# Genesis-Embodied-AI/ThinShellLab

Hardware: AMD Instinct MI355X
Metric: element-steps/s (fwd+adjoint), 100k-tri cloth; 1/2/4/8-GPU scaling (higher is better)
Workload: dtype f64

## Files before the change

### include/tsl_hip.h

```cpp
#ifndef TSL_HIP_H
#define TSL_HIP_H
#include <stdint.h>

#ifdef __cplusplus
extern "C" {
#endif

typedef struct tsl_ctx tsl_ctx;

typedef struct {
  int32_t N, M, NV, NF, v_offset;
  double dx, mass, Kl, Ka, Kb, k_angle;
  const int32_t* f2v_host;
  const int32_t* counter_face_host;
  const int32_t* counter_point_host;
  const double* rest_area_host;
  const double* rest_len_host;
} tsl_cloth_desc;

typedef struct {
  int32_t kind, n_verts, n_cells, v_offset;
  double mu, lam, alpha;
  const int32_t* tets_host;
  const double* B_host;
  const double* W_host;
} tsl_elastic_desc;

typedef struct {
  int32_t b_idx, v_start, v_end;
  int32_t mu_is_param;
  double mu;
} tsl_contact_pair;

typedef struct { int32_t v_start, v_end, f_start, f_end; } tsl_body;

typedef struct {
  int32_t tot_NV, tot_NF;
  double dt, k_contact, eps_contact, eps_v, damping;
  int32_t max_n_constraints;
  int32_t n_cloth;   const tsl_cloth_desc* cloths;
  int32_t n_elastic; const tsl_elastic_desc* elastics;
  int32_t n_body;    const tsl_body* bodies;
  int32_t n_pair;    const tsl_contact_pair* pairs;
  const double* mass_host;
  const double* gravity_host;
  const int32_t* faces_host;
  const int32_t* frozen_host;
  double grid_h;
} tsl_scene_desc;

typedef struct {
  int32_t newton_iters, ls_evals, cg_iters, solves, restarts, fallback, nc;
  double last_delta, last_alpha, energy;
  int32_t unconverged, attained, factorizations, plans;
  double max_rel_residual, max_backward_error;
} tsl_step_stats;

typedef struct {
  int32_t iters, restarts, flag;
  double rel_residual;
  int32_t method;
  int32_t attained;
  double backward_error;
} tsl_solve_stats;

const char* tsl_version(void);
const char* tsl_last_error(void);

int tsl_ctx_create(const tsl_scene_desc* desc, tsl_ctx** out);
void tsl_ctx_destroy(tsl_ctx* ctx);
int tsl_set_stream(tsl_ctx* ctx, void* hip_stream);

int tsl_set_param(tsl_ctx* ctx, const char* key, double value);
int tsl_set_frozen(tsl_ctx* ctx, const int32_t* frozen_host);
int tsl_set_ext_force(tsl_ctx* ctx, const double* ext_force_host);
int tsl_set_gravity(tsl_ctx* ctx, const double* gravity_host);

int tsl_energy(tsl_ctx* ctx, const double* pos_dev, const double* prev_pos_dev, const double* vel_dev,
               const double* ref_angle_dev, double* energy_host);

int tsl_assemble(tsl_ctx* ctx, const double* pos_dev, const double* prev_pos_dev, const double* vel_dev,
                 const double* ref_angle_dev, int spd, double* grad_dev);

int tsl_solve(tsl_ctx* ctx, const double* rhs_dev, double* x_dev, tsl_solve_stats* stats_host);

int tsl_step(tsl_ctx* ctx, double* pos_dev, double* prev_pos_dev, double* vel_dev, double* ref_angle_dev,
             tsl_step_stats* stats_host);

int tsl_contact_detect(tsl_ctx* ctx, const double* pos_dev, const double* prev_pos_dev, int32_t* nc_host);
int tsl_contact_reset(tsl_ctx* ctx);
int tsl_contact_counts(tsl_ctx* ctx, int32_t* out2_host);

int tsl_update_ref_angle(tsl_ctx* ctx, const double* pos_dev, double* ref_angle_dev);

int tsl_adjoint_step(tsl_ctx* ctx, int step, int tot_timestep, const double* pos_buffer_dev, double* pos_grad_dev,
                     const double* ref_angle_buffer_dev, double* angleref_grad_dev, double* tmp_z_frozen_dev,
                     double adjoint_damping, tsl_solve_stats* stats_host);

int tsl_elastic_force(tsl_ctx* ctx, const double* pos_dev, double* force_dev);

int tsl_param_grad(tsl_ctx* ctx, const double* pos_dev, const double* ref_angle_dev, double* out_host);

int tsl_friction_grad(tsl_ctx* ctx, const double* pos_dev, double* out_host);

int tsl_param_grad_keys(tsl_ctx* ctx, const double* pos_dev, const double* ref_angle_dev, const double* p_dev, const char* const* keys,
                        int32_t n_keys, double* out_host);

int tsl_matrix_nnzb(tsl_ctx* ctx, int32_t* nb_host, int32_t* nnzb_host);
int tsl_matrix_export(tsl_ctx* ctx, int32_t* row_ptr_host, int32_t* col_host, double* vals_host);
int tsl_matrix_import(tsl_ctx* ctx, const double* vals_host);
int tsl_constraints_export(tsl_ctx* ctx, int32_t* idx_host, double* w_host, double* k_host, double* dx0_host,
                           double* T_host, double* n_host, double* mu_host, int32_t max_n);
int tsl_contact_blocks_export(tsl_ctx* ctx, double* blocks_host, int32_t max_n, int32_t masked);
int tsl_proj_export(tsl_ctx* ctx, int32_t* proj_flag_host, int32_t* proj_dir_host, int32_t* proj_idx_host, double* proj_w_host);
int tsl_proj_import(tsl_ctx* ctx, const int32_t* proj_flag_host, const int32_t* proj_dir_host);
int tsl_set_border(tsl_ctx* ctx, const int32_t* border_flag_host);

int tsl_spd_project(tsl_ctx* ctx, double* blocks_dev, int32_t n_blocks, int32_t D);

int tsl_profile_reset(tsl_ctx* ctx, int enable);
int tsl_profile_read(tsl_ctx* ctx, double* spmv_ms_host, int64_t* spmv_launches_host, int64_t* spmv_bytes_per_launch_host);
int tsl_profile_read_events(tsl_ctx* ctx, double* spmv_ms_hip_events_host);
int tsl_bench_spmv(tsl_ctx* ctx, int variant, int reps, double* us_per_launch_host);

int tsl_bench_direct(tsl_ctx* ctx, int cls, int reps, double* out4_host);
int tsl_direct_info(tsl_ctx* ctx, double* out10_host);
int tsl_direct_counters(tsl_ctx* ctx, double* out_host, int32_t n);

typedef struct tsl_group tsl_group;
int tsl_group_create(tsl_ctx* const* ctxs, int32_t n, tsl_group** out);
void tsl_group_destroy(tsl_group* g);
int tsl_group_step(tsl_group* g, double* const* pos, double* const* prev_pos, double* const* vel, double* const* ref_angle, tsl_step_stats* stats_host);
int tsl_group_adjoint_step(tsl_group* g, int step, int T, const double* const* pos_buffer, double* const* pos_grad, const double* const* ref_buffer,
                           double* const* angleref_grad, double* const* tmp_z_frozen, const double* adj_damping_host, tsl_solve_stats* stats_host);
int tsl_group_info(tsl_group* g, double* out9_host);

#ifdef __cplusplus
}
#endif
#endif
```

### thinshelllab_amd/_lib.py

```python
import ctypes as C
import os

_HERE = os.path.dirname(os.path.abspath(__file__))
LIB_PATH = os.environ.get("TSL_HIP_LIB") or os.path.join(_HERE, "lib", "libtsl_hip.so")


class TslLibraryError(RuntimeError):
    pass


class TslError(RuntimeError):
    pass


class ClothDesc(C.Structure):
    _fields_ = [("N", C.c_int32), ("M", C.c_int32), ("NV", C.c_int32), ("NF", C.c_int32), ("v_offset", C.c_int32),
                ("dx", C.c_double), ("mass", C.c_double), ("Kl", C.c_double), ("Ka", C.c_double), ("Kb", C.c_double), ("k_angle", C.c_double),
                ("f2v", C.c_void_p), ("counter_face", C.c_void_p), ("counter_point", C.c_void_p), ("rest_area", C.c_void_p), ("rest_len", C.c_void_p)]


class ElasticDesc(C.Structure):
    _fields_ = [("kind", C.c_int32), ("n_verts", C.c_int32), ("n_cells", C.c_int32), ("v_offset", C.c_int32),
                ("mu", C.c_double), ("lam", C.c_double), ("alpha", C.c_double),
                ("tets", C.c_void_p), ("B", C.c_void_p), ("W", C.c_void_p)]


class ContactPair(C.Structure):
    _fields_ = [("b_idx", C.c_int32), ("v_start", C.c_int32), ("v_end", C.c_int32), ("mu_is_param", C.c_int32), ("mu", C.c_double)]


class Body(C.Structure):
    _fields_ = [("v_start", C.c_int32), ("v_end", C.c_int32), ("f_start", C.c_int32), ("f_end", C.c_int32)]


class SceneDesc(C.Structure):
    _fields_ = [("tot_NV", C.c_int32), ("tot_NF", C.c_int32),
                ("dt", C.c_double), ("k_contact", C.c_double), ("eps_contact", C.c_double), ("eps_v", C.c_double), ("damping", C.c_double),
                ("max_n_constraints", C.c_int32),
                ("n_cloth", C.c_int32), ("cloths", C.POINTER(ClothDesc)),
                ("n_elastic", C.c_int32), ("elastics", C.POINTER(ElasticDesc)),
                ("n_body", C.c_int32), ("bodies", C.POINTER(Body)),
                ("n_pair", C.c_int32), ("pairs", C.POINTER(ContactPair)),
                ("mass", C.c_void_p), ("gravity", C.c_void_p), ("faces", C.c_void_p), ("frozen", C.c_void_p),
                ("grid_h", C.c_double)]


class StepStats(C.Structure):
    _fields_ = [("newton_iters", C.c_int32), ("ls_evals", C.c_int32), ("cg_iters", C.c_int32), ("solves", C.c_int32),
                ("restarts", C.c_int32), ("fallback", C.c_int32), ("nc", C.c_int32),
                ("last_delta", C.c_double), ("last_alpha", C.c_double), ("energy", C.c_double),
                ("unconverged", C.c_int32), ("attained", C.c_int32), ("factorizations", C.c_int32), ("plans", C.c_int32),
                ("max_rel_residual", C.c_double), ("max_backward_error", C.c_double)]

    def as_dict(self):
        return {k: getattr(self, k) for k, _ in self._fields_}


class SolveStats(C.Structure):
    _fields_ = [("iters", C.c_int32), ("restarts", C.c_int32), ("flag", C.c_int32), ("rel_residual", C.c_double),
                ("method", C.c_int32), ("attained", C.c_int32), ("backward_error", C.c_double)]

    def as_dict(self):
        return {k: getattr(self, k) for k, _ in self._fields_}


EXPORTS = [
    "tsl_version", "tsl_last_error", "tsl_ctx_create", "tsl_ctx_destroy", "tsl_set_stream", "tsl_set_param", "tsl_set_frozen",
    "tsl_set_ext_force", "tsl_set_gravity", "tsl_energy", "tsl_assemble", "tsl_solve", "tsl_step", "tsl_contact_detect",
    "tsl_contact_reset", "tsl_contact_counts", "tsl_update_ref_angle", "tsl_adjoint_step", "tsl_param_grad", "tsl_param_grad_keys", "tsl_friction_grad", "tsl_elastic_force", "tsl_matrix_nnzb", "tsl_matrix_export", "tsl_matrix_import",
    "tsl_constraints_export", "tsl_contact_blocks_export", "tsl_proj_export", "tsl_proj_import", "tsl_set_border", "tsl_spd_project", "tsl_profile_reset", "tsl_profile_read", "tsl_profile_read_events",
    "tsl_bench_spmv", "tsl_bench_direct", "tsl_direct_info", "tsl_direct_counters",
    "tsl_group_create", "tsl_group_destroy", "tsl_group_step", "tsl_group_adjoint_step", "tsl_group_info",
]

_lib = None


def load():
    global _lib
    if _lib is not None:
        return _lib
    import torch
    if not os.path.exists(LIB_PATH):
        raise TslLibraryError(
            f"{LIB_PATH} not found: build it with `python -c 'import __graft_entry__ as g; g.build()'` "
            "(hipcc --offload-arch=gfx950). thinshelllab_amd has no CPU fallback.")
    try:
        L = C.CDLL(LIB_PATH)
    except OSError as e:
        raise TslLibraryError(f"cannot load {LIB_PATH}: {e}") from e
    L.tsl_version.restype = C.c_char_p
    L.tsl_last_error.restype = C.c_char_p
    L.tsl_ctx_create.argtypes = [C.POINTER(SceneDesc), C.POINTER(C.c_void_p)]
    L.tsl_ctx_destroy.argtypes = [C.c_void_p]
    L.tsl_ctx_destroy.restype = None
    L.tsl_set_stream.argtypes = [C.c_void_p, C.c_void_p]
    L.tsl_set_param.argtypes = [C.c_void_p, C.c_char_p, C.c_double]
    L.tsl_set_frozen.argtypes = [C.c_void_p, C.c_void_p]
    L.tsl_set_ext_force.argtypes = [C.c_void_p, C.c_void_p]
    L.tsl_set_gravity.argtypes = [C.c_void_p, C.c_void_p]
    L.tsl_energy.argtypes = [C.c_void_p] + [C.c_void_p] * 4 + [C.POINTER(C.c_double)]
    L.tsl_assemble.argtypes = [C.c_void_p] + [C.c_void_p] * 4 + [C.c_int, C.c_void_p]
    L.tsl_solve.argtypes = [C.c_void_p, C.c_void_p, C.c_void_p, C.POINTER(SolveStats)]
    L.tsl_step.argtypes = [C.c_void_p] + [C.c_void_p] * 4 + [C.POINTER(StepStats)]
    L.tsl_contact_detect.argtypes = [C.c_void_p, C.c_void_p, C.c_void_p, C.POINTER(C.c_int32)]
    L.tsl_contact_reset.argtypes = [C.c_void_p]
    L.tsl_contact_counts.argtypes = [C.c_void_p, C.POINTER(C.c_int32)]
    L.tsl_update_ref_angle.argtypes = [C.c_void_p, C.c_void_p, C.c_void_p]
    L.tsl_adjoint_step.argtypes = [C.c_void_p, C.c_int, C.c_int, C.c_void_p, C.c_void_p, C.c_void_p, C.c_void_p, C.c_void_p, C.c_double,
                                   C.POINTER(SolveStats)]
    L.tsl_matrix_nnzb.argtypes = [C.c_void_p, C.POINTER(C.c_int32), C.POINTER(C.c_int32)]
    L.tsl_matrix_export.argtypes = [C.c_void_p, C.c_void_p, C.c_void_p, C.c_void_p]
    L.tsl_matrix_import.argtypes = [C.c_void_p, C.c_void_p]
    L.tsl_constraints_export.argtypes = [C.c_void_p] + [C.c_void_p] * 7 + [C.c_int32]
    L.tsl_contact_blocks_export.argtypes = [C.c_void_p, C.c_void_p, C.c_int32, C.c_int32]
    L.tsl_proj_export.argtypes = [C.c_void_p] + [C.c_void_p] * 4
    L.tsl_proj_import.argtypes = [C.c_void_p, C.c_void_p, C.c_void_p]
    L.tsl_set_border.argtypes = [C.c_void_p, C.c_void_p]
    L.tsl_spd_project.argtypes = [C.c_void_p, C.c_void_p, C.c_int32, C.c_int32]
    L.tsl_profile_reset.argtypes = [C.c_void_p, C.c_int]
    L.tsl_profile_read.argtypes = [C.c_void_p, C.POINTER(C.c_double), C.POINTER(C.c_int64), C.POINTER(C.c_int64)]
    L.tsl_profile_read_events.argtypes = [C.c_void_p, C.POINTER(C.c_double)]
    L.tsl_bench_spmv.argtypes = [C.c_void_p, C.c_int, C.c_int, C.POINTER(C.c_double)]
    L.tsl_bench_direct.argtypes = [C.c_void_p, C.c_int, C.c_int, C.POINTER(C.c_double)]
    L.tsl_direct_info.argtypes = [C.c_void_p, C.POINTER(C.c_double)]
    L.tsl_direct_counters.argtypes = [C.c_void_p, C.POINTER(C.c_double), C.c_int32]
    L.tsl_param_grad.argtypes = [C.c_void_p, C.c_void_p, C.c_void_p, C.POINTER(C.c_double)]
    L.tsl_friction_grad.argtypes = [C.c_void_p, C.c_void_p, C.POINTER(C.c_double)]
    L.tsl_param_grad_keys.argtypes = [C.c_void_p, C.c_void_p, C.c_void_p, C.c_void_p, C.POINTER(C.c_char_p), C.c_int32, C.POINTER(C.c_double)]
    L.tsl_elastic_force.argtypes = [C.c_void_p, C.c_void_p, C.c_void_p]
    L.tsl_group_create.argtypes = [C.POINTER(C.c_void_p), C.c_int32, C.POINTER(C.c_void_p)]
    L.tsl_group_destroy.argtypes = [C.c_void_p]
    L.tsl_group_destroy.restype = None
    L.tsl_group_step.argtypes = [C.c_void_p] + [C.POINTER(C.c_void_p)] * 4 + [C.POINTER(StepStats)]
    L.tsl_group_adjoint_step.argtypes = [C.c_void_p, C.c_int, C.c_int] + [C.POINTER(C.c_void_p)] * 5 + [C.POINTER(C.c_double), C.POINTER(SolveStats)]
    L.tsl_group_info.argtypes = [C.c_void_p, C.POINTER(C.c_double)]
    _lib = L
    return L


def check(rc, what=""):
    if rc < 0:
        raise TslError(f"{what}: {load().tsl_last_error().decode()}")
    return rc
```

### thinshelllab_amd/context.py

```python
import ctypes as C
import os

import numpy as np
import torch

from . import _lib
from ._lib import Body, ClothDesc, ContactPair, ElasticDesc, SceneDesc, SolveStats, StepStats, check


def _np(a, dt):
    return np.ascontiguousarray(a, dtype=dt)


def _ptr(t):
    if t is None:
        return None
    if isinstance(t, torch.Tensor):
        assert t.is_contiguous(), "tensor must be contiguous"
        return C.c_void_p(t.data_ptr())
    return C.c_void_p(t.ctypes.data)


class TslContext:
    def __init__(self, *, tot_NV, dt, mass, gravity, frozen, cloths=(), elastics=(), faces=None, bodies=(), pairs=(),
                 k_contact=1000.0, eps_contact=1e-3, eps_v=0.01, damping=1.0, max_n_constraints=10000, grid_h=0.003, device="cuda:0"):
        self.L = _lib.load()
        if not torch.cuda.is_available():
            raise _lib.TslLibraryError("no HIP device visible: thinshelllab_amd has no CPU path")
        self.device = torch.device(device)
        torch.cuda.set_device(self.device)
        self.tot_NV = int(tot_NV)
        self._keep = []
        cl = (ClothDesc * max(len(cloths), 1))()
        for i, c in enumerate(cloths):
            arrs = [_np(c["f2v"], np.int32), _np(c["counter_face"], np.int32), _np(c["counter_point"], np.int32),
                    _np(c["rest_area"], np.float64), _np(c["rest_len"], np.float64)]
            self._keep += arrs
            cl[i] = ClothDesc(c["N"], c["M"], c["NV"], c["NF"], c["v_offset"], c["dx"], c["mass"], c["Kl"], c["Ka"], c["Kb"], c["k_angle"],
                              *[a.ctypes.data for a in arrs])
        el = (ElasticDesc * max(len(elastics), 1))()
        for i, e in enumerate(elastics):
            arrs = [_np(e["tets"], np.int32), _np(e["B"], np.float64), _np(e["W"], np.float64)]
            self._keep += arrs
            el[i] = ElasticDesc(e["kind"], e["n_verts"], e["n_cells"], e["v_offset"], e["mu"], e["lam"], e["alpha"], *[a.ctypes.data for a in arrs])
        bd = (Body * max(len(bodies), 1))()
        for i, b in enumerate(bodies):
            bd[i] = Body(*[int(x) for x in b])
        pr = (ContactPair * max(len(pairs), 1))()
        for i, p in enumerate(pairs):
            mu = p[3]
            factor = float(p[4]) if len(p) > 4 else 0.0
            kind = 0 if isinstance(mu, (int, float)) else (2 if mu == "cloth_cloth" else 1)
            pr[i] = ContactPair(int(p[0]), int(p[1]), int(p[2]), kind, float(mu) if kind == 0 else factor)
        faces = _np(faces if faces is not None else np.zeros((0, 3)), np.int32)
        mass = _np(mass, np.float64); gravity = _np(gravity, np.float64); frozen = _np(frozen, np.int32)
        assert mass.shape == (tot_NV,) and gravity.shape == (tot_NV, 3) and frozen.shape == (3 * tot_NV,)
        d = SceneDesc(tot_NV, len(faces), dt, k_contact, eps_contact, eps_v, damping, int(max_n_constraints),
                      len(cloths), cl, len(elastics), el, len(bodies), bd, len(pairs), pr,
                      mass.ctypes.data, gravity.ctypes.data, faces.ctypes.data, frozen.ctypes.data, grid_h)
        self.h = C.c_void_p()
        check(self.L.tsl_ctx_create(C.byref(d), C.byref(self.h)), "tsl_ctx_create")
        self.n_body = len(bodies)
        self.n_cface = sum(c["NF"] for c in cloths)
        self.dt = dt
        self.max_n_constraints = int(max_n_constraints)
        self.L.tsl_set_stream(self.h, C.c_void_p(torch.cuda.current_stream(self.device).cuda_stream))
        for kv in os.environ.get("TSL_PARAMS", "").split(","):
            if "=" in kv:
                k, v = kv.split("=", 1)
                self.set_param(k.strip(), float(v))

    def close(self):
        if getattr(self, "h", None) is not None and self.h:
            g = getattr(self, "_group", None)
            if g is not None:
                g.close()
            self.L.tsl_ctx_destroy(self.h)
            self.h = None

    def __del__(self):
        try:
            self.close()
        except Exception:
            pass

    def set_param(self, key, value):
        check(self.L.tsl_set_param(self.h, key.encode(), float(value)), f"tsl_set_param({key})")

    def set_frozen(self, frozen):
        f = _np(frozen, np.int32)
        check(self.L.tsl_set_frozen(self.h, f.ctypes.data), "tsl_set_frozen")

    def set_ext_force(self, f):
        f = _np(f, np.float64)
        check(self.L.tsl_set_ext_force(self.h, f.ctypes.data), "tsl_set_ext_force")

    def set_gravity(self, g):
        g = _np(g, np.float64)
        check(self.L.tsl_set_gravity(self.h, g.ctypes.data), "tsl_set_gravity")

    def energy(self, pos, prev_pos, vel, ref_angle):
        self.refresh_stream()
        e = C.c_double(0)
        check(self.L.tsl_energy(self.h, _ptr(pos), _ptr(prev_pos), _ptr(vel), _ptr(ref_angle), C.byref(e)), "tsl_energy")
        return e.value

    def assemble(self, pos, prev_pos, vel, ref_angle, spd=True, grad=None):
        self.refresh_stream()
        check(self.L.tsl_assemble(self.h, _ptr(pos), _ptr(prev_pos), _ptr(vel), _ptr(ref_angle), int(bool(spd)), _ptr(grad)), "tsl_assemble")

    def solve(self, rhs, x=None):
        self.refresh_stream()
        if x is None:
            x = torch.empty_like(rhs)
        st = SolveStats()
        check(self.L.tsl_solve(self.h, _ptr(rhs), _ptr(x), C.byref(st)), "tsl_solve")
        return x, st.as_dict()

    def step(self, pos, prev_pos, vel, ref_angle):
        self.refresh_stream()
        st = StepStats()
        check(self.L.tsl_step(self.h, _ptr(pos), _ptr(prev_pos), _ptr(vel), _ptr(ref_angle), C.byref(st)), "tsl_step")
        return st.as_dict()

    def contact_detect(self, pos, prev_pos):
        self.refresh_stream()
        nc = C.c_int32(0)
        check(self.L.tsl_contact_detect(self.h, _ptr(pos), _ptr(prev_pos), C.byref(nc)), "tsl_contact_detect")
        return nc.value

    def contact_counts(self):
        out = (C.c_int32 * 2)()
        check(self.L.tsl_contact_counts(self.h, out), "tsl_contact_counts")
        return int(out[0]), int(out[1])

    def contact_reset(self):
        check(self.L.tsl_contact_reset(self.h), "tsl_contact_reset")

    def update_ref_angle(self, pos, ref_angle):
        check(self.L.tsl_update_ref_angle(self.h, _ptr(pos), _ptr(ref_angle)), "tsl_update_ref_angle")

    def adjoint_step(self, step, T, pos_buffer, pos_grad, ref_angle_buffer, angleref_grad, tmp_z_frozen, damping=1.0):
        self.refresh_stream()
        st = SolveStats()
        check(self.L.tsl_adjoint_step(self.h, int(step), int(T), _ptr(pos_buffer), _ptr(pos_grad), _ptr(ref_angle_buffer), _ptr(angleref_grad),
                                      _ptr(tmp_z_frozen), float(damping), C.byref(st)), "tsl_adjoint_step")
        return st.as_dict()

    def elastic_force(self, pos, out):
        check(self.L.tsl_elastic_force(self.h, _ptr(pos), _ptr(out)), "tsl_elastic_force")
        return out

    def friction_grad(self, pos):
        out = C.c_double(0)
        check(self.L.tsl_friction_grad(self.h, _ptr(pos), C.byref(out)), "tsl_friction_grad")
        return out.value

    def param_grad(self, pos, ref_angle):
        out = (C.c_double * 3)()
        check(self.L.tsl_param_grad(self.h, _ptr(pos), _ptr(ref_angle), out), "tsl_param_grad")
        return dict(kb=out[0], mu=out[1], lam=out[2])

    def param_grads(self, pos, ref_angle, keys, p=None):
        keys = list(keys)
        if not keys:
            return {}
        self.refresh_stream()
        arr = (C.c_char_p * len(keys))(*[k.encode() for k in keys])
        out = (C.c_double * len(keys))()
        check(self.L.tsl_param_grad_keys(self.h, _ptr(pos), _ptr(ref_angle), _ptr(p), arr, len(keys), out), "tsl_param_grad_keys")
        return {k: out[j] for j, k in enumerate(keys)}

    def matrix(self):
        nb = C.c_int32(0); nnzb = C.c_int32(0)
        check(self.L.tsl_matrix_nnzb(self.h, C.byref(nb), C.byref(nnzb)), "tsl_matrix_nnzb")
        rp = np.zeros(nb.value + 1, np.int32); col = np.zeros(nnzb.value, np.int32); vals = np.zeros((nnzb.value, 3, 3), np.float64)
        check(self.L.tsl_matrix_export(self.h, rp.ctypes.data, col.ctypes.data, vals.ctypes.data), "tsl_matrix_export")
        return rp, col, vals

    def matrix_import(self, vals):
        rp, col, _ = self.matrix()
        v = np.ascontiguousarray(vals, dtype=np.float64)
        assert v.shape == (len(col), 3, 3), (v.shape, len(col))
        check(self.L.tsl_matrix_import(self.h, v.ctypes.data), "tsl_matrix_import")

    def matrix_csr(self):
        import scipy.sparse as sp
        rp, col, vals = self.matrix()
        n = 3 * (len(rp) - 1)
        return sp.bsr_matrix((vals, col, rp), shape=(n, n)).tocsr()

    def constraints(self):
        m = self.max_n_constraints
        idx = np.zeros((m, 4), np.int32); w = np.zeros((m, 3)); k = np.zeros(m); dx0 = np.zeros((m, 3)); T = np.zeros((m, 6)); n = np.zeros((m, 3)); mu = np.zeros(m)
        cnt = check(self.L.tsl_constraints_export(self.h, idx.ctypes.data, w.ctypes.data, k.ctypes.data, dx0.ctypes.data, T.ctypes.data, n.ctypes.data,
                                                  mu.ctypes.data, m), "tsl_constraints_export")
        return dict(idx=idx[:cnt], w=w[:cnt], k=k[:cnt], dx0=dx0[:cnt], T=T[:cnt], n=n[:cnt], mu=mu[:cnt])

    def contact_blocks(self, masked=True):
        m = self.max_n_constraints
        blk = np.zeros((m, 12, 12))
        cnt = check(self.L.tsl_contact_blocks_export(self.h, blk.ctypes.data, m, int(masked)), "tsl_contact_blocks_export")
        return blk[:cnt]

    def operator_csr(self):
        import scipy.sparse as sp
        A = self.matrix_csr().tolil()
        cons = self.constraints()
        blk = self.contact_blocks(True)
        for c in range(len(blk)):
            idx = cons["idx"][c]
            dofs = np.concatenate([3 * idx[k] + np.arange(3) for k in range(4)])
            for r in range(12):
                for cc in range(12):
                    if blk[c, r, cc] != 0.0:
                        A[dofs[r], dofs[cc]] += blk[c, r, cc]
        return A.tocsr()

    def proj_export(self):
        nb = max(self.n_body, 1)
        flag = np.zeros((nb, self.tot_NV), np.int32); dr = np.zeros((nb, self.tot_NV), np.int32)
        pidx = np.zeros((nb, self.tot_NV, 3), np.int32); pw = np.zeros((nb, self.tot_NV, 3))
        check(self.L.tsl_proj_export(self.h, flag.ctypes.data, dr.ctypes.data, pidx.ctypes.data, pw.ctypes.data), "tsl_proj_export")
        return flag, dr, pidx, pw

    def proj_import(self, flag, dr):
        flag = _np(flag, np.int32); dr = _np(dr, np.int32)
        check(self.L.tsl_proj_import(self.h, flag.ctypes.data, dr.ctypes.data), "tsl_proj_import")

    def set_border(self, border):
        b = _np(border, np.int32)
        assert b.shape == (self.tot_NV,)
        check(self.L.tsl_set_border(self.h, b.ctypes.data), "tsl_set_border")

    def refresh_stream(self):
        self.L.tsl_set_stream(self.h, C.c_void_p(torch.cuda.current_stream(self.device).cuda_stream))

    def spd_project(self, blocks, D):
        check(self.L.tsl_spd_project(self.h, _ptr(blocks), blocks.numel() // (D * D), D), "tsl_spd_project")

    def profile_reset(self, enable=True):
        check(self.L.tsl_profile_reset(self.h, int(bool(enable))), "tsl_profile_reset")

    def profile_read(self):
        ms = C.c_double(0); n = C.c_int64(0); b = C.c_int64(0)
        check(self.L.tsl_profile_read(self.h, C.byref(ms), C.byref(n), C.byref(b)), "tsl_profile_read")
        ev = C.c_double(0)
        check(self.L.tsl_profile_read_events(self.h, C.byref(ev)), "tsl_profile_read_events")
        return dict(ms_per_launch=ms.value, launches=n.value, bytes_per_launch=b.value, ms_per_launch_events=ev.value)

    def bench_direct(self, cls, reps=20):
        out = (C.c_double * 4)()
        check(self.L.tsl_bench_direct(self.h, int(cls), int(reps), out), "tsl_bench_direct")
        return dict(us_per_launch=out[0], flops_per_launch=out[1], bytes_per_launch=out[2], launches=int(out[3]))

    def direct_info(self):
        out = (C.c_double * 10)()
        check(self.L.tsl_direct_info(self.h, out), "tsl_direct_info")
        keys = ("plans", "factorizations", "applications", "perturbed_pivots", "plan_seconds", "supernodes", "levels", "batches", "flops_per_factorization", "front_bytes")
        return dict(zip(keys, [float(v) for v in out]))

    def direct_counters(self):
        out = (C.c_double * 13)()
        check(self.L.tsl_direct_counters(self.h, out, 13), "tsl_direct_counters")
        keys = ("flow_launches", "flow_aborts", "plan_cache_hits", "panel_bytes", "schur_bytes", "g_bytes", "schur_entries", "plans_parked",
                "berr_seen", "berr_accepted", "berr_max", "berr_rel_max", "tiles_guarded")
        return dict(zip(keys, [float(v) for v in out]))

    def bench_spmv(self, variant=20, reps=500):
        us = C.c_double(0)
        check(self.L.tsl_bench_spmv(self.h, int(variant), int(reps), C.byref(us)), "tsl_bench_spmv")
        return us.value
```

### thinshelllab_amd/csrc/k_cloth.hpp

```cpp
#pragma once
#include "tsl_ctx.hpp"
#include "tsl_device.hpp"

struct FaceGeom {
  d3 n;
  double h[3];
  double ca[3];
};

TSL_DEV FaceGeom face_geom(const d3 P[3]) {
  FaceGeom g;
  g.n = normalized(cross(P[1] - P[0], P[2] - P[1]));
#pragma unroll
  for (int l = 0; l < 3; l++) {
    const d3 p = P[l], a = P[(l + 1) % 3], b = P[(l + 2) % 3];
    const d3 en = cross(g.n, b - a);
    g.h[l] = fabs(dot(p - a, en)) / norm(en);
    g.ca[l] = dot(normalized(a - p), normalized(b - p));
  }
  return g;
}

TSL_DEV bool sign_neg(const d3& n2, const d3& e) { return dot(n2, e) < -1e-10 * norm(e); }
TSL_DEV double dihedral(const d3& n1, const d3& n2, const d3& e) {
// ... 267 lines not shown
        for (int k = 0; k < 3; k++) {
          const double G = (j == k) ? (1.0 - dd[j] * dd[j]) / len : dd[j] * dd[k] / len;
          K[j * 3 + k] = dl * G + dl2 * dd[j] * dd[k];
        }
      if (spd) {
        if constexpr (LIT) spd_literal3<10>(K);
        else spd_clamp<3>(K);
      }
#pragma unroll
      for (int j = 0; j < 3; j++)
#pragma unroll
        for (int k = 0; k < 3; k++) {
          const double kv = K[j * 3 + k];
          L[(l * 3 + j) * 9 + l * 3 + k] += kv;
          L[(l * 3 + j) * 9 + m * 3 + k] -= kv;
          L[(m * 3 + j) * 9 + l * 3 + k] -= kv;
          L[(m * 3 + j) * 9 + m * 3 + k] += kv;
        }
    }

    {
      const d3 Nn = cross(P[1] - P[0], P[2] - P[0]);
      const double nN = norm(Nn);
      const double area = 0.5 * nN;
      const double base_area = A.V[f];
      const double da = -c.Ka * 2.0 * (1.0 - area / base_area);
      const double da2 = c.Ka * 2.0 / base_area;
      const d3 nh = Nn / nN;
      d3 e[3], g[3];
#pragma unroll
      for (int l = 0; l < 3; l++) { e[l] = P[(l + 2) % 3] - P[(l + 1) % 3]; g[l] = 0.5 * cross(nh, e[l]); }
      const double nx[9] = {0, -nh.z, nh.y, nh.z, 0, -nh.x, -nh.y, nh.x, 0};
      const double a2 = 2.0 * area, a2c = a2 * a2 * a2;
#pragma unroll
      for (int l = 0; l < 3; l++)
#pragma unroll
        for (int m = 0; m < 3; m++) {
          const double elm = dot(e[l], e[m]);
          const double sigma = (m == l) ? 0.0 : ((m == (l + 2) % 3) ? 1.0 : -1.0);
          const double el[3] = {e[l].x, e[l].y, e[l].z}, em[3] = {e[m].x, e[m].y, e[m].z};
          const double gl[3] = {g[l].x, g[l].y, g[l].z}, gm[3] = {g[m].x, g[m].y, g[m].z};
          const int o = 3 - l - m;
#pragma unroll
          for (int j = 0; j < 3; j++)
#pragma unroll
            for (int k = 0; k < 3; k++) {
              double h2 = 0.5 * ((((j == k) ? elm : 0.0) - em[j] * el[k] - 4.0 * gl[j] * gm[k]) / nN + sigma * nx[j * 3 + k]);
              if (l != m && j != k) {
                const d3 p1 = P[l], p2 = P[m], p3 = P[o];
                const int d2 = 3 - j - k;
                const double Cjk = (p2[j] - p1[j]) * (p3[k] - p1[k]) - (p3[j] - p1[j]) * (p2[k] - p1[k]);
                const double Cjd = (p2[j] - p1[j]) * (p3[d2] - p1[d2]) - (p3[j] - p1[j]) * (p2[d2] - p1[d2]);
                const double S = (p2[k] - p3[k]) * Cjk + (p2[d2] - p3[d2]) * Cjd;
                h2 -= 0.5 * (p1[j] - p3[j]) * Cjk * S / a2c;
              }
              L[(l * 3 + j) * 9 + m * 3 + k] += da2 * gl[j] * gm[k] + da * h2;
            }
        }
    }
  }

  {
    const d3 n = ld3(A.norm_dir, f);
    double hgt[3], ca[3], ci[3];
    m3 Mm[3];
#pragma unroll
    for (int l = 0; l < 3; l++) {
      const int nb = A.cf[3 * f + l];
      const d3 e = P[(l + 1) % 2] - P[l];
      bool judge = true;
      ci[l] = 0;
      if (nb != -1) {
        const d3 n2 = ld3(A.norm_dir, nb);
        if (sign_neg(n2, e)) judge = false;
        const double theta = dihedral(n, n2, e);
        ci[l] = 2.0 * c.Kb * (theta - ref_angle[3 * f + l]) * c.dx * c.dx * (1.0 / 3.0);
      }
      const d3 nd = judge ? -n : n;
      const d3 p = P[l], a = P[(l + 1) % 3], b = P[(l + 2) % 3];
      d3 en = cross(nd, b - a);
      if (dot(en, a - p) > 0) en = -en;
      Mm[l] = m3_outer(nd, en);
      ca[l] = dot(normalized(a - p), normalized(b - p));
      hgt[l] = fabs(dot(p - a, en)) / norm(en);
    }
    double di[3];
#pragma unroll
    for (int l = 0; l < 3; l++) di[l] = ci[(l + 1) % 3] * ca[(l + 2) % 3] + ci[(l + 2) % 3] * ca[(l + 1) % 3] - ci[l];
    const double* Qc = Q + (size_t)cid * 90;
#pragma unroll
    for (int l = 0; l < 3; l++)
#pragma unroll
      for (int lm = 0; lm < 2; lm++) {
        const int m = (l + lm) % 3;
        const double inv = 1.0 / (hgt[l] * hgt[m]);
        double Hlm[9];
#pragma unroll
        for (int j = 0; j < 3; j++)
#pragma unroll
          for (int k = 0; k < 3; k++) Hlm[j * 3 + k] = inv * (di[l] * Mm[m].m[k * 3 + j] + di[m] * Mm[l].m[j * 3 + k]);
        if (l == m) {
          const int i1 = (l + 1) % 3, i2 = (l + 2) % 3;
          const double* q1 = Qc + (l * 3 + i1) * 10;
          const double* q2 = Qc + (l * 3 + i2) * 10;
#pragma unroll
          for (int e9 = 0; e9 < 9; e9++) Hlm[e9] -= q1[0] * q1[1 + e9] + q2[0] * q2[1 + e9];
        } else {
          const int i3 = 3 - l - m;
          const double* q3 = Qc + (l * 3 + i3) * 10;
#pragma unroll
          for (int e9 = 0; e9 < 9; e9++) Hlm[e9] += q3[0] * q3[1 + e9];
        }
#pragma unroll
        for (int j = 0; j < 3; j++)
#pragma unroll
          for (int k = 0; k < 3; k++) {
            L[(l * 3 + j) * 9 + m * 3 + k] += Hlm[j * 3 + k];
            if (l != m) L[(m * 3 + j) * 9 + l * 3 + k] += Hlm[k * 3 + j];
          }
      }
  }

  if (CLAMP_ALL) spd_clamp<9>(L);
  double* R = rec + (size_t)t * 81;
#pragma unroll
  for (int l = 0; l < 3; l++)
#pragma unroll
    for (int m = 0; m < 3; m++)
#pragma unroll
      for (int j = 0; j < 3; j++)
#pragma unroll
        for (int k = 0; k < 3; k++) R[(l * 3 + m) * 9 + j * 3 + k] = L[(l * 3 + j) * 9 + m * 3 + k];
}

__global__ void __launch_bounds__(256) k_cloth_hess_hinge(ClothArgs A, const double* __restrict__ pos, double* __restrict__ rec) {
  const int h = blockIdx.x * blockDim.x + threadIdx.x;
  if (h >= A.n_hinge) return;
  const int f1 = A.hg_info[8 * h], l = A.hg_info[8 * h + 1], f2 = A.hg_info[8 * h + 2], p4 = A.hg_info[8 * h + 3], p21 = A.hg_info[8 * h + 4];
  const ClothDev c = A.cloth[A.cid[f1]];
  int v1[3], v2[3]; d3 P1[3], P2[3];
  load_face(pos, A.f2v, f1, v1, P1);
  load_face(pos, A.f2v, f2, v2, P2);
  const FaceGeom g1 = face_geom(P1), g2 = face_geom(P2);
  d3 g[4];
  hinge_grad(g1, g2, l, p4, p21, g);
  const double d2 = 2.0 * c.Kb * c.dx * c.dx * (1.0 / 3.0);
  double* R = rec + (size_t)h * 16;
#pragma unroll
  for (int j = 0; j < 4; j++) { R[3 * j] = g[j].x; R[3 * j + 1] = g[j].y; R[3 * j + 2] = g[j].z; }
  R[12] = d2;
}

#define CG_BPW 28
__global__ void __launch_bounds__(256) k_cloth_gather(int n_blk, const int* __restrict__ base, const int* __restrict__ ptr, const unsigned* __restrict__ ent, int n_hinge, int n_cface,
                                                      const double* __restrict__ hrec, const double* __restrict__ frec, const double* __restrict__ trec, double* __restrict__ vals) {
  __shared__ double tile[9][CG_BPW + 1];
  const int b0 = blockIdx.x * CG_BPW, t = threadIdx.x;
  if (t < 9 * CG_BPW) {
    const int bl = t / 9, e9 = t - 9 * bl, b = b0 + bl, r = e9 / 3, c = e9 - 3 * r;
    double acc = 0.0;
    if (b < n_blk) {
      for (int q = ptr[b]; q < ptr[b + 1]; q++) {
        const unsigned e = ent[q];
        const int el = (int)((e >> 4) & 0x7ffffff), pr = (int)(e & 15);
        if ((e >> 30) == 1) {
          acc += trec[(size_t)(el & 0x3ffffff) * 144 + pr * 9 + e9];
        } else if (e >> 31) {
          const int j = pr >> 2, k = pr & 3;
          const double* R = hrec + (size_t)el * 16;
          acc += R[12] * (R[3 * j + r] * R[3 * k + c]);
        } else {
          acc += frec[(size_t)el * 81 + pr * 9 + e9];
        }
      }
    }
    tile[e9][bl] = acc;
  }
  __syncthreads();
  if (t < 9 * CG_BPW) {
    const int e9 = t / CG_BPW, bl = t - CG_BPW * e9, b = b0 + bl;
    if (b < n_blk) vals[(size_t)base[b] + 64 * e9] += tile[e9][bl];
  }
}

__global__ void k_cloth_update_ref(ClothArgs A, const double* __restrict__ pos, double* __restrict__ ref_angle) {
  const int h = blockIdx.x * blockDim.x + threadIdx.x;
  if (h >= A.n_hinge) return;
  const int f1 = A.hg_info[8 * h], l = A.hg_info[8 * h + 1], f2 = A.hg_info[8 * h + 2];
  const ClothDev c = A.cloth[A.cid[f1]];
  const d3 n1 = ld3(A.norm_dir, f1), n2 = ld3(A.norm_dir, f2);
  const d3 e = ld3(pos, A.f2v[3 * f1 + (l + 1) % 2]) - ld3(pos, A.f2v[3 * f1 + l]);
  const double theta = dihedral(n1, n2, e);
  const double dis = theta - ref_angle[3 * f1 + l];
  const double ad = fabs(dis);
  if (ad > c.k_angle) ref_angle[3 * f1 + l] += (ad - c.k_angle) * dis / ad;
}
```

### thinshelllab_amd/csrc/k_solver.hpp

```cpp
#pragma once
#include "tsl_ctx.hpp"
#include "tsl_device.hpp"

struct CgScal {
  double pAp[4], rzn[4], rr[4];
  double bb, thresh2, energy, pmax, aux[4];
  int flag, iters, pad0, pad1;
};
static_assert(sizeof(CgScal) <= sizeof(SolverScalars), "CgScal must fit the scalar record");

__global__ void k_mask_matrix(int n_slices, const int* __restrict__ slice_off, const int* __restrict__ slice_len, const int* __restrict__ colidx,
                              const unsigned char* __restrict__ fz, const double* __restrict__ mdt2, const double* __restrict__ src, double* __restrict__ dst, int NV) {
  const int slice = blockIdx.x, lane = threadIdx.x & 63;
  if (slice >= n_slices) return;
  const int off = slice_off[slice], len = slice_len[slice];
  const int p = slice * 64 + lane;
  const unsigned rm = (p < NV) ? fz[p] : 7u;
  const double md = (p < NV) ? mdt2[p] : 0.0;
  for (int k = threadIdx.x >> 6; k < len; k += (blockDim.x >> 6)) {
    const int c = colidx[off + 64 * k + lane];
    const unsigned cm = fz[c];
    const size_t base = ((size_t)off + 64 * (size_t)k) * 9 + lane;
#pragma unroll
    for (int e = 0; e < 9; e++) {
      const int r = e / 3, cc = e % 3;
      double v = src[base + 64 * e];
      if (((rm >> r) & 1u) || ((cm >> cc) & 1u)) v = 0.0;
      if (c == p && r == cc && ((rm >> r) & 1u)) v = md;
      dst[base + 64 * e] = v;
    }
  }
}

__global__ void k_block_jacobi(int NV, const int* __restrict__ diag_perm, const double* __restrict__ vals, const double* __restrict__ extra, double* __restrict__ Dinv) {
  const int p = blockIdx.x * blockDim.x + threadIdx.x;
  if (p >= NV) return;
  const size_t base = (size_t)diag_perm[p];
  m3 D;
#pragma unroll
  for (int e = 0; e < 9; e++) D.m[e] = vals[base + 64 * e] + (extra ? extra[9 * (size_t)p + e] : 0.0);
  const m3 Di = m3_inv(D);
#pragma unroll
  for (int e = 0; e < 9; e++) Dinv[9 * (size_t)p + e] = Di.m[e];
}

__global__ void k_gather_perm(int NV, const int* __restrict__ perm, const double* __restrict__ in, double* __restrict__ out) {
  const int p = blockIdx.x * blockDim.x + threadIdx.x;
  if (p >= NV) return;
  st3(out, p, ld3(in, perm[p]));
}
__global__ void k_scatter_perm(int NV, const int* __restrict__ perm, const double* __restrict__ in, double* __restrict__ out) {
  const int p = blockIdx.x * blockDim.x + threadIdx.x;
  if (p >= NV) return;
  st3(out, perm[p], ld3(in, p));
}

struct ContactRows {
  const int* ptr;
  const int* ent;
  const int4* rows;
  const double* H;
  int nv;
};
template <int NVEC>
TSL_DEV void contact_slice_add(const ContactRows& C, int e0, int e1, int row0, const double* __restrict__ x, const double* __restrict__ x2, double (*acc)[64]) {
  (void)e0; (void)e1;
  const int lane = threadIdx.x & 63, nw = blockDim.x >> 6;
  for (int l = threadIdx.x >> 6; l < 64; l += nw) {
    const bool in = row0 + l < C.nv;
    const int r0 = in ? C.ptr[row0 + l] : 0, r1 = in ? C.ptr[row0 + l + 1] : 0;
    if (r1 <= r0) { if (lane == 0) { acc[0][l] = 0.0; acc[1][l] = 0.0; acc[2][l] = 0.0; if (NVEC == 2) { acc[3][l] = 0.0; acc[4][l] = 0.0; acc[5][l] = 0.0; } } continue; }
    double y0 = 0, y1 = 0, y2 = 0, q0 = 0, q1 = 0, q2 = 0;
    for (int e = r0 + lane; e < r1; e += 64) {
      const int q = C.ent[e];
      const int4 r4 = C.rows[e];
      const int c = q >> 2, a = q & 3;
      const double* H = C.H + 144 * (size_t)c + 36 * a;
      const int pb[4] = {r4.x, r4.y, r4.z, r4.w};
#pragma unroll
      for (int b = 0; b < 4; b++) {
        const d3 xb = ld3(x, pb[b]);
        y0 += H[3 * b] * xb.x + H[3 * b + 1] * xb.y + H[3 * b + 2] * xb.z;
        y1 += H[12 + 3 * b] * xb.x + H[12 + 3 * b + 1] * xb.y + H[12 + 3 * b + 2] * xb.z;
        y2 += H[24 + 3 * b] * xb.x + H[24 + 3 * b + 1] * xb.y + H[24 + 3 * b + 2] * xb.z;
        if (NVEC == 2) {
          const d3 wb = ld3(x2, pb[b]);
          q0 += H[3 * b] * wb.x + H[3 * b + 1] * wb.y + H[3 * b + 2] * wb.z;
          q1 += H[12 + 3 * b] * wb.x + H[12 + 3 * b + 1] * wb.y + H[12 + 3 * b + 2] * wb.z;
          q2 += H[24 + 3 * b] * wb.x + H[24 + 3 * b + 1] * wb.y + H[24 + 3 * b + 2] * wb.z;
        }
      }
    }
    y0 = wave_sum(y0); y1 = wave_sum(y1); y2 = wave_sum(y2);
    if (NVEC == 2) { q0 = wave_sum(q0); q1 = wave_sum(q1); q2 = wave_sum(q2); }
    if (lane == 0) { acc[0][l] = y0; acc[1][l] = y1; acc[2][l] = y2; if (NVEC == 2) { acc[3][l] = q0; acc[4][l] = q1; acc[5][l] = q2; } }
  }
}

__global__ void __launch_bounds__(256)
k_spmv(int NV, int n_slices, const int* __restrict__ slice_off, const int* __restrict__ slice_len, const int* __restrict__ colidx,
       const double* __restrict__ vals, const double* __restrict__ x, double* __restrict__ y, CgScal* sc, int slot, int check_flag,
       unsigned long long* prof) {
  if (check_flag && sc->flag) return;
  unsigned long long t_start = 0;
  if (prof) t_start = wall_clock64();
  const int p = blockIdx.x * blockDim.x + threadIdx.x;
  const int slice = p >> 6, lane = p & 63;
  double acc = 0.0;
  if (slice < n_slices) {
    const int off = slice_off[slice], len = slice_len[slice];
    double y0 = 0, y1 = 0, y2 = 0;
    const int* cp = colidx + off + lane;
    const double* vp = vals + (size_t)off * 9 + lane;
#pragma unroll 2
    for (int k = 0; k < len; k++) {
      const int c = cp[64 * k];
      const double* a = vp + (size_t)k * 576;
      const double a0 = a[0], a1 = a[64], a2 = a[128], a3 = a[192], a4 = a[256], a5 = a[320], a6 = a[384], a7 = a[448], a8 = a[512];
      const d3 xj = ld3(x, c);
      y0 += a0 * xj.x + a1 * xj.y + a2 * xj.z;
      y1 += a3 * xj.x + a4 * xj.y + a5 * xj.z;
      y2 += a6 * xj.x + a7 * xj.y + a8 * xj.z;
    }
    if (p < NV) {
      st3(y, p, d3(y0, y1, y2));
      const d3 xi = ld3(x, p);
      acc = xi.x * y0 + xi.y * y1 + xi.z * y2;
    }
  }
  if (slot >= 0) {
    acc = wave_sum(acc);
    if ((threadIdx.x & 63) == 0 && acc != 0.0) atomicAdd(&sc->pAp[slot], acc);
    if (p == 0) { const int z = (slot + 2) & 3; sc->pAp[z] = 0; sc->rzn[z] = 0; sc->rr[z] = 0; }
  }
  if (prof && (threadIdx.x & 63) == 0) {
    const size_t w = (size_t)blockIdx.x * (blockDim.x >> 6) + (threadIdx.x >> 6);
    prof[2 * w] = t_start;
    prof[2 * w + 1] = (unsigned long long)wall_clock64();
  }
}

#define SELL_U 4
template <int U, int NVEC, int WPS, bool NT, typename VT>
TSL_DEV void sell_wave_trip(const int* __restrict__ cp, const VT* __restrict__ vp, int len, int k0, const double* __restrict__ x, const double* __restrict__ x2,
                            double& y0, double& y1, double& y2, double& q0, double& q1, double& q2) {
  int kk[U], c[U];
  double m[U];
#pragma unroll
  for (int u = 0; u < U; u++) {
    const int k = k0 + u * WPS;
    kk[u] = k < len ? k : k0;
    m[u] = k < len ? 1.0 : 0.0;
    c[u] = NT ? __builtin_nontemporal_load(cp + 64 * kk[u]) : cp[64 * kk[u]];
  }
  double a[U][9];
#pragma unroll
  for (int u = 0; u < U; u++) {
    const VT* ap = vp + (size_t)kk[u] * 576;
#pragma unroll
    for (int e = 0; e < 9; e++) a[u][e] = (double)(NT ? __builtin_nontemporal_load(ap + 64 * e) : ap[64 * e]);
  }
  d3 xj[U], wj[U];
#pragma unroll
  for (int u = 0; u < U; u++) {
    xj[u] = ld3(x, c[u]);
    if (NVEC == 2) wj[u] = ld3(x2, c[u]);
  }
#pragma unroll
  for (int u = 0; u < U; u++) {
    y0 += m[u] * (a[u][0] * xj[u].x + a[u][1] * xj[u].y + a[u][2] * xj[u].z);
    y1 += m[u] * (a[u][3] * xj[u].x + a[u][4] * xj[u].y + a[u][5] * xj[u].z);
    y2 += m[u] * (a[u][6] * xj[u].x + a[u][7] * xj[u].y + a[u][8] * xj[u].z);
    if (NVEC == 2) {
      q0 += m[u] * (a[u][0] * wj[u].x + a[u][1] * wj[u].y + a[u][2] * wj[u].z);
      q1 += m[u] * (a[u][3] * wj[u].x + a[u][4] * wj[u].y + a[u][5] * wj[u].z);
      q2 += m[u] * (a[u][6] * wj[u].x + a[u][7] * wj[u].y + a[u][8] * wj[u].z);
    }
  }
}
template <int NVEC, int WPS, bool NT, typename VT = double>
TSL_DEV void sell_wave_product(const int* __restrict__ cp, const VT* __restrict__ vp, int len, int w, const double* __restrict__ x, const double* __restrict__ x2,
                               double& y0, double& y1, double& y2, double& q0, double& q1, double& q2) {
  const int nk = (len - w + WPS - 1) / WPS;
  if (nk == SELL_U + 1) {
// ... 529 lines not shown
```

### thinshelllab_amd/csrc/tsl_ctx.hpp

```cpp
#pragma once
#include <memory>
#include <hip/hip_runtime.h>
#include <stdint.h>

#include <algorithm>
#include <cmath>
#include <cstdio>
#include <cstring>
#include <string>
#include <vector>

#include "../../include/tsl_hip.h"
#include "k_body.hpp"
#include "direct_plan.hpp"

#define TSL_SLICE 64

extern thread_local std::string g_tsl_err;
int tsl_fail(const char* fmt, ...);

#define HIP_OK(call)                                                                     \
  do {                                                                                   \
    hipError_t e__ = (call);                                                             \
    if (e__ != hipSuccess) return tsl_fail("%s failed: %s (%s:%d)", #call, hipGetErrorString(e__), __FILE__, __LINE__); \
// ... 57 lines not shown
  DevBuf<float> Cinv;
  DevBuf<int> cbad;
  DevBuf<double> gjD, gjR, gjC, gjP;
  int gj_ld = 0;
};
struct MgCloth {
  int v_offset = 0, N0 = 0, M0 = 0;
  std::vector<MgLevel*> lv;
  int dense_lv = -1;
  ~MgCloth() { for (auto* l : lv) delete l; }
};

#define DS_NSIDE 2
struct DsPlanSlot {
  DirectPlan plan;
  std::vector<int> h_cons, h_cset;
  uint64_t key = 0;
  long stamp = 0;
  bool used = false;
  DevBuf<int> level_sn, pmap, vtx, blk_ld, wl_front, wl_row, blk_q, cgr_ptr, cgr_ent, cgr_ld;
  DevBuf<long long> blk_dst, cgr_dst;
  DevBuf<DsFrontDesc> fr, frl;
  DevBuf<DsChildRec> ch_rec;
};
struct DirectSolver {
  char* pin = nullptr; size_t pin_cap = 0, pin_off = 0;
  int enable = -1;
  bool hard = false;
  int hard_steps = 0, probe_cap = 60, probe_every = 16;
  hipStream_t zstream = 0;
  hipEvent_t ev_zfork = nullptr, ev_zero = nullptr;
  bool prezero_pending = false;
  size_t prezero_n = 0;
  int prezero = 1;
  hipStream_t fstream[2] = {nullptr, nullptr};
  hipEvent_t ev_ffork = nullptr, ev_fjoin[2] = {nullptr, nullptr};
  hipEvent_t ev_la[5] = {nullptr, nullptr, nullptr, nullptr, nullptr};
  hipStream_t lastream = nullptr;
  int eager_n = 0; const double* eager_r = nullptr; double* eager_z = nullptr;
  int lookahead = 103;
  int device = 0;
  int flow_wgs_last = 0;
  int flow = 3, flow_cap = 0, flow_epoch = 0;
  int flow_token = 0, flow_token_fd = -1;
  long flow_token_asked = 0;
  int small_rounds = 2;
  int xcd_map = 64;
  long n_flow = 0, n_flow_abort = 0;
  DevBuf<double> flow_x;
  DevBuf<int> flow_f;
  DevBuf<unsigned long long> tlog;
  int gemv_wide_below = 300;
  int g32_below = 1100;
  bool cons_checked = false;
  double* h_anorm = nullptr;
  int bench_batch = -1;
  double piv_tol = 1e-11;
  int fallback_cap = 1000;
  int leaf = 64;
  bool static_ready = false, numeric_valid = false;
  bool have_factor = false;
  int dbg = 0;
  double berr_tol = 1e-12, berr_rel_cap = 50.0;
  long berr_seen = 0, berr_accepted = 0;
  double berr_max = 0, berr_rel_max = 0;
  int n_setup_fail = 0;
  std::vector<std::unique_ptr<DsPlanSlot>> cache;
  int cache_cap = 64, cache_mb = 1024;
  long cache_clock = 0, n_plan_hits = 0, n_plan_evicted = 0;
  DirectPlan plan;
  std::vector<DsGrid> grids;
  std::vector<DsBlock> blocks;
  std::vector<int> row_ptr;
  std::vector<int> h_c2s;
  std::vector<int> h_cons;
  std::vector<int> h_cset;
  bool plan_valid = false;
  DevBuf<int> level_sn, pmap, vtx, blk_ld, bad, wl_front, wl_row, blk_q, cgr_ptr, cgr_ent, cgr_ld;
  DevBuf<long long> blk_dst, cgr_dst;
  DevBuf<DsFrontDesc> fr, frl;
  DevBuf<DsChildRec> ch_rec;
  DevBuf<double> arena, sarena, garena, scr, w;
  long n_plans = 0, n_factor = 0, n_apply = 0, n_perturbed = 0;
  long plan_gen = 0;
  bool keep_host_maps = false;
  bool merged = false;
  DirectSolver* token_lender = nullptr;
  double t_plan = 0;
  double anorm = 0;
  bool anorm_valid = false;
  int anorm_age = 0;
  int anorm_spd = -1;
  DevBuf<double> anorm_dev;
  hipEvent_t ev0 = nullptr, ev1 = nullptr;
};

struct tsl_group;
struct tsl_ctx {
  tsl_group* group = nullptr;
  hipStream_t stream = 0;
  hipStream_t user_stream = 0;
  hipEvent_t ev_in = nullptr, ev_out = nullptr;
  int depth = 0;
  hipGraphExec_t pcg_graph = nullptr;
  long pcg_graph_key = -1;
  hipGraphExec_t mr_graph = nullptr;
  long mr_graph_key = -1;
  int use_graph = 1;
  int NV = 0, NF = 0;
  double dt = 5e-3, k_contact = 1000, eps_contact = 1e-3, eps_v = 0.01, damping = 1.0, mu_cloth_elastic = 1.0, mu_cloth_cloth = 1.0;
  int max_n_constraints = 10000;
  int newton_cap = 1000, plastic = 0, contact_enable = 1;
  int spd_literal = 0;
  double cg_tol = 1e-10;
  int cg_maxit = 200000, cg_check = 32;
  double grid_h = 0.003;
  double grid_extent = 0.2;

  std::vector<ClothDev> h_cloth;
  DevBuf<ClothDev> d_cloth;
  int n_cface = 0, n_hinge = 0;
  DevBuf<int> cf_f2v, cf_cf, cf_cp, cf_cloth;
  DevBuf<double> cf_V, cf_li;
  DevBuf<int> cf_blk;
  DevBuf<int> cf_order;
  DevBuf<int> hg_info;
  DevBuf<int> hg_v;
  DevBuf<int> hg_blk;
  DevBuf<double> norm_dir;
  DevBuf<double> quirk;
  std::vector<int> h_cf_f2v, h_cf_cf, h_cf_cp;
  std::vector<double> h_stvk;
  DevBuf<double> d_stvk, cf_dminv;
  int n_stvk = 0;

  std::vector<ElasticDev> h_el;
  DevBuf<ElasticDev> d_el;
  int n_tet = 0;
  DevBuf<int> tet_v, tet_el, tet_blk;
  DevBuf<double> tet_B, tet_W;

  DevBuf<double> mass, grav, fext;
  DevBuf<int> frozen;
  DevBuf<int> diag_blk;
  std::vector<int> h_frozen;
  std::vector<double> h_mass;

  int n_slices = 0;
  long n_slots = 0;
  std::vector<int> h_rowpos, h_perm, h_slice_off, h_slice_len, h_colidx;
  std::vector<std::vector<int>> h_rows;
  DevBuf<int> rowpos, perm, slice_off, slice_len, colidx, diag_perm;
  DevBuf<double> vals, vals_full;
  DevBuf<float> vals32;
  bool vals32_valid = false;
  int mg_f32 = 1;
  DevBuf<double> Dinv;
  DevBuf<unsigned char> fzmask;
  DevBuf<double> mdt2;
  long nnzb = 0;

  DevBuf<double> v_x, v_r, v_z, v_p, v_Ap, v_b, v_t0, v_t1, v_t2, v_t3, v_t4, v_mg;
  BodyDenseArgs bd_args{};
  int bd_rows_n = 0, bd_n3max = 0, bd_wg = 0, bd_scr_n = 0, bd_enable = -1;
  size_t bd_w_total = 0;
  bool bd_valid = false;
  DevBuf<int> bd_rows, bd_body_of, bd_local_of, bd_bad;
  DevBuf<double> bd_W, bd_scr;
  DevBuf<double> bd_rb;
  int pcg_body_fold = 1;
  int mg_st_f32 = 1;
  int mg_chunk = 0;
  double mr_eta = 0.3;
  int mg_fr_rows = 32;
  DevBuf<float> bd_Binv;
  DevBuf<double> gm_V, gm_h;
  DevBuf<double> gm_Z;
  DevBuf<unsigned> cg_ent;
  DevBuf<int> cg_base, cg_ptr;
  DevBuf<double> cg_hrec, cg_frec;
  DevBuf<int> trans;
  DevBuf<int> vg_ptr, vg_idx;
  DevBuf<double> vg_stage, cg_trec;
  int vg_ns = 0, vg_hinge0 = 0, vg_tet0 = 0;
  DevBuf<double> vg_stage2;
  DevBuf<double> dot_part; DevBuf<int> dot_ticket;
  DevBuf<double> e_part;
  int n_cgblk = 0, n_cgblk_cloth = 0;
  DevBuf<double> tet_V;
  long tet_V_count = 0;
  int tet_warm = 1;
  DevBuf<double> ir_part;
  DevBuf<int> ir_ticket;
  double* h_ir = nullptr;
  double last_xmax = 0;
  bool last_xmax_valid = false;
  int gmres_m = 300, use_gmres = 1, use_minres = 1, verbose = 0;
  double adj_clamp = 1000.0;
  int adj_clamp_angleref = 1;
  DevBuf<double> dmu_accum;
  DevBuf<double> pg_part, pg_out;
  DevBuf<double> vals_pc, c_H_pc;
  bool pc_separate = false, pc_frozen = false, in_step = false;
  bool cdiag_valid = false;
  bool dinv_valid = false;
  const double *st_pos = nullptr, *st_prev = nullptr, *st_vel = nullptr, *st_ref = nullptr;
  int fwd_spd_pc = 1;
  int adj_spd_pc = 1;
  DevBuf<SolverScalars> scal;
  DevBuf<double> part_pAp, part_rz, part_rr;
  SolverScalars* h_scal = nullptr;
  SolverScalars* h_scal2 = nullptr;
  hipEvent_t rb_event[2] = {nullptr, nullptr};
  hipStream_t side = 0;
  hipEvent_t ev_fork = nullptr, ev_fork0 = nullptr, ev_g2 = nullptr, ev_join = nullptr, ev_join2 = nullptr, ev_hh = nullptr, ev_gf = nullptr;
  hipStream_t side2 = 0;

  DevBuf<double> F, pdir, x1;

  int n_body = 0, n_pair = 0;
  std::vector<tsl_body> h_bodies;
  std::vector<tsl_contact_pair> h_pairs;
  std::vector<int> self_contact;
  DevBuf<int> faces;
  DevBuf<int> border;
  DevBuf<double> vn;
  DevBuf<int> proj_flag, proj_dir, proj_idx;
  DevBuf<double> proj_w;
  DevBuf<int> nc_dev;
  int nc = 0;
  DevBuf<int> c_idx;
  DevBuf<double> c_w, c_n, c_dx0, c_k, c_mu, c_T;
  DevBuf<int> cr_ptr, cr_cnt, cr_fill, cr_ent;
  DevBuf<int4> cr_rows;
  DevBuf<int> cr_tmp;
  DevBuf<int> c_kind;
  DevBuf<double> c_H;
  DevBuf<double> c_Hfull;
  DevBuf<double> c_diag;
  DevBuf<double> c_G;
  DevBuf<int> grid_key, grid_val, grid_key2, grid_val2, grid_range;
  DevBuf<int> vnf_ptr, vnf_lst;
  DevBuf<int> cq_flag, cq_scan;
  DevBuf<int> grid_scan;
  std::vector<size_t> gb_f0, gb_t0, gb_s0;
  DevBuf<int> grid_cnt, grid_ptr, grid_cur, scan_tmp;
  int grid_buckets_max = 0;
  int max_body_faces = 0;
  struct EeDesc { int pair, target, qoff, nq; };
  int contact_ee = 0, nc_ee = 0;
  std::vector<int> h_ee_e0;
  std::vector<EeDesc> ee_desc;
  std::vector<char> ee_target;
  long ee_qtot = 0;
  bool ee_ready = false;
  DevBuf<int> ee_edges, ee_qlist;
  DevBuf<int> ee_key, ee_val, ee_key2, ee_val2, ee_range, ee_bcnt, ee_bptr, ee_bcur, ee_bscan;
  std::vector<size_t> ee_f0, ee_t0, ee_s0;
  DevBuf<unsigned long long> ee_lmax;
  DevBuf<int> ee_qcnt, ee_qscan, ee_cand, ee_scan_tmp, ee_nvf;

  std::vector<MgCloth*> mg;
  int mg_enable = -1;
  double mg_omega = 0.0;
  int mg_pi_iters = 12;
  DevBuf<double> mg_omega0, mg_pi_part, mg_pi_norm;
  int mg_nu = 1, mg_coarse_sweeps = 8, mg_fuse = 1, mg_fuse_restrict = 1, mg_max_levels = 16, mg_coarse_exact = 1, mg_coarse_lag = 0, mg_dense_nodes = 64, mg_dense_auto = 1;
  double last_step_iters_per_solve = 0.0;
  bool warm_valid = false;
  bool mg_cinv_valid = false;
  bool mg_ops_valid = false, mg_suspended = false, mg_omega_valid = false;

  int prof_enable = 0;
  hipEvent_t ev0 = nullptr, ev1 = nullptr;
  double prof_ms = 0;
  long prof_launches = 0, prof_samples = 0;
  DevBuf<unsigned long long> prof_dev;
  long prof_dev_used = 0, prof_dev_cap = 512;
  size_t prof_waves = 0;
  double prof_event_ms = 0, prof_dev_ticks = 0;
  long prof_dev_n = 0;
  std::vector<std::pair<hipEvent_t, hipEvent_t>> ev_pool;
  size_t ev_used = 0;
  long prof_chunks = 0;
  double tm_loop = 0;
  bool ev_sample_next = false;

  DirectSolver ds;
  bool ds_probe = false;
  bool ds_suspended = false;
  tsl_step_stats step_stats{};
  ~tsl_ctx() { for (auto* m : mg) delete m; }
};

struct Scope {
  tsl_ctx* c;
  explicit Scope(tsl_ctx* c_) : c(c_) {
    if (c->depth++ == 0) { (void)hipEventRecord(c->ev_in, c->user_stream); (void)hipStreamWaitEvent(c->stream, c->ev_in, 0); }
  }
  ~Scope() {
    if (--c->depth == 0) { (void)hipEventRecord(c->ev_out, c->stream); (void)hipStreamWaitEvent(c->user_stream, c->ev_out, 0); }
  }
};
```

### thinshelllab_amd/csrc/tsl_hip.hip

```cpp
#include <stdarg.h>
#include <cctype>
#include <chrono>
#include <mutex>

#include <array>
#include <map>

#include "k_cloth.hpp"
#include "k_contact.hpp"
#include "k_fem.hpp"
#include "k_mg.hpp"
#include "k_param.hpp"
#include "k_solver.hpp"
#include "tsl_ctx.hpp"

thread_local std::string g_tsl_err;
int tsl_fail(const char* fmt, ...) {
  char buf[1024];
  va_list ap;
  va_start(ap, fmt);
  vsnprintf(buf, sizeof(buf), fmt, ap);
  va_end(ap);
  g_tsl_err = buf;
  return -1;
// ... 91 lines not shown
static TetArgs tet_args(tsl_ctx* c) {
  TetArgs A;
  A.n_tet = c->n_tet; A.el = c->d_el.p; A.tv = c->tet_v.p; A.tel = c->tet_el.p; A.B = c->tet_B.p; A.W = c->tet_W.p; A.gstage = nullptr;
  return A;
}
static ContactArgs contact_args(tsl_ctx* c) {
  ContactArgs A;
  A.idx = c->c_idx.p; A.w = c->c_w.p; A.n = c->c_n.p; A.dx0 = c->c_dx0.p; A.k = c->c_k.p; A.mu = c->c_mu.p; A.T = c->c_T.p;
  A.k_contact = c->k_contact; A.eps_contact = c->eps_contact; A.eps_vh = c->eps_v * c->dt;
  return A;
}

static int upload_frozen(tsl_ctx* c) {
  TSL_TRY(c->frozen.upload(c->h_frozen));
  std::vector<unsigned char> fz(c->NV);
  std::vector<double> md(c->NV);
  for (int p = 0; p < c->NV; p++) {
    const int v = c->h_perm[p];
    fz[p] = (unsigned char)((c->h_frozen[3 * v] ? 1 : 0) | (c->h_frozen[3 * v + 1] ? 2 : 0) | (c->h_frozen[3 * v + 2] ? 4 : 0));
    md[p] = c->h_mass[v] / (c->dt * c->dt);
  }
  TSL_TRY(c->fzmask.upload(fz));
  TSL_TRY(c->mdt2.upload(md));
  return 0;
}

extern "C" int tsl_ctx_create(const tsl_scene_desc* d, tsl_ctx** out) {
  if (!d || !out) return tsl_fail("tsl_ctx_create: null argument");
  int ndev = 0;
  if (hipGetDeviceCount(&ndev) != hipSuccess || ndev == 0) return tsl_fail("tsl_ctx_create: no HIP device (this engine has no CPU path)");
  tsl_ctx* c = new tsl_ctx();
  if (hipStreamCreateWithFlags(&c->stream, hipStreamNonBlocking) != hipSuccess || hipEventCreateWithFlags(&c->ev_in, hipEventDisableTiming) != hipSuccess ||
      hipEventCreateWithFlags(&c->ev_out, hipEventDisableTiming) != hipSuccess) { delete c; return tsl_fail("stream / event creation failed"); }
  c->NV = d->tot_NV; c->NF = d->tot_NF;
  c->dt = d->dt; c->k_contact = d->k_contact; c->eps_contact = d->eps_contact; c->eps_v = d->eps_v; c->damping = d->damping;
  c->max_n_constraints = d->max_n_constraints > 0 ? d->max_n_constraints : 10000;
  c->grid_h = d->grid_h > 0 ? d->grid_h : 0.003;
  const int NV = c->NV;
  std::vector<std::vector<int>> cliques;

  std::vector<int> f2v, cf, cp, cid, hinfo, hv;
  std::vector<double> V, li;
  int face_start = 0;
  for (int ci = 0; ci < d->n_cloth; ci++) {
    const tsl_cloth_desc& cd = d->cloths[ci];
    ClothDev cdv{face_start, cd.NF, cd.v_offset, cd.NV, cd.dx, cd.mass, cd.Kl, cd.Ka, cd.Kb, cd.k_angle};
    c->h_cloth.push_back(cdv);
    if ((cd.N + 1) * (cd.M + 1) == cd.NV) c->ds.grids.push_back(DsGrid{cd.v_offset, cd.N, cd.M});
    for (int i = 0; i < cd.NF; i++) {
      for (int k = 0; k < 3; k++) {
        f2v.push_back(cd.f2v_host[3 * i + k] + cd.v_offset);
        const int nb = cd.counter_face_host[3 * i + k];
        cf.push_back(nb < 0 ? -1 : nb + face_start);
        cp.push_back(cd.counter_point_host[3 * i + k]);
        li.push_back(cd.rest_len_host[3 * i + k]);
      }
      cid.push_back(ci);
      V.push_back(cd.rest_area_host[i]);
      cliques.push_back({cd.f2v_host[3 * i] + cd.v_offset, cd.f2v_host[3 * i + 1] + cd.v_offset, cd.f2v_host[3 * i + 2] + cd.v_offset});
    }
    for (int i = 0; i < cd.NF; i++)
      for (int l = 0; l < 3; l++) {
        const int nb = cd.counter_face_host[3 * i + l];
        if (nb > i) {
          const int p4 = cd.counter_point_host[3 * i + l];
          const int p11 = (l + 1) % 3;
          int p21 = (p4 + 1) % 3;
          if (cd.f2v_host[3 * i + p11] != cd.f2v_host[3 * nb + p21]) p21 = (p4 + 2) % 3;
          const int a = cd.f2v_host[3 * i + l] + cd.v_offset, b = cd.f2v_host[3 * i + (l + 1) % 3] + cd.v_offset;
          const int cc = cd.f2v_host[3 * i + (l + 2) % 3] + cd.v_offset, dd = cd.f2v_host[3 * nb + p4] + cd.v_offset;
          const int info[8] = {i + face_start, l, nb + face_start, p4, p21, 0, 0, 0};
          hinfo.insert(hinfo.end(), info, info + 8);
          hv.push_back(a); hv.push_back(b); hv.push_back(cc); hv.push_back(dd);
          cliques.push_back({a, b, cc, dd});
        }
      }
    face_start += cd.NF;
  }
  c->n_cface = face_start;
  c->n_hinge = (int)hv.size() / 4;
  {
    const int nh = c->n_hinge;
    std::map<std::array<int, 3>, int> cls;
    std::vector<int> key(nh), idx(nh);
    for (int h = 0; h < nh; h++) {
      const std::array<int, 3> t{hv[4 * h + 1] - hv[4 * h], hv[4 * h + 2] - hv[4 * h], hv[4 * h + 3] - hv[4 * h]};
      auto it = cls.find(t);
      if (it == cls.end()) it = cls.emplace(t, (int)cls.size()).first;
      key[h] = it->second; idx[h] = h;
    }
    std::stable_sort(idx.begin(), idx.end(), [&](int x, int y) { return key[x] != key[y] ? key[x] < key[y] : hv[4 * x] < hv[4 * y]; });
    std::vector<int> hinfo2(hinfo.size()), hv2(hv.size());
    for (int h = 0; h < nh; h++) {
      std::copy(hinfo.begin() + 8 * (size_t)idx[h], hinfo.begin() + 8 * (size_t)idx[h] + 8, hinfo2.begin() + 8 * (size_t)h);
      std::copy(hv.begin() + 4 * (size_t)idx[h], hv.begin() + 4 * (size_t)idx[h] + 4, hv2.begin() + 4 * (size_t)h);
    }
    hinfo.swap(hinfo2); hv.swap(hv2);
  }
  c->h_cf_f2v = f2v; c->h_cf_cf = cf; c->h_cf_cp = cp;

  std::vector<int> tv, tel;
  std::vector<double> tB, tW;
  int cell_start = 0;
  for (int ei = 0; ei < d->n_elastic; ei++) {
    const tsl_elastic_desc& ed = d->elastics[ei];
    ElasticDev edv{ed.kind, cell_start, ed.n_cells, ed.v_offset, ed.n_verts, ed.mu, ed.lam, ed.alpha};
    c->h_el.push_back(edv);
    c->ds.blocks.push_back(DsBlock{ed.v_offset, ed.n_verts});
    for (int t = 0; t < ed.n_cells; t++) {
      std::vector<int> cl;
      for (int k = 0; k < 4; k++) { tv.push_back(ed.tets_host[4 * t + k] + ed.v_offset); cl.push_back(ed.tets_host[4 * t + k] + ed.v_offset); }
      tel.push_back(ei);
      for (int k = 0; k < 9; k++) tB.push_back(ed.B_host[9 * t + k]);
      tW.push_back(ed.W_host[t]);
      cliques.push_back(cl);
    }
    cell_start += ed.n_cells;
  }
  c->n_tet = cell_start;

  Pattern P;
  build_pattern(NV, cliques, P);
  c->h_rows = P.rows; c->h_perm = P.perm; c->h_rowpos = P.rowpos; c->h_slice_off = P.slice_off; c->h_slice_len = P.slice_len; c->h_colidx = P.colidx;
  c->n_slices = P.n_slices; c->n_slots = P.n_slots;
  c->nnzb = 0;
  for (auto& r : P.rows) c->nnzb += (long)r.size();
  if (P.n_slots * 9 >= (1L << 31)) { delete c; return tsl_fail("matrix too large for 32-bit slot offsets (%ld slots)", P.n_slots); }
  std::vector<int> cfblk((size_t)c->n_cface * 9), hgblk((size_t)c->n_hinge * 16), tetblk((size_t)c->n_tet * 16), dblk(NV);
  for (int f = 0; f < c->n_cface; f++)
    for (int l = 0; l < 3; l++)
      for (int m = 0; m < 3; m++) cfblk[(size_t)f * 9 + l * 3 + m] = P.lookup(f2v[3 * f + l], f2v[3 * f + m]);
  for (int h = 0; h < c->n_hinge; h++)
    for (int j = 0; j < 4; j++)
      for (int k = 0; k < 4; k++) hgblk[(size_t)h * 16 + j * 4 + k] = P.lookup(hv[4 * h + j], hv[4 * h + k]);
  for (int t = 0; t < c->n_tet; t++)
    for (int j = 0; j < 4; j++)
      for (int k = 0; k < 4; k++) tetblk[(size_t)t * 16 + j * 4 + k] = P.lookup(tv[4 * t + j], tv[4 * t + k]);
  for (int v = 0; v < NV; v++) dblk[v] = P.lookup(v, v);
#define UP(buf, vec) do { if (c->buf.upload(vec)) { delete c; return -1; } } while (0)
  UP(d_cloth, c->h_cloth); UP(cf_f2v, f2v); UP(cf_cf, cf); UP(cf_cp, cp); UP(cf_cloth, cid); UP(cf_V, V); UP(cf_li, li);
  std::vector<int> forder(c->n_cface);
  {
    std::map<std::array<int, 3>, int> cls;
    std::vector<int> key(c->n_cface);
    for (int f = 0; f < c->n_cface; f++) {
      const std::array<int, 3> t{f2v[3 * f + 1] - f2v[3 * f], f2v[3 * f + 2] - f2v[3 * f], 0};
      auto it = cls.find(t);
      if (it == cls.end()) it = cls.emplace(t, (int)cls.size()).first;
      key[f] = it->second; forder[f] = f;
    }
    std::stable_sort(forder.begin(), forder.end(), [&](int x, int y) { return key[x] != key[y] ? key[x] < key[y] : f2v[3 * x] < f2v[3 * y]; });
  }
  UP(cf_order, forder);
  std::vector<int> cg_base, cg_ptr;
  std::vector<unsigned> cg_ent;
  {
    std::vector<std::pair<int, unsigned>> tup;
    tup.reserve((size_t)c->n_cface * 9 + (size_t)c->n_hinge * 16);
    std::vector<int> fpos(c->n_cface);
    for (int t = 0; t < c->n_cface; t++) fpos[forder[t]] = t;
    for (int f = 0; f < c->n_cface; f++)
      for (int e = 0; e < 9; e++) tup.emplace_back(cfblk[(size_t)f * 9 + e], ((unsigned)fpos[f] << 4) | (unsigned)e);
    for (int h = 0; h < c->n_hinge; h++)
      for (int e = 0; e < 16; e++) tup.emplace_back(hgblk[(size_t)h * 16 + e], 0x80000000u | ((unsigned)h << 4) | (unsigned)e);
    for (int t = 0; t < c->n_tet; t++)
      for (int e = 0; e < 16; e++) tup.emplace_back(tetblk[(size_t)t * 16 + e], 0x40000000u | ((unsigned)t << 4) | (unsigned)e);
    auto is_tet = [](unsigned e) { return (e >> 30) == 1u; };
    std::sort(tup.begin(), tup.end(), [&](const std::pair<int, unsigned>& x, const std::pair<int, unsigned>& y) {
      if (is_tet(x.second) != is_tet(y.second)) return is_tet(y.second);
      return x < y;
    });
    cg_ent.reserve(tup.size());
    c->n_cgblk_cloth = 0;
    for (size_t i = 0; i < tup.size(); i++) {
      if (i == 0 || tup[i].first != tup[i - 1].first || is_tet(tup[i].second) != is_tet(tup[i - 1].second)) {
        cg_base.push_back(tup[i].first); cg_ptr.push_back((int)i);
        if (!is_tet(tup[i].second)) c->n_cgblk_cloth++;
      }
      cg_ent.push_back(tup[i].second);
    }
    cg_ptr.push_back((int)tup.size());
    c->n_cgblk = (int)cg_base.size();
    if (c->n_cface >= (1 << 26) || c->n_hinge >= (1 << 26) || c->n_tet >= (1 << 26)) { delete c; return tsl_fail("mesh too large for the packed gather lists"); }
  }
  std::vector<int> vg_ptr(NV + 1, 0), vg_idx;
  {
    c->vg_hinge0 = 3 * c->n_cface; c->vg_tet0 = c->vg_hinge0 + 4 * c->n_hinge; c->vg_ns = c->vg_tet0 + 4 * c->n_tet;
    for (int v : f2v) vg_ptr[v + 1]++;
    for (int v : hv) vg_ptr[v + 1]++;
    for (int v : tv) vg_ptr[v + 1]++;
    for (int v = 0; v < NV; v++) vg_ptr[v + 1] += vg_ptr[v];
    vg_idx.resize(vg_ptr[NV]);
    std::vector<int> cur(vg_ptr.begin(), vg_ptr.end() - 1);
    for (size_t i = 0; i < f2v.size(); i++) vg_idx[cur[f2v[i]]++] = (int)i;
    for (size_t i = 0; i < hv.size(); i++) vg_idx[cur[hv[i]]++] = c->vg_hinge0 + (int)i;
    for (size_t i = 0; i < tv.size(); i++) vg_idx[cur[tv[i]]++] = c->vg_tet0 + (int)i;
  }

  UP(cf_blk, cfblk); UP(hg_info, hinfo); UP(hg_v, hv); UP(hg_blk, hgblk);
  if (c->n_cgblk > 0) { UP(cg_base, cg_base); UP(cg_ptr, cg_ptr); UP(cg_ent, cg_ent); }
  UP(vg_ptr, vg_ptr); if (!vg_idx.empty()) UP(vg_idx, vg_idx);
  {
    std::vector<int> trans((size_t)P.n_slots, -1);
    for (int v = 0; v < NV; v++) {
      const int pr = P.rowpos[v], sl = pr >> 6, lane = pr & 63;
      for (int k = 0; k < (int)P.rows[v].size(); k++) trans[(size_t)P.slice_off[sl] + 64 * (size_t)k + lane] = P.lookup(P.rows[v][k], v);
    }
    UP(trans, trans);
  }
  UP(d_el, c->h_el); UP(tet_v, tv); UP(tet_el, tel); UP(tet_blk, tetblk); UP(tet_B, tB); UP(tet_W, tW);
  UP(diag_blk, dblk); UP(rowpos, P.rowpos); UP(perm, P.perm); UP(slice_off, P.slice_off); UP(slice_len, P.slice_len); UP(colidx, P.colidx);
  UP(diag_perm, P.diag_perm);
  c->h_mass.assign(d->mass_host, d->mass_host + NV);
  std::vector<double> grav(d->gravity_host, d->gravity_host + 3 * (size_t)NV), fext(3 * (size_t)NV, 0.0);
  UP(mass, c->h_mass); UP(grav, grav); UP(fext, fext);
  c->h_frozen.assign(d->frozen_host, d->frozen_host + 3 * (size_t)NV);
  if (upload_frozen(c)) { delete c; return -1; }
#undef UP
  int rc = 0;
  rc |= c->norm_dir.alloc((size_t)std::max(c->n_cface, 1) * 3);
  rc |= c->quirk.alloc((size_t)std::max(d->n_cloth, 1) * 90);
  rc |= c->dot_part.alloc(64 * 512); rc |= c->dot_ticket.alloc(512);
  if (!rc) (void)hipMemset(c->dot_ticket.p, 0, 512 * sizeof(int));
  rc |= c->vals.alloc((size_t)P.n_slots * 9); rc |= c->vals_full.alloc((size_t)P.n_slots * 9);
  rc |= c->Dinv.alloc((size_t)NV * 9);
  const size_t n3 = (size_t)NV * 3;
  rc |= c->v_x.alloc(n3); rc |= c->v_r.alloc(n3); rc |= c->v_z.alloc(n3); rc |= c->v_p.alloc(n3); rc |= c->v_Ap.alloc(n3); rc |= c->v_b.alloc(n3);
  rc |= c->v_t0.alloc(n3); rc |= c->v_t1.alloc(n3); rc |= c->v_t2.alloc(n3); rc |= c->v_t3.alloc(n3); rc |= c->v_t4.alloc(n3); rc |= c->v_mg.alloc(n3);
  rc |= c->F.alloc(n3); rc |= c->pdir.alloc(n3); rc |= c->x1.alloc(n3);
  rc |= c->scal.alloc(1);
  rc |= c->part_pAp.alloc((size_t)P.n_slices + (size_t)(c->max_n_constraints + 63) / 64 + 8); rc |= c->part_rz.alloc((size_t)NV / 256 + 8 + 1024); rc |= c->part_rr.alloc((size_t)NV / 256 + 8 + 1024);
  if (rc) { delete c; return -1; }
  if (hipHostMalloc((void**)&c->h_scal, sizeof(SolverScalars) > sizeof(CgScal) ? sizeof(SolverScalars) : sizeof(CgScal)) != hipSuccess) { delete c; return tsl_fail("hipHostMalloc failed"); }
  if (hipHostMalloc((void**)&c->h_scal2, 2 * sizeof(SolverScalars)) != hipSuccess) { delete c; return tsl_fail("hipHostMalloc failed"); }
  for (int i = 0; i < 2; i++)
    if (hipEventCreateWithFlags(&c->rb_event[i], hipEventDisableTiming) != hipSuccess) { delete c; return tsl_fail("hipEventCreate failed"); }
  if (hipStreamCreateWithFlags(&c->side, hipStreamNonBlocking) != hipSuccess || hipStreamCreateWithFlags(&c->side2, hipStreamNonBlocking) != hipSuccess ||
      hipEventCreateWithFlags(&c->ev_join2, hipEventDisableTiming) != hipSuccess || hipEventCreateWithFlags(&c->ev_fork, hipEventDisableTiming) != hipSuccess || hipEventCreateWithFlags(&c->ev_fork0, hipEventDisableTiming) != hipSuccess || hipEventCreateWithFlags(&c->ev_g2, hipEventDisableTiming) != hipSuccess || hipEventCreateWithFlags(&c->ev_hh, hipEventDisableTiming) != hipSuccess || hipEventCreateWithFlags(&c->ev_gf, hipEventDisableTiming) != hipSuccess ||
      hipEventCreateWithFlags(&c->ev_join, hipEventDisableTiming) != hipSuccess) { delete c; return tsl_fail("side stream / event creation failed"); }
  c->vals.zero(); c->vals_full.zero(); c->scal.zero(); c->part_rz.zero(); c->part_rr.zero();

  c->n_body = d->n_body; c->n_pair = d->n_pair;
  if (d->n_body > 0) c->h_bodies.assign(d->bodies, d->bodies + d->n_body);
  if (d->n_pair > 0) c->h_pairs.assign(d->pairs, d->pairs + d->n_pair);
  if (contact_alloc(c, d)) { delete c; return -1; }
  if (mg_build(c, d)) { delete c; return -1; }
  if (body_dense_setup(c)) { delete c; return -1; }
  (void)hipDeviceSynchronize();
  (void)hipGetDevice(&c->ds.device);
  *out = c;
  return 0;
}

static void group_unregister_and_destroy(tsl_group* G);
extern "C" void tsl_ctx_destroy(tsl_ctx* c) {
  if (!c) return;
  if (c->group) group_unregister_and_destroy(c->group);
  (void)hipDeviceSynchronize();
  ds_flow_token_release(c->ds);
  if (c->h_scal) (void)hipHostFree(c->h_scal);
  if (c->h_scal2) (void)hipHostFree(c->h_scal2);
  for (int i = 0; i < 2; i++) if (c->rb_event[i]) (void)hipEventDestroy(c->rb_event[i]);
  if (c->pcg_graph) (void)hipGraphExecDestroy(c->pcg_graph);
  if (c->mr_graph) (void)hipGraphExecDestroy(c->mr_graph);
  if (c->ev_in) (void)hipEventDestroy(c->ev_in);
  if (c->ev_out) (void)hipEventDestroy(c->ev_out);
  for (int k = 0; k < DS_NSIDE; k++) if (c->ds.fstream[k]) { (void)hipStreamSynchronize(c->ds.fstream[k]); (void)hipEventDestroy(c->ds.ev_fjoin[k]); (void)hipStreamDestroy(c->ds.fstream[k]); }
  if (c->ds.ev_ffork) (void)hipEventDestroy(c->ds.ev_ffork);
  for (int k = 0; k < 5; k++) if (c->ds.ev_la[k]) (void)hipEventDestroy(c->ds.ev_la[k]);
  if (c->ds.lastream) { (void)hipStreamSynchronize(c->ds.lastream); (void)hipStreamDestroy(c->ds.lastream); }
  if (c->ds.h_anorm) (void)hipHostFree(c->ds.h_anorm);
  if (c->ds.pin) (void)hipHostFree(c->ds.pin);
  if (c->h_ir) (void)hipHostFree(c->h_ir);
  if (c->ds.zstream) { (void)hipStreamSynchronize(c->ds.zstream); (void)hipEventDestroy(c->ds.ev_zfork); (void)hipEventDestroy(c->ds.ev_zero); (void)hipStreamDestroy(c->ds.zstream); }
  if (c->ev_fork) (void)hipEventDestroy(c->ev_fork);
  if (c->ev_fork0) (void)hipEventDestroy(c->ev_fork0);
  if (c->ev_g2) (void)hipEventDestroy(c->ev_g2);
  if (c->ev_hh) (void)hipEventDestroy(c->ev_hh);
  if (c->ev_gf) (void)hipEventDestroy(c->ev_gf);
  if (c->ev_join) (void)hipEventDestroy(c->ev_join);
  if (c->side) (void)hipStreamDestroy(c->side);
  if (c->ev_join2) (void)hipEventDestroy(c->ev_join2);
  if (c->side2) (void)hipStreamDestroy(c->side2);
  if (c->stream) (void)hipStreamDestroy(c->stream);
  for (auto& e : c->ev_pool) { (void)hipEventDestroy(e.first); (void)hipEventDestroy(e.second); }
  delete c;
}

extern "C" int tsl_set_stream(tsl_ctx* c, void* s) { c->user_stream = (hipStream_t)s; return 0; }

static int stvk_prepare(tsl_ctx* c) {
  if (c->cf_dminv.n > 0 || c->n_cface == 0) return 0;
  std::vector<double> li(3 * (size_t)c->n_cface), dm(4 * (size_t)c->n_cface);
  HIP_OK(hipMemcpy(li.data(), c->cf_li.p, li.size() * sizeof(double), hipMemcpyDeviceToHost));
  std::vector<int> cid(c->n_cface);
  HIP_OK(hipMemcpy(cid.data(), c->cf_cloth.p, cid.size() * sizeof(int), hipMemcpyDeviceToHost));
  for (int f = 0; f < c->n_cface; f++) {
    const double l0 = li[3 * f], l1 = li[3 * f + 1], l2 = li[3 * f + 2];
    if (!(l0 > 0 && l1 > 0 && l2 > 0 && l0 < l1 + l2 && l1 < l2 + l0 && l2 < l0 + l1))
      return tsl_fail("tsl_set_param: StVK membrane: rest lengths (%g, %g, %g) of face %d (cloth %d, face %d of the cloth) violate the triangle inequality", l0, l1, l2, f,
                      cid[f], f - c->h_cloth[cid[f]].face_start);
    const double a = (l0 * l0 + l2 * l2 - l1 * l1) / (2.0 * l0), b = sqrt(l2 * l2 - a * a);
    dm[4 * f] = 1.0 / l0; dm[4 * f + 1] = -a / (l0 * b); dm[4 * f + 2] = 0.0; dm[4 * f + 3] = 1.0 / b;
  }
  return c->cf_dminv.upload(dm);
}

static int stvk_set(tsl_ctx* c, const char* key, long idx, const std::string& f, double v) {
  const int n_cloth = (int)c->h_cloth.size();
  if (f == "membrane") {
    if (v != 0.0 && v != 1.0) return tsl_fail("tsl_set_param: %s must be 0 or 1 (got %g)", key, v);
    if (v == 1.0) TSL_TRY(stvk_prepare(c));
  }
  if (c->h_stvk.empty()) {
    c->h_stvk.assign(4 * (size_t)n_cloth, 0.0);
    TSL_TRY(c->d_stvk.alloc(c->h_stvk.size()));
  }
  c->h_stvk[4 * idx + (f == "membrane" ? 0 : (f == "stvk_mu" ? 1 : 2))] = v;
  c->n_stvk = 0;
  for (int i = 0; i < n_cloth; i++) c->n_stvk += c->h_stvk[4 * i] != 0.0;
  HIP_OK(hipMemcpy(c->d_stvk.p, c->h_stvk.data(), c->h_stvk.size() * sizeof(double), hipMemcpyHostToDevice));
  return 0;
}

extern "C" int tsl_set_param(tsl_ctx* c, const char* key, double v) {
  Scope scope(c);
  (void)hipStreamSynchronize(c->stream);
  c->mg_omega_valid = false; c->mg_cinv_valid = false;
  c->ds.anorm_valid = false;
  std::string k(key);
  if (k == "mu_cloth_elastic") c->mu_cloth_elastic = v;
  else if (k == "mu_cloth_cloth") c->mu_cloth_cloth = v;
  else if (k == "k_contact") c->k_contact = v;
  else if (k == "eps_contact") c->eps_contact = v;
  else if (k == "eps_v") c->eps_v = v;
  else if (k == "damping") c->damping = v;
  else if (k == "cg_tol") c->cg_tol = v;
  else if (k == "cg_maxit") c->cg_maxit = (int)v;
  else if (k == "newton_cap") c->newton_cap = (int)v;
  else if (k == "plastic") c->plastic = (int)v;
  else if (k == "spd_literal") {
    if (v != 0.0 && v != 1.0) return tsl_fail("tsl_set_param: spd_literal must be 0 or 1 (got %g)", v);
    c->spd_literal = (int)v;
  }
  else if (k == "contact") c->contact_enable = (v != 0.0);
  else if (k == "contact_ee") {
    if (v != 0.0 && v != 1.0) return tsl_fail("tsl_set_param: contact_ee must be 0 or 1 (got %g)", v);
    c->contact_ee = (int)v;
    if (c->contact_ee) TSL_TRY(ee_prepare(c));
  }
  else if (k == "grid_h") c->grid_h = v;
  else if (k == "grid_extent") c->grid_extent = v;
  else if (k == "adj_spd_pc") c->adj_spd_pc = (int)v;
  else if (k == "adj_clamp") c->adj_clamp = v;
  else if (k == "adj_clamp_angleref") c->adj_clamp_angleref = (int)v;
  else if (k == "verbose") c->verbose = (int)v;
  else if (k == "direct") { c->ds.enable = (int)v; c->ds.numeric_valid = false; c->ds.hard = false; }
  else if (k == "direct_berr") c->ds.berr_tol = v;
  else if (k == "direct_small_rounds") { c->ds.small_rounds = std::max(1, (int)v); c->ds.plan_valid = false; c->ds.numeric_valid = false; c->ds.cache.clear(); }
  else if (k == "tet_warm") c->tet_warm = (int)v;
  else if (k == "ds_dbg") c->ds.dbg = (int)v;
  else if (k == "ds_bench_batch") c->ds.bench_batch = (int)v;
  else if (k == "direct_flow") c->ds.flow = std::max(0, (int)v);
  else if (k == "direct_flow_token") { if (v == 0) ds_flow_token_release(c->ds); }
  else if (k == "direct_gemv_wide_below") c->ds.gemv_wide_below = std::max(0, (int)v);
  else if (k == "direct_g32_below") c->ds.g32_below = std::max(0, (int)v);
  else if (k == "direct_lookahead") c->ds.lookahead = (int)v;
  else if (k == "direct_piv_tol") { c->ds.piv_tol = v; c->ds.numeric_valid = false; }
  else if (k == "direct_leaf") { c->ds.leaf = std::max(4, (int)v); c->ds.static_ready = false; c->ds.plan_valid = false; c->ds.numeric_valid = false; }
  else if (k == "gmres_m") c->gmres_m = (int)v;
  else if (k == "body_inv") { c->bd_enable = (int)v; c->bd_valid = false; }
  else if (k == "mg") c->mg_enable = (int)v;
  else if (k.rfind("self_contact", 0) == 0 && k.size() > 12) {
    char* endp = nullptr;
    const long b = strtol(k.c_str() + 12, &endp, 10);
    if (*endp != 0 || b < 0 || b >= c->n_body) return tsl_fail("tsl_set_param: bad body index in %s", key);
    if ((long)c->self_contact.size() < c->n_body) c->self_contact.assign(c->n_body, 0);
    c->self_contact[b] = (v != 0.0);
  }
  else if (k == "mg_coarse_exact") c->mg_coarse_exact = (int)v;
  else if (k == "mg_dense_nodes") { c->mg_dense_auto = v < 0; if (v >= 0) c->mg_dense_nodes = (int)v; c->mg_ops_valid = false; }
  else if ((k.rfind("cloth", 0) == 0 || k.rfind("elastic", 0) == 0) && k.find('.') != std::string::npos) {
    const bool is_cloth = k[0] == 'c';
    const size_t p0 = is_cloth ? 5 : 7, dot = k.find('.');
    char* endp = nullptr;
    const long idx = strtol(k.c_str() + p0, &endp, 10);
    if (endp != k.c_str() + dot || dot == p0) return tsl_fail("tsl_set_param: bad index in %s", key);
    const std::string f = k.substr(dot + 1);
    if (is_cloth) {
      if (idx < 0 || idx >= (long)c->h_cloth.size()) return tsl_fail("tsl_set_param: bad cloth index in %s", key);
      ClothDev& cd = c->h_cloth[idx];
      if (f == "membrane" || f == "stvk_mu" || f == "stvk_lam") return stvk_set(c, key, idx, f, v);
      if (f == "Kb") cd.Kb = v; else if (f == "Kl") cd.Kl = v; else if (f == "Ka") cd.Ka = v; else if (f == "k_angle") cd.k_angle = v;
      else return tsl_fail("tsl_set_param: unknown key %s", key);
      HIP_OK(hipMemcpy(c->d_cloth.p, c->h_cloth.data(), c->h_cloth.size() * sizeof(ClothDev), hipMemcpyHostToDevice));
    } else {
      if (idx < 0 || idx >= (long)c->h_el.size()) return tsl_fail("tsl_set_param: bad elastic index in %s", key);
      ElasticDev& ed = c->h_el[idx];
      if (f == "mu") ed.mu = v; else if (f == "lam") ed.lam = v; else if (f == "alpha") ed.alpha = v;
      else return tsl_fail("tsl_set_param: unknown key %s", key);
      HIP_OK(hipMemcpy(c->d_el.p, c->h_el.data(), c->h_el.size() * sizeof(ElasticDev), hipMemcpyHostToDevice));
      c->bd_valid = false;
    }
  } else return tsl_fail("tsl_set_param: unknown key %s", key);
  return 0;
}

extern "C" int tsl_set_frozen(tsl_ctx* c, const int32_t* fr) {
  Scope scope(c);
  (void)hipStreamSynchronize(c->stream);
  c->h_frozen.assign(fr, fr + 3 * (size_t)c->NV);
  c->mg_omega_valid = false; c->mg_cinv_valid = false;
  TSL_TRY(upload_frozen(c));
  if (c->pcg_graph) { (void)hipGraphExecDestroy(c->pcg_graph); c->pcg_graph = nullptr; }
  if (c->mr_graph) { (void)hipGraphExecDestroy(c->mr_graph); c->mr_graph = nullptr; }
  return body_dense_setup(c);
}
extern "C" int tsl_set_ext_force(tsl_ctx* c, const double* f) {
  Scope scope(c);
  (void)hipStreamSynchronize(c->stream);
  HIP_OK(hipMemcpy(c->fext.p, f, 3 * (size_t)c->NV * sizeof(double), hipMemcpyHostToDevice));
  return 0;
}
extern "C" int tsl_set_gravity(tsl_ctx* c, const double* g) {
  Scope scope(c);
  (void)hipStreamSynchronize(c->stream);
  HIP_OK(hipMemcpy(c->grav.p, g, 3 * (size_t)c->NV * sizeof(double), hipMemcpyHostToDevice));
  return 0;
}

template <bool STVK>
TSL_DEV void energy_body(VertArgs VA, ClothArgs CA, TetArgs TA, const double* __restrict__ pos, const double* __restrict__ prev,
                         const double* __restrict__ vel, const double* __restrict__ ref_angle, double* __restrict__ e_part, StvkArgs S) {
  const int t = blockIdx.x * blockDim.x + threadIdx.x;
  double e = 0;
  if (t < VA.NV) e += vert_energy(VA, t, pos, prev, vel);
  if (t < CA.n_cface) {
    int v[3]; d3 P[3];
    load_face(pos, CA.f2v, t, v, P);
    const double li[3] = {CA.li[3 * t], CA.li[3 * t + 1], CA.li[3 * t + 2]};
    if constexpr (STVK) e += cface_energy_sel(CA.cloth[CA.cid[t]], S.stvk + 4 * CA.cid[t], S.dminv + 4 * t, P, CA.V[t], li);
    else e += cface_energy(CA.cloth[CA.cid[t]], P, CA.V[t], li);
  }
  if (t < CA.n_hinge) e += hinge_energy(CA, t, pos, ref_angle);
  if (t < TA.n_tet) e += tet_energy(TA, t, pos);
  e = wave_sum(e);
  __shared__ double sw[4];
  if ((threadIdx.x & 63) == 0) sw[threadIdx.x >> 6] = e;
  __syncthreads();
  if (threadIdx.x == 0) e_part[blockIdx.x] = ((sw[0] + sw[1]) + sw[2]) + sw[3];
}
__global__ void k_energy(VertArgs VA, ClothArgs CA, TetArgs TA, const double* __restrict__ pos, const double* __restrict__ prev,
                         const double* __restrict__ vel, const double* __restrict__ ref_angle, double* __restrict__ e_part) {
  energy_body<false>(VA, CA, TA, pos, prev, vel, ref_angle, e_part, StvkArgs{nullptr, nullptr});
}
__global__ void k_energy_stvk(VertArgs VA, ClothArgs CA, TetArgs TA, const double* __restrict__ pos, const double* __restrict__ prev,
                              const double* __restrict__ vel, const double* __restrict__ ref_angle, double* __restrict__ e_part, StvkArgs S) {
  energy_body<true>(VA, CA, TA, pos, prev, vel, ref_angle, e_part, S);
}
__global__ void __launch_bounds__(256) k_energy_final(int n, const double* __restrict__ part, double* __restrict__ e_out) {
  __shared__ double sh[256];
  double a = 0.0;
  for (int i = threadIdx.x; i < n; i += 256) a += part[i];
  sh[threadIdx.x] = a;
  __syncthreads();
  for (int o = 128; o > 0; o >>= 1) { if ((int)threadIdx.x < o) sh[threadIdx.x] += sh[threadIdx.x + o]; __syncthreads(); }
  if (threadIdx.x == 0) *e_out = sh[0];
}

static CgScal* SC(tsl_ctx* c) { return (CgScal*)c->scal.p; }
static CgScal* HSC(tsl_ctx* c) { return (CgScal*)c->h_scal; }

static int energy_async(tsl_ctx* c, const double* pos, const double* prev, const double* vel, const double* ref) {
  hipStream_t s = c->stream;
  if (c->n_cface) hipLaunchKernelGGL(k_cloth_normals, dim3(nblk(c->n_cface, 256)), dim3(256), 0, s, c->n_cface, pos, c->cf_f2v.p, c->norm_dir.p);
  const int nmax = std::max(std::max(c->NV, c->n_cface), std::max(c->n_hinge, c->n_tet));
  const int nvf = c->nc - c->nc_ee;
  const int nb1 = nblk(nmax, 256), nb2 = nvf > 0 ? nblk(nvf, 64) : 0, nb3 = c->nc_ee > 0 ? nblk(c->nc_ee, 64) : 0;
  if (c->e_part.n < (size_t)nb1 + (size_t)nblk(c->max_n_constraints, 64) + 1) { if (c->e_part.alloc((size_t)nb1 + (size_t)nblk(c->max_n_constraints, 64) + 1)) return -1; }
  if (c->n_stvk > 0) hipLaunchKernelGGL(k_energy_stvk, dim3(nb1), dim3(256), 0, s, vert_args(c), cloth_args(c), tet_args(c), pos, prev, vel, ref, c->e_part.p, stvk_args(c));
  else hipLaunchKernelGGL(k_energy, dim3(nb1), dim3(256), 0, s, vert_args(c), cloth_args(c), tet_args(c), pos, prev, vel, ref, c->e_part.p);
  if (nb2 > 0) hipLaunchKernelGGL(k_contact_energy, dim3(nb2), dim3(64), 0, s, nvf, contact_args(c), pos, c->e_part.p + nb1);
  if (nb3 > 0) hipLaunchKernelGGL(k_ee_energy, dim3(nb3), dim3(64), 0, s, c->nc_ee, ee_args(contact_args(c), nvf), pos, c->e_part.p + nb1 + nb2);
  hipLaunchKernelGGL(k_energy_final, dim3(1), dim3(256), 0, s, nb1 + nb2 + nb3, (const double*)c->e_part.p, &SC(c)->energy);
  return 0;
}
static int energy_sync(tsl_ctx* c, const double* pos, const double* prev, const double* vel, const double* ref, double* E) {
  TSL_TRY(energy_async(c, pos, prev, vel, ref));
  HIP_OK(hipMemcpyAsync(&HSC(c)->energy, &SC(c)->energy, sizeof(double), hipMemcpyDeviceToHost, c->stream));
  HIP_OK(hipStreamSynchronize(c->stream));
  *E = HSC(c)->energy;
  return 0;
}

extern "C" int tsl_energy(tsl_ctx* c, const double* pos, const double* prev, const double* vel, const double* ref, double* E) {
  Scope scope(c);
  return energy_sync(c, pos, prev, vel, ref, E);
}

__global__ void k_vertex_gather(int NV, const int* __restrict__ vg_ptr, const int* __restrict__ vg_idx, const double* __restrict__ stage, int lo, int hi, double* __restrict__ F) {
  const int v = blockIdx.x * blockDim.x + threadIdx.x;
  if (v >= NV) return;
  d3 a = ld3(F, v);
  for (int e = vg_ptr[v]; e < vg_ptr[v + 1]; e++) { const int i = vg_idx[e]; if (i >= lo && i < hi) a = a + ld3(stage, i); }
  st3(F, v, a);
}
__global__ void __launch_bounds__(256) k_contact_row_gather(int NV, const int* __restrict__ rowpos, const int* __restrict__ cr_ptr, const int* __restrict__ cr_ent,
                                                            const double* __restrict__ cg, double* __restrict__ F) {
  const int v = (int)((blockIdx.x * (size_t)blockDim.x + threadIdx.x) >> 6), lane = threadIdx.x & 63;
  if (v >= NV) return;
  const int p = rowpos[v];
  const int r0 = cr_ptr[p], r1 = cr_ptr[p + 1];
  if (r1 <= r0) return;
  double a0 = 0, a1 = 0, a2 = 0;
  for (int e = r0 + lane; e < r1; e += 64) {
    const int q = cr_ent[e];
    const double* g = cg + 12 * (size_t)(q >> 2) + 3 * (q & 3);
    a0 += g[0]; a1 += g[1]; a2 += g[2];
  }
  a0 = wave_sum(a0); a1 = wave_sum(a1); a2 = wave_sum(a2);
  if (lane == 0) st3(F, v, ld3(F, v) + d3(a0, a1, a2));
}

static void cloth_grad_face_launch(tsl_ctx* c, hipStream_t s, const ClothArgs& CA, const double* pos) {
  if (c->n_stvk > 0) hipLaunchKernelGGL(k_cloth_grad_face<true>, dim3(nblk(c->n_cface, 256)), dim3(256), 0, s, CA, pos, stvk_args(c));
  else hipLaunchKernelGGL(k_cloth_grad_face<false>, dim3(nblk(c->n_cface, 256)), dim3(256), 0, s, CA, pos, stvk_args(c));
}
static void cloth_hess_face_launch(tsl_ctx* c, hipStream_t s, const ClothArgs& CA, const double* pos, const double* ref, int spd) {
  const dim3 g(nblk(c->n_cface, 128)), b(128);
  const StvkArgs S = stvk_args(c);
  const bool lit = c->spd_literal && spd == 1;
  if (c->n_stvk > 0) {
    if (spd == 2) hipLaunchKernelGGL((k_cloth_hess_face<true, false, true>), g, b, 0, s, CA, pos, ref, c->quirk.p, spd, c->cg_frec.p, S);
    else if (lit) hipLaunchKernelGGL((k_cloth_hess_face<false, true, true>), g, b, 0, s, CA, pos, ref, c->quirk.p, spd, c->cg_frec.p, S);
    else hipLaunchKernelGGL((k_cloth_hess_face<false, false, true>), g, b, 0, s, CA, pos, ref, c->quirk.p, spd, c->cg_frec.p, S);
  } else {
    if (spd == 2) hipLaunchKernelGGL((k_cloth_hess_face<true>), g, b, 0, s, CA, pos, ref, c->quirk.p, spd, c->cg_frec.p, S);
    else if (lit) hipLaunchKernelGGL((k_cloth_hess_face<false, true>), g, b, 0, s, CA, pos, ref, c->quirk.p, spd, c->cg_frec.p, S);
    else hipLaunchKernelGGL((k_cloth_hess_face<false>), g, b, 0, s, CA, pos, ref, c->quirk.p, spd, c->cg_frec.p, S);
  }
}

static int assemble_enqueue_early(tsl_ctx* c, const double* pos, const double* prev, const double* vel, const double* ref, int spd, double* grad, int tet_warm_flag);
static int assemble_enqueue(tsl_ctx* c, const double* pos, const double* prev, const double* vel, const double* ref, int spd, double* grad, int tet_warm_flag) {
  hipStream_t s = c->stream;
  const int NV = c->NV;
  if (c->nc > 0 || c->n_tet > 0) return assemble_enqueue_early(c, pos, prev, vel, ref, spd, grad, tet_warm_flag);
  HIP_OK(hipMemsetAsync(c->vals_full.p, 0, c->vals_full.n * sizeof(double), s));
  if (c->n_cface) hipLaunchKernelGGL(k_cloth_normals, dim3(nblk(c->n_cface, 256)), dim3(256), 0, s, c->n_cface, pos, c->cf_f2v.p, c->norm_dir.p);
  ClothArgs CA = cloth_args(c);
  const VertArgs VA = vert_args(c);
  CA.gstage = c->vg_stage.p;
  if (grad) {
    HIP_OK(hipMemsetAsync(grad, 0, 3 * (size_t)NV * sizeof(double), s));
    hipLaunchKernelGGL(k_vert_grad, dim3(nblk(NV, 256)), dim3(256), 0, s, VA, pos, prev, vel, grad);
  }
  hipLaunchKernelGGL(k_vert_hess, dim3(nblk(NV, 256)), dim3(256), 0, s, VA, c->diag_blk.p, c->vals_full.p);
  if (grad) {
    if (c->n_cface) cloth_grad_face_launch(c, s, CA, pos);
    if (c->n_hinge) hipLaunchKernelGGL(k_cloth_grad_hinge, dim3(nblk(c->n_hinge, 256)), dim3(256), 0, s, CA, pos, ref);
  }
  if (c->n_cface) {
    const int nq = (int)c->h_cloth.size() * 9;
    hipLaunchKernelGGL(k_cloth_quirk, dim3(nblk(nq, 64)), dim3(64), 0, s, CA, (int)c->h_cloth.size(), pos, ref, c->quirk.p);
    cloth_hess_face_launch(c, s, CA, pos, ref, spd);
  }
  if (c->n_hinge) hipLaunchKernelGGL(k_cloth_hess_hinge, dim3(nblk(c->n_hinge, 256)), dim3(256), 0, s, CA, pos, c->cg_hrec.p);
  if (c->n_cgblk_cloth > 0)
    hipLaunchKernelGGL(k_cloth_gather, dim3(nblk(c->n_cgblk_cloth, CG_BPW)), dim3(256), 0, s, c->n_cgblk_cloth, c->cg_base.p, c->cg_ptr.p, (const unsigned*)c->cg_ent.p, c->n_hinge, c->n_cface,
                       (const double*)c->cg_hrec.p, (const double*)c->cg_frec.p, (const double*)c->cg_trec.p, c->vals_full.p);
  if (grad) {
    hipLaunchKernelGGL(k_vertex_gather, dim3(nblk(NV, 256)), dim3(256), 0, s, NV, (const int*)c->vg_ptr.p, (const int*)c->vg_idx.p, (const double*)c->vg_stage.p, 0, c->vg_ns, grad);
    hipLaunchKernelGGL(k_mask_vec, dim3(gsz(3 * (size_t)NV)), dim3(256), 0, s, 3 * (size_t)NV, c->frozen.p, grad);
  }
  hipLaunchKernelGGL(k_mask_matrix, dim3(c->n_slices), dim3(256), 0, s, c->n_slices, c->slice_off.p, c->slice_len.p, c->colidx.p, c->fzmask.p, c->mdt2.p,
                     c->vals_full.p, c->vals.p, NV);
  if (!c->pc_frozen) {
    if (direct_takes_solve(c)) c->dinv_valid = false;
    else TSL_TRY(block_jacobi_refresh(c));
  }
  HIP_OK(hipGetLastError());
  return 0;
}

static int assemble_enqueue_early(tsl_ctx* c, const double* pos, const double* prev, const double* vel, const double* ref, int spd, double* grad, int tet_warm_flag) {
  hipStream_t s = c->stream, st = c->side;
  const bool fork_t = c->n_tet > 0 && c->nc > 0;
  hipStream_t stt = fork_t ? c->side2 : st;
  const int NV = c->NV;
  ClothArgs CA = cloth_args(c);
  const VertArgs VA = vert_args(c);
  TetArgs TA = tet_args(c);
  CA.gstage = c->vg_stage.p; TA.gstage = c->vg_stage.p + 3 * (size_t)c->vg_tet0;
  HIP_OK(hipEventRecord(c->ev_fork0, s));
  HIP_OK(hipStreamWaitEvent(st, c->ev_fork0, 0));
  if (fork_t) HIP_OK(hipStreamWaitEvent(stt, c->ev_fork0, 0));
  TSL_TRY(contact_assemble(c, pos, spd, grad, st));
  const bool gather = c->n_cgblk > 0;
  const bool hh_side = fork_t && gather;
  if (hh_side && c->n_hinge) {
    hipLaunchKernelGGL(k_cloth_hess_hinge, dim3(nblk(c->n_hinge, 256)), dim3(256), 0, stt, CA, pos, c->cg_hrec.p);
    HIP_OK(hipEventRecord(c->ev_hh, stt));
  }
  if (c->n_tet) {
    if (grad) { hipLaunchKernelGGL(k_tet_grad, dim3(nblk(c->n_tet, 256)), dim3(256), 0, stt, TA, pos); HIP_OK(hipEventRecord(c->ev_g2, stt)); }
    const bool lit = c->spd_literal && spd == 1;
    double* vws = (c->tet_warm && spd != 0 && !lit) ? c->tet_V.p : (double*)nullptr;
    if (lit) hipLaunchKernelGGL(k_tet_hess_coop<true>, dim3(nblk(c->n_tet, 16)), dim3(256), 0, stt, TA, pos, spd, vws, 0, c->cg_trec.p);
    else hipLaunchKernelGGL(k_tet_hess_coop<false>, dim3(nblk(c->n_tet, 16)), dim3(256), 0, stt, TA, pos, spd, vws, vws ? tet_warm_flag : 0, c->cg_trec.p);
  }
  HIP_OK(hipMemsetAsync(c->vals_full.p, 0, c->vals_full.n * sizeof(double), s));
  if (c->n_cface) hipLaunchKernelGGL(k_cloth_normals, dim3(nblk(c->n_cface, 256)), dim3(256), 0, s, c->n_cface, pos, c->cf_f2v.p, c->norm_dir.p);
  if (grad) {
    HIP_OK(hipMemsetAsync(grad, 0, 3 * (size_t)NV * sizeof(double), s));
    hipLaunchKernelGGL(k_vert_grad, dim3(nblk(NV, 256)), dim3(256), 0, s, VA, pos, prev, vel, grad);
  }
  hipLaunchKernelGGL(k_vert_hess, dim3(nblk(NV, 256)), dim3(256), 0, s, VA, c->diag_blk.p, c->vals_full.p);
  HIP_OK(hipEventRecord(c->ev_fork, s));
  if (c->n_cface) {
    const int nq = (int)c->h_cloth.size() * 9;
    hipLaunchKernelGGL(k_cloth_quirk, dim3(nblk(nq, 64)), dim3(64), 0, s, CA, (int)c->h_cloth.size(), pos, ref, c->quirk.p);
    cloth_hess_face_launch(c, s, CA, pos, ref, spd);
  }
  HIP_OK(hipStreamWaitEvent(stt, c->ev_fork, 0));
  if (c->n_hinge && !hh_side) hipLaunchKernelGGL(k_cloth_hess_hinge, dim3(nblk(c->n_hinge, 256)), dim3(256), 0, s, CA, pos, c->cg_hrec.p);
  const int nt_blk = c->n_cgblk - c->n_cgblk_cloth;
  if (c->n_tet && nt_blk > 0)
    hipLaunchKernelGGL(k_cloth_gather, dim3(nblk(nt_blk, CG_BPW)), dim3(256), 0, stt, nt_blk, c->cg_base.p + c->n_cgblk_cloth, c->cg_ptr.p + c->n_cgblk_cloth, (const unsigned*)c->cg_ent.p,
                       c->n_hinge, c->n_cface, (const double*)c->cg_hrec.p, (const double*)c->cg_frec.p, (const double*)c->cg_trec.p, c->vals_full.p);
  HIP_OK(hipEventRecord(c->ev_join2, stt));
  if (grad) {
    if (fork_t) HIP_OK(hipStreamWaitEvent(st, c->ev_fork, 0));
    if (c->n_hinge) hipLaunchKernelGGL(k_cloth_grad_hinge, dim3(nblk(c->n_hinge, 256)), dim3(256), 0, st, CA, pos, ref);
    if (c->n_cface) {
      cloth_grad_face_launch(c, hh_side ? stt : st, CA, pos);
      if (hh_side) HIP_OK(hipEventRecord(c->ev_gf, stt));
    }
  }
  if (hh_side && c->n_hinge) HIP_OK(hipStreamWaitEvent(s, c->ev_hh, 0));
  if (gather && c->n_cgblk_cloth > 0)
    hipLaunchKernelGGL(k_cloth_gather, dim3(nblk(c->n_cgblk_cloth, CG_BPW)), dim3(256), 0, s, c->n_cgblk_cloth, c->cg_base.p, c->cg_ptr.p, (const unsigned*)c->cg_ent.p, c->n_hinge, c->n_cface,
                       (const double*)c->cg_hrec.p, (const double*)c->cg_frec.p, (const double*)c->cg_trec.p, c->vals_full.p);
  HIP_OK(hipStreamWaitEvent(s, c->ev_join2, 0));
  hipLaunchKernelGGL(k_mask_matrix, dim3(c->n_slices), dim3(256), 0, s, c->n_slices, c->slice_off.p, c->slice_len.p, c->colidx.p, c->fzmask.p, c->mdt2.p,
                     c->vals_full.p, c->vals.p, NV);
  if (grad) {
    if (fork_t && c->n_tet) HIP_OK(hipStreamWaitEvent(st, c->ev_g2, 0));
    if (hh_side && c->n_cface) HIP_OK(hipStreamWaitEvent(st, c->ev_gf, 0));
    hipLaunchKernelGGL(k_vertex_gather, dim3(nblk(NV, 256)), dim3(256), 0, st, NV, (const int*)c->vg_ptr.p, (const int*)c->vg_idx.p, (const double*)c->vg_stage.p, 0, c->vg_ns, grad);
    if (c->nc > 0) hipLaunchKernelGGL(k_contact_row_gather, dim3(nblk((long)NV * 64, 256)), dim3(256), 0, st, NV, (const int*)c->rowpos.p, (const int*)c->cr_ptr.p, (const int*)c->cr_ent.p,
                                      (const double*)c->c_G.p, grad);
    hipLaunchKernelGGL(k_mask_vec, dim3(gsz(3 * (size_t)NV)), dim3(256), 0, st, 3 * (size_t)NV, c->frozen.p, grad);
  }
  HIP_OK(hipEventRecord(c->ev_join, st));
  HIP_OK(hipStreamWaitEvent(s, c->ev_join, 0));
  if (!c->pc_frozen) {
    if (direct_takes_solve(c)) c->dinv_valid = false;
    else TSL_TRY(block_jacobi_refresh(c));
  }
  HIP_OK(hipGetLastError());
  return 0;
}

static int assemble(tsl_ctx* c, const double* pos, const double* prev, const double* vel, const double* ref, int spd, double* grad) {
  hipStream_t s = c->stream;
  if (c->vg_stage.n < 3 * (size_t)std::max(c->vg_ns, 1)) { if (c->vg_stage.alloc(3 * (size_t)std::max(c->vg_ns, 1))) return tsl_fail("out of device memory (gradient staging)"); }
  if (c->n_tet > 0 && c->cg_trec.n < 144 * (size_t)c->n_tet) { if (c->cg_trec.alloc(144 * (size_t)c->n_tet)) return tsl_fail("out of device memory (element records)"); }
  if (grad && c->nc > 0 && c->c_G.n < 12 * (size_t)c->max_n_constraints) { if (c->c_G.alloc(12 * (size_t)c->max_n_constraints)) return -1; }
  if (c->n_cgblk > 0 && c->n_cface > 0 && c->cg_frec.n == 0) {
    if (c->cg_hrec.alloc((size_t)std::max(c->n_hinge, 1) * 16) | c->cg_frec.alloc((size_t)c->n_cface * 81)) return tsl_fail("out of device memory (cloth element records)");
  }
  int warm = 0;
  if (c->n_tet > 0 && c->tet_warm && spd != 0 && !(c->spd_literal && spd == 1)) {
    if (c->tet_V.n < (size_t)81 * c->n_tet) {
      if (c->tet_V.alloc((size_t)81 * c->n_tet)) return tsl_fail("out of device memory (tet eigenvectors)");
      HIP_OK(hipMemsetAsync(c->tet_V.p, 0, c->tet_V.n * sizeof(double), s));
      c->tet_V_count = 0;
    }
    warm = (c->tet_V_count++ % 16) != 0;
  }
  c->st_pos = pos; c->st_prev = prev; c->st_vel = vel; c->st_ref = ref;
  c->ds.numeric_valid = false;
  if (spd != c->ds.anorm_spd) { c->ds.anorm_valid = false; c->ds.anorm_spd = spd; }
  if (!c->pc_frozen) { c->mg_ops_valid = false; c->pc_separate = false; }
  return assemble_enqueue(c, pos, prev, vel, ref, spd, grad, warm);
}

extern "C" int tsl_assemble(tsl_ctx* c, const double* pos, const double* prev, const double* vel, const double* ref, int spd, double* grad) {
  Scope scope(c);
  c->bd_valid = false;
  c->mg_omega_valid = false; c->mg_cinv_valid = false;
  c->ds.anorm_valid = false;
  return assemble(c, pos, prev, vel, ref, spd, grad);
}

static ContactRows contact_rows(tsl_ctx* c, const double* blocks) {
  ContactRows R;
  R.ptr = c->nc > 0 ? c->cr_ptr.p : (const int*)nullptr;
  R.ent = c->cr_ent.p; R.rows = c->cr_rows.p; R.H = blocks; R.nv = c->NV;
  return R;
}

static void launch_spmv(tsl_ctx* c, const double* vals, const double* x, double* y, int slot, int check_flag, bool full_contact = false) {
  hipStream_t s = c->stream;
  if (slot < 0 && !check_flag) {
    hipLaunchKernelGGL((k_spmv_mw<4, 1, TSL_NT>), dim3(c->n_slices), dim3(256), 0, s, c->NV, c->n_slices, c->slice_off.p, c->slice_len.p, c->colidx.p, vals, x, y,
                       (double*)nullptr, (const int*)nullptr, contact_rows(c, full_contact ? c->c_Hfull.p : c->c_H.p));
    return;
  }
  const bool sample = c->prof_enable && slot >= 0 && (c->prof_launches % 16 == 0) && c->ev_used < c->ev_pool.size();
  if (sample) (void)hipEventRecord(c->ev_pool[c->ev_used].first, s);
  unsigned long long* dprof = nullptr;
  if (c->prof_enable && slot >= 0 && (c->prof_launches % 64 == 40) && c->prof_dev_used < c->prof_dev_cap) dprof = c->prof_dev.p + 2 * c->prof_waves * (c->prof_dev_used++);
  hipLaunchKernelGGL(k_spmv, dim3(nblk((long)c->n_slices * 64, 256)), dim3(256), 0, s, c->NV, c->n_slices, c->slice_off.p, c->slice_len.p, c->colidx.p, vals, x, y,
                     SC(c), slot, check_flag, dprof);
  if (sample) { (void)hipEventRecord(c->ev_pool[c->ev_used].second, s); c->ev_used++; }
  if (slot >= 0) c->prof_launches++;
  if (c->nc > 0)
    hipLaunchKernelGGL(k_contact_matvec, dim3(nblk(c->nc, 64)), dim3(CONTACT_MV_THREADS), 0, s, c->nc, c->c_idx.p, c->rowpos.p, full_contact ? c->c_Hfull.p : c->c_H.p, x, y, SC(c), slot,
                       check_flag);
}

static void prof_collect(tsl_ctx* c) {
  for (size_t i = 0; i < c->ev_used; i++) {
    float ms = 0;
    if (hipEventElapsedTime(&ms, c->ev_pool[i].first, c->ev_pool[i].second) == hipSuccess) { c->prof_ms += ms; c->prof_samples++; }
  }
  c->ev_used = 0;
}

static int read_scal(tsl_ctx* c) {
  HIP_OK(hipMemcpyAsync(c->h_scal, c->scal.p, sizeof(CgScal), hipMemcpyDeviceToHost, c->stream));
  HIP_OK(hipStreamSynchronize(c->stream));
  if (c->prof_enable) prof_collect(c);
  return 0;
}

static int bicgstab(tsl_ctx* c, tsl_solve_stats* st);
static int gmres(tsl_ctx* c, tsl_solve_stats* st, bool direct = false);
static int direct_refine(tsl_ctx* c, tsl_solve_stats* st, bool first_done = false);
static int solve_perm(tsl_ctx* c, tsl_solve_stats* st, const tsl_solve_stats* first = nullptr);
static bool direct_takes_solve(tsl_ctx* c) {
  const DirectSolver& d = c->ds;
  return direct_enabled(c) && !c->ds_suspended && !(d.enable < 0 && !d.hard && c->n_tet == 0 && c->nc == 0);
}
static int block_jacobi_refresh(tsl_ctx* c) {
  if (c->nc > 0 && !c->cdiag_valid) contact_diag_refresh(c, c->stream);
  hipLaunchKernelGGL(k_block_jacobi, dim3(nblk(c->NV, 256)), dim3(256), 0, c->stream, c->NV, c->diag_perm.p, c->vals.p, c->nc > 0 ? c->c_diag.p : (const double*)nullptr, c->Dinv.p);
  if (body_active(c) && c->bd_valid) body_zero_dinv(c);
  c->dinv_valid = true;
  return 0;
}
static int block_jacobi_ensure(tsl_ctx* c) { return c->dinv_valid ? 0 : block_jacobi_refresh(c); }

static int minres(tsl_ctx* c, tsl_solve_stats* st);

static int body_dense_setup(tsl_ctx* c) {
  BodyDenseArgs& A = c->bd_args;
  A = BodyDenseArgs{};
  c->bd_valid = false; c->bd_rows_n = 0; c->bd_n3max = 0; c->bd_wg = 0; c->bd_scr_n = 0; c->bd_w_total = 0;
  std::vector<int> rows, body_of(c->NV, -1), local_of(c->NV, 0);
  for (const ElasticDev& e : c->h_el) {
    if (A.nb >= TSL_MAX_DENSE_BODIES || e.n_verts > 512 || e.n_verts < 2) continue;
    bool any_free = false;
    for (int v = e.v_offset; v < e.v_offset + e.n_verts && !any_free; v++)
      any_free = !(c->h_frozen[3 * v] && c->h_frozen[3 * v + 1] && c->h_frozen[3 * v + 2]);
    if (!any_free) continue;
    const int b = A.nb++;
    A.n3[b] = 3 * e.n_verts;
    A.rows_off[b] = (int)rows.size();
    A.w_off[b] = (long)c->bd_w_total;
    A.scr_off[b] = c->bd_scr_n;
    A.wg_off[b] = c->bd_wg;
    for (int k = 0; k < e.n_verts; k++) {
      const int v = e.v_offset + k;
      rows.push_back(c->h_rowpos[v]); body_of[v] = b; local_of[v] = k;
    }
    c->bd_w_total += (size_t)A.n3[b] * ((A.n3[b] + 3) & ~3);
    c->bd_scr_n += A.n3[b];
    c->bd_wg += (A.n3[b] + BODY_APPLY_ROWS - 1) / BODY_APPLY_ROWS;
    c->bd_n3max = std::max(c->bd_n3max, A.n3[b]);
  }
  A.wg_off[A.nb] = c->bd_wg;
  c->bd_rows_n = (int)rows.size();
  if (!A.nb) return 0;
  TSL_TRY(c->bd_rows.upload(rows)); TSL_TRY(c->bd_body_of.upload(body_of)); TSL_TRY(c->bd_local_of.upload(local_of));
  if (c->bd_bad.alloc(TSL_MAX_DENSE_BODIES) | c->bd_W.alloc(c->bd_w_total) | c->bd_Binv.alloc(c->bd_w_total) | c->bd_scr.alloc(4 * (size_t)c->bd_scr_n) | c->bd_rb.alloc(2 * (size_t)c->bd_scr_n)) return -1;
  A.rows = c->bd_rows.p; A.body_of = c->bd_body_of.p; A.local_of = c->bd_local_of.p;
  HIP_OK(hipMemsetAsync(c->bd_Binv.p, 0, c->bd_w_total * sizeof(float), c->stream));
  return 0;
}

static bool body_active(tsl_ctx* c) {
  if (c->bd_args.nb <= 0 || c->bd_enable == 0) return false;
  return c->bd_enable > 0 || (!c->mg.empty() && c->mg_enable != 0);
}

static void body_zero_dinv(tsl_ctx* c) {
  hipLaunchKernelGGL(k_body_zero_dinv, dim3(nblk(c->bd_rows_n, 256)), dim3(256), 0, c->stream, c->bd_args, c->bd_rows_n, c->Dinv.p);
}

static int body_build_inverse(tsl_ctx* c) {
  hipStream_t s = c->stream;
  const BodyDenseArgs& A = c->bd_args;
  HIP_OK(hipMemsetAsync(c->bd_W.p, 0, c->bd_w_total * sizeof(double), s));
  HIP_OK(hipMemsetAsync(c->bd_bad.p, 0, TSL_MAX_DENSE_BODIES * sizeof(int), s));
  for (int b = 0; b < A.nb; b++)
    hipLaunchKernelGGL(k_body_gather, dim3(A.n3[b] / 3), dim3(64), 0, s, A, b, c->slice_off.p, c->slice_len.p, c->colidx.p, c->perm.p, c->vals.p, c->bd_W.p);
  if (c->nc > 0) hipLaunchKernelGGL(k_body_contact, dim3(nblk(c->nc, 64)), dim3(64), 0, s, A, c->nc, c->c_idx.p, c->c_H.p, c->bd_W.p);
  double* col[2] = {c->bd_scr.p, c->bd_scr.p + 2 * (size_t)c->bd_scr_n};
  double* row[2] = {c->bd_scr.p + c->bd_scr_n, c->bd_scr.p + 3 * (size_t)c->bd_scr_n};
  hipLaunchKernelGGL(k_body_gj_init, dim3(nblk(c->bd_n3max, 256), A.nb), dim3(256), 0, s, A, c->bd_W.p, col[0], row[0]);
  const dim3 grid(nblk((long)c->bd_n3max * c->bd_n3max, 256), A.nb);
  for (int k = 0; k < c->bd_n3max; k++)
    hipLaunchKernelGGL(k_body_gj, grid, dim3(256), 0, s, A, k, c->bd_W.p, col[k & 1], row[k & 1], col[(k & 1) ^ 1], row[(k & 1) ^ 1], c->bd_bad.p);
  hipLaunchKernelGGL(k_body_finalize, grid, dim3(256), 0, s, A, c->bd_W.p, c->bd_bad.p, c->Dinv.p, c->bd_Binv.p);
  body_zero_dinv(c);
  c->bd_valid = true;
  HIP_OK(hipGetLastError());
  return 0;
}

static void body_apply(tsl_ctx* c, int mode, const double* r, const double* t, double* z, const double* rdot, double* part) {
  hipLaunchKernelGGL(k_body_apply, dim3(c->bd_wg), dim3(256), 0, c->stream, c->bd_args, c->bd_Binv.p, mode, r, t, z, rdot, part);
}

static int mg_build(tsl_ctx* c, const tsl_scene_desc* d) {
  for (int ci = 0; ci < d->n_cloth; ci++) {
    const tsl_cloth_desc& cd = d->cloths[ci];
    int N = cd.N, M = cd.M;
    if (N < 8 || M < 8 || (N & 1) || (M & 1)) continue;
    MgCloth* mc = new MgCloth();
    mc->v_offset = cd.v_offset; mc->N0 = N; mc->M0 = M;
    while (!(N & 1) && !(M & 1) && std::min(N, M) >= 4) {
      N >>= 1; M >>= 1;
      MgLevel* L = new MgLevel();
      L->N = N; L->M = M; L->n = (N + 1) * (M + 1);
      int rc = L->A.alloc((size_t)225 * L->n) | L->Dinv.alloc((size_t)9 * L->n) | L->x.alloc((size_t)3 * L->n) | L->x2.alloc((size_t)3 * L->n) | L->r.alloc((size_t)3 * L->n) | L->t.alloc((size_t)3 * L->n) | L->omega.alloc(2);
      mc->lv.push_back(L);
      if (rc) { delete mc; return -1; }
    }
    for (size_t l = 0; l + 1 < mc->lv.size(); l++)
      if (mc->lv[l]->S.alloc((size_t)441 * mc->lv[l + 1]->n)) { delete mc; return -1; }
    c->mg.push_back(mc);
  }
  if (!c->mg.empty()) {
// ... 1111 lines not shown
  const int nvf = c->nc - c->nc_ee;
  const char* supported = "cloth<i>.Kl|Ka|Kb|stvk_mu|stvk_lam, elastic<i>.mu|lam, k_contact, mu_cloth_elastic, mu_cloth_cloth";
  std::vector<std::array<int, 2>> kr(n_keys);
  bool need[5] = {false, false, false, false, false};
  for (int j = 0; j < n_keys; j++) {
    if (!keys[j]) return tsl_fail("tsl_param_grad_keys: key %d is null", j);
    const std::string k(keys[j]);
    int cls = -1, row = -1;
    if (k == "k_contact") { cls = 3; row = 0; }
    else if (k == "mu_cloth_elastic") { cls = 3; row = 1; }
    else if (k == "mu_cloth_cloth") { cls = 3; row = 2; }
    else if ((k.rfind("cloth", 0) == 0 || k.rfind("elastic", 0) == 0) && k.find('.') != std::string::npos) {
      const bool is_cloth = k[0] == 'c';
      const size_t p0 = is_cloth ? 5 : 7, dot = k.find('.');
      char* endp = nullptr;
      const long idx = strtol(k.c_str() + p0, &endp, 10);
      const char c0 = k[p0];
      if (endp != k.c_str() + dot || dot == p0 || !(isdigit((unsigned char)c0) || c0 == '-')) return tsl_fail("tsl_param_grad_keys: bad index in %s", keys[j]);
      const std::string f = k.substr(dot + 1);
      if (is_cloth) {
        if (f == "Kl" || f == "Ka") { cls = 0; row = f == "Kl" ? 0 : 1; }
        else if (f == "Kb") { cls = 1; row = 0; }
        else if (f == "stvk_mu" || f == "stvk_lam") { cls = 4; row = f == "stvk_mu" ? 0 : 1; }
        if (cls >= 0 && (idx < 0 || idx >= n_cloth)) return tsl_fail("tsl_param_grad_keys: bad cloth index in %s (%d cloths)", keys[j], n_cloth);
        if (cls == 0 || cls == 4) row += 2 * (int)idx; else if (cls == 1) row = (int)idx;
      } else {
        if (f == "mu" || f == "lam") { cls = 2; row = f == "mu" ? 0 : 1; }
        if (cls >= 0 && (idx < 0 || idx >= n_el)) return tsl_fail("tsl_param_grad_keys: bad elastic index in %s (%d bodies)", keys[j], n_el);
        if (cls == 2) row += 2 * (int)idx;
      }
    }
    if (cls < 0) return tsl_fail("tsl_param_grad_keys: %s is not a differentiated key (supported: %s)", keys[j], supported);
    if (cls == 3) {
      if (row == 0 && c->nc_ee > 0)
        return tsl_fail("tsl_param_grad_keys: k_contact: %d edge-edge constraints (contact_ee = 1) are present; their friction derivative is not implemented", c->nc_ee);
      const double live = row == 0 ? c->k_contact : (row == 1 ? c->mu_cloth_elastic : c->mu_cloth_cloth);
      bool used = row == 0;
      for (const auto& pr : c->h_pairs) used |= pr.mu_is_param == row;
      if (live == 0.0 && used && nvf > 0)
        return tsl_fail("tsl_param_grad_keys: %s = 0: the friction weights c_k of the detection vanish with it, their derivative is not available", keys[j]);
    }
    if (cls == 1 && !ref) return tsl_fail("tsl_param_grad_keys: %s needs ref_angle", keys[j]);
    kr[j] = {cls, row};
    need[cls] = true;
  }
  const int rows[5] = {2 * n_cloth, n_cloth, 2 * n_el, 3, 2 * n_cloth};
  const int nb[5] = {c->n_cface > 0 ? nblk(c->n_cface, PG_THREADS) : 0, c->n_hinge > 0 ? nblk(c->n_hinge, PG_THREADS) : 0, c->n_tet > 0 ? nblk(c->n_tet, PG_THREADS) : 0,
                     nvf > 0 ? nblk(nvf, PG_THREADS) : 0, c->n_cface > 0 && c->n_stvk > 0 ? nblk(c->n_cface, PG_THREADS) : 0};
  size_t off[5], tot = 0;
  for (int q = 0; q < 5; q++) { off[q] = tot; if (need[q]) tot += (size_t)rows[q] * nb[q]; }
  if (tot > (size_t)INT32_MAX) return tsl_fail("tsl_param_grad_keys: too many partials");
  if (c->pg_part.n < std::max<size_t>(tot, 1)) TSL_TRY(c->pg_part.alloc(std::max<size_t>(tot, 1)));
  if (c->pg_out.n < (size_t)n_keys + 2) TSL_TRY(c->pg_out.alloc((size_t)n_keys + 2));
  const double* p = p_dev ? p_dev : c->pdir.p;
  const int* fz = c->frozen.p;
  double* part = c->pg_part.p;
  if (need[0] && nb[0]) {
    if (c->n_stvk > 0) hipLaunchKernelGGL(k_pg_face<true>, dim3(nb[0]), dim3(PG_THREADS), 0, s, cloth_args(c), n_cloth, pos, p, fz, part + off[0], stvk_args(c));
    else hipLaunchKernelGGL(k_pg_face<false>, dim3(nb[0]), dim3(PG_THREADS), 0, s, cloth_args(c), n_cloth, pos, p, fz, part + off[0], stvk_args(c));
  }
  if (need[4] && nb[4]) hipLaunchKernelGGL(k_pg_stvk, dim3(nb[4]), dim3(PG_THREADS), 0, s, cloth_args(c), n_cloth, pos, p, fz, part + off[4], stvk_args(c));
  if (need[1] && nb[1]) hipLaunchKernelGGL(k_pg_hinge, dim3(nb[1]), dim3(PG_THREADS), 0, s, cloth_args(c), n_cloth, pos, ref, p, fz, part + off[1]);
  if (need[2] && nb[2]) hipLaunchKernelGGL(k_pg_tet, dim3(nb[2]), dim3(PG_THREADS), 0, s, tet_args(c), n_el, pos, p, fz, part + off[2]);
  if (need[3] && nb[3])
    hipLaunchKernelGGL(k_pg_contact, dim3(nb[3]), dim3(PG_THREADS), 0, s, nvf, contact_args(c), (const int*)c->c_kind.p, c->mu_cloth_elastic, c->mu_cloth_cloth, pos, p, fz,
                       part + off[3]);
  const int n_ee = need[3] ? c->nc_ee : 0;
  for (int j0 = 0; j0 < n_keys; j0 += PG_KEYS_PER_LAUNCH) {
    PgTable tab;
    tab.n = std::min(PG_KEYS_PER_LAUNCH, n_keys - j0);
    for (int j = 0; j < tab.n; j++) {
      const int q = kr[j0 + j][0];
      tab.off[j] = (int)(off[q] + (size_t)kr[j0 + j][1] * nb[q]);
      tab.cnt[j] = nb[q];
    }
    hipLaunchKernelGGL(k_pg_final, dim3(1), dim3(PG_THREADS), 0, s, tab, (const double*)part, j0 == 0 ? n_ee : 0,
                       n_ee > 0 ? (const int*)c->c_kind.p + nvf : (const int*)nullptr, c->pg_out.p + j0, j0 == 0 ? c->pg_out.p + n_keys : (double*)nullptr);
  }
  HIP_OK(hipGetLastError());
  std::vector<double> h((size_t)n_keys + 2);
  HIP_OK(hipMemcpyAsync(h.data(), c->pg_out.p, h.size() * sizeof(double), hipMemcpyDeviceToHost, s));
  HIP_OK(hipStreamSynchronize(s));
  for (int j = 0; j < n_keys; j++) {
    if (kr[j][0] != 3 || kr[j][1] == 0) continue;
    const double n_kind = h[n_keys + kr[j][1] - 1];
    if (n_kind > 0)
      return tsl_fail("tsl_param_grad_keys: %s: %d edge-edge constraints (contact_ee = 1) use it; their friction derivative is not implemented", keys[j], (int)n_kind);
  }
  for (int j = 0; j < n_keys; j++) out_host[j] = h[j];
  return 0;
}

extern "C" int tsl_update_ref_angle(tsl_ctx* c, const double* pos, double* ref) {
  Scope scope(c);
  if (!c->n_hinge) return 0;
  hipStream_t s = c->stream;
  hipLaunchKernelGGL(k_cloth_normals, dim3(nblk(c->n_cface, 256)), dim3(256), 0, s, c->n_cface, pos, c->cf_f2v.p, c->norm_dir.p);
  hipLaunchKernelGGL(k_cloth_update_ref, dim3(nblk(c->n_hinge, 256)), dim3(256), 0, s, cloth_args(c), pos, ref);
  HIP_OK(hipGetLastError());
  return 0;
}

struct StepMember { tsl_ctx* c; double *pos, *prev, *vel, *ref; };
using StepSolve = std::function<int(const std::vector<int>& act, std::vector<tsl_solve_stats>& ss, const std::function<void(int)>& lap)>;

static void add_solve_stats(tsl_step_stats& t, const tsl_solve_stats& s) {
  t.cg_iters += s.iters; t.solves++; t.restarts += s.restarts; t.fallback += (s.flag == 1); t.unconverged += (s.flag == 3); t.attained += s.attained;
  t.max_rel_residual = std::max(t.max_rel_residual, s.rel_residual); t.max_backward_error = std::max(t.max_backward_error, s.backward_error);
}

static int newton_step(const std::vector<StepMember>& m, GroupPool* pool, tsl_ctx* g, const StepSolve& solve, tsl_step_stats* stats) {
  const int n = (int)m.size();
  struct InStep { const std::vector<StepMember>& m; ~InStep() { for (const StepMember& e : m) { e.c->in_step = false; e.c->st_pos = nullptr; } } } guard{m};
  std::vector<tsl_step_stats> st(n);
  std::vector<long> fact0(n), plans0(n);
  std::vector<int> iter(n, 0), active(n, 1);
  std::vector<double> delta(n, 1e5), E0(n, 0.0), E(n, 0.0), alpha(n, 1.0);
  for (int i = 0; i < n; i++) {
    tsl_ctx* c = m[i].c;
    memset(&st[i], 0, sizeof(tsl_step_stats));
    fact0[i] = c->ds.n_factor; plans0[i] = c->ds.n_plans;
    c->in_step = true; c->warm_valid = false; c->mg_omega_valid = false; c->mg_cinv_valid = false; c->tm_loop = 0;
    if (c->mg_dense_auto) {
      const double it = c->last_step_iters_per_solve;
      const int cur = c->mg_dense_nodes;
      const double to_900 = cur >= 900 ? 120.0 : 200.0, to_256 = cur >= 256 ? 36.0 : 60.0;
      c->mg_dense_nodes = it > to_900 ? 900 : it > to_256 ? 256 : 64;
    }
    if (c->ds.hard && ++c->ds.hard_steps > c->ds.probe_every) c->ds.hard = false;
    c->bd_valid = false;
    HIP_OK(hipMemcpyAsync(m[i].prev, m[i].pos, 3 * (size_t)c->NV * sizeof(double), hipMemcpyDeviceToDevice, c->stream));
  }
  for (int i = 0; i < n; i++) {
    tsl_ctx* c = m[i].c;
    int nc = 0;
    if (c->contact_enable) TSL_TRY(tsl_contact_detect(c, m[i].pos, m[i].prev, &nc));
    else { c->nc = 0; c->nc_ee = 0; c->ds.cons_checked = false; }
    st[i].nc = nc;
  }
  const long gfact0 = g ? g->ds.n_factor : 0;
  const bool timed = m[0].c->verbose >= 1;
  double tph[7] = {0, 0, 0, 0, 0, 0, 0};
  auto tick = std::chrono::steady_clock::now();
  const std::function<void(int)> lap = [&](int k) { if (!timed) return; for (const StepMember& e : m) (void)hipStreamSynchronize(e.c->stream); if (g) (void)hipStreamSynchronize(g->stream);
                                                     const auto nw = std::chrono::steady_clock::now(); if (k >= 0) tph[k] += std::chrono::duration<double>(nw - tick).count(); tick = nw; };
  auto energy_issue = [&](int i) -> int {
    tsl_ctx* c = m[i].c;
    TSL_TRY(energy_async(c, m[i].pos, m[i].prev, m[i].vel, m[i].ref));
    HIP_OK(hipMemcpyAsync(&HSC(c)->energy, &SC(c)->energy, sizeof(double), hipMemcpyDeviceToHost, c->stream));
    return 0;
  };
  const std::function<int(int)> assemble_one = [&](int i) -> int {
    tsl_ctx* c = m[i].c;
    TSL_TRY(assemble(c, m[i].pos, m[i].prev, m[i].vel, m[i].ref, 1, c->F.p));
    hipLaunchKernelGGL(k_gather_perm, dim3(nblk(c->NV, 256)), dim3(256), 0, c->stream, c->NV, c->perm.p, (const double*)c->F.p, c->v_b.p);
    return 0;
  };
  std::vector<tsl_solve_stats> ss(n);
  lap(-1);
  for (;;) {
    std::vector<int> act;
    for (int i = 0; i < n; i++) if (active[i] && iter[i] < m[i].c->newton_cap) act.push_back(i);
    if (act.empty()) break;
    for (int i : act) if (++iter[i] == 1) TSL_TRY(energy_issue(i));
    for (int i : act) { if (iter[i] == 1) { HIP_OK(hipStreamSynchronize(m[i].c->stream)); E0[i] = HSC(m[i].c)->energy; } else E0[i] = E[i]; }
    lap(0);
    if (pool) TSL_TRY(pool->run(act, assemble_one));
    else for (int i : act) TSL_TRY(assemble_one(i));
    lap(1);
    TSL_TRY(solve(act, ss, lap));
    lap(5);
    for (int i : act) {
      tsl_ctx* c = m[i].c;
      const size_t n3 = 3 * (size_t)c->NV;
      hipStream_t s = c->stream;
      add_solve_stats(st[i], ss[i]);
      const bool have_pmax = ss[i].method == 4 && ss[i].flag == 0 && c->last_xmax_valid;
      if (have_pmax) HSC(c)->pmax = c->last_xmax;
      else {
        HIP_OK(hipMemsetAsync(&SC(c)->pmax, 0, sizeof(double), s));
        hipLaunchKernelGGL(k_absmax, dim3(gsz(n3)), dim3(256), 0, s, n3, c->pdir.p, &SC(c)->pmax);
        HIP_OK(hipMemcpyAsync(&HSC(c)->pmax, &SC(c)->pmax, sizeof(double), hipMemcpyDeviceToHost, s));
      }
      HIP_OK(hipMemcpyAsync(c->x1.p, m[i].pos, n3 * sizeof(double), hipMemcpyDeviceToDevice, s));
      alpha[i] = 1.0;
    }
    std::vector<int> pend = act;
    while (!pend.empty()) {
      for (int i : pend) {
        tsl_ctx* c = m[i].c;
        const size_t n3 = 3 * (size_t)c->NV;
        hipLaunchKernelGGL(k_linesearch, dim3(gsz(n3)), dim3(256), 0, c->stream, n3, c->x1.p, c->pdir.p, alpha[i], m[i].pos);
        TSL_TRY(energy_issue(i));
      }
      std::vector<int> again;
      for (int i : pend) {
        HIP_OK(hipStreamSynchronize(m[i].c->stream));
        E[i] = HSC(m[i].c)->energy;
        st[i].ls_evals++;
        if (E[i] < E0[i]) continue;
        alpha[i] /= 2;
        if (alpha[i] > 1e-8) again.push_back(i);
      }
      pend.swap(again);
    }
    for (int i : act) {
      tsl_ctx* c = m[i].c;
      delta[i] = HSC(c)->pmax / c->dt;
      st[i].last_alpha = alpha[i]; st[i].energy = E[i];
      if (c->verbose >= 4) fprintf(stderr, "[tsl]   scene %d newton %2d: E0 %.12e  E - E0 %+.3e  alpha %.3g  |p|max %.3e  delta %.3e  (solve: %d its, rel_residual %.1e)\n", i, iter[i], E0[i], E[i] - E0[i], alpha[i],
                                   HSC(c)->pmax, delta[i], ss[i].iters, ss[i].rel_residual);
      if (delta[i] < 1e-7) active[i] = 0;
    }
    lap(6);
  }
  if (timed) {
    long its = 0;
    double loops = 0;
    for (int i = 0; i < n; i++) { its += st[i].cg_iters; loops += m[i].c->tm_loop; }
    fprintf(stderr, "[tsl] step of %d scene(s): %d Newton iterations (most of a scene), %ld solver iterations; energy %.3f s, assembly + preconditioner set-up %.3f s, solves %.3f s "
            "(merged plans + merge %.3f s, factorisation %.3f s, application %.3f s; iteration loops %.3f s), line search %.3f s\n",
            n, *std::max_element(iter.begin(), iter.end()), its, tph[0], tph[1], tph[2] + tph[3] + tph[4] + tph[5], tph[2], tph[3], tph[4], loops, tph[6]);
  }
  for (int i = 0; i < n; i++) {
    tsl_ctx* c = m[i].c;
    const size_t n3 = 3 * (size_t)c->NV;
    st[i].newton_iters = iter[i]; st[i].last_delta = delta[i];
    st[i].factorizations = (int)(c->ds.n_factor - fact0[i]) + (g && i == 0 ? (int)(g->ds.n_factor - gfact0) : 0); st[i].plans = (int)(c->ds.n_plans - plans0[i]);
    hipLaunchKernelGGL(k_update_vel, dim3(gsz(n3)), dim3(256), 0, c->stream, n3, m[i].pos, m[i].prev, c->damping / c->dt, m[i].vel);
    if (c->plastic) TSL_TRY(tsl_update_ref_angle(c, m[i].pos, m[i].ref));
  }
  for (int i = 0; i < n; i++) {
    tsl_ctx* c = m[i].c;
    HIP_OK(hipStreamSynchronize(c->stream));
    if (st[i].solves > 0) c->last_step_iters_per_solve = (double)st[i].cg_iters / st[i].solves;
    if (stats) stats[i] = st[i];
  }
  if (g) HIP_OK(hipStreamSynchronize(g->stream));
  HIP_OK(hipGetLastError());
  return 0;
}

extern "C" int tsl_step(tsl_ctx* c, double* pos, double* prev, double* vel, double* ref, tsl_step_stats* stats) {
  Scope scope(c);
  const StepSolve solve = [c](const std::vector<int>&, std::vector<tsl_solve_stats>& ss, const std::function<void(int)>&) -> int {
    TSL_TRY(solve_perm(c, &ss[0]));
    hipLaunchKernelGGL(k_scatter_perm, dim3(nblk(c->NV, 256)), dim3(256), 0, c->stream, c->NV, c->perm.p, (const double*)c->v_x.p, c->pdir.p);
    HIP_OK(hipGetLastError());
    if (ss[0].method == 4) TSL_TRY(direct_prezero(c));
    return 0;
  };
  return newton_step({StepMember{c, pos, prev, vel, ref}}, nullptr, nullptr, solve, stats);
}

static std::mutex g_group_mu;
static std::vector<tsl_group*> g_groups;
static void group_unregister_and_destroy(tsl_group* G) {
  { std::lock_guard<std::mutex> lk(g_group_mu);
    auto it = std::find(g_groups.begin(), g_groups.end(), G);
    if (it == g_groups.end()) return;
    g_groups.erase(it); }
  group_destroy(G);
}
extern "C" int tsl_group_create(tsl_ctx* const* ctxs, int32_t n, tsl_group** out) {
  for (int i = 0; i < n; i++) if (!direct_enabled(ctxs[i])) return tsl_fail("tsl_group_create: scene %d does not use the sparse direct solve (\"direct\" = 1 or a cloth grid of >= 1024 cells)", i);
  TSL_TRY(group_create(ctxs, n, out));
  std::lock_guard<std::mutex> lk(g_group_mu);
  g_groups.push_back(*out);
  return 0;
}
extern "C" void tsl_group_destroy(tsl_group* G) { if (G) group_unregister_and_destroy(G); }
extern "C" int tsl_group_info(tsl_group* G, double* out9) {
  out9[0] = (double)G->n_merge; out9[1] = (double)G->n_relayout; out9[2] = G->t_merge; out9[3] = 8.0 * (double)(G->arena.n + G->sarena.n + G->garena.n + G->w.n);
  out9[4] = (double)G->g->ds.n_factor; out9[5] = (double)G->g->ds.n_apply; out9[6] = (double)G->n_own_path;
  out9[7] = (double)G->g->ds.n_flow; out9[8] = (double)G->g->ds.n_flow_abort;
  return 0;
}

static int group_solve(tsl_group* G, const std::vector<int>& act, std::vector<tsl_solve_stats>& ss, const std::function<void(int)>& lap) {
  const int n = (int)G->m.size();
  tsl_ctx* g = G->g;
  {
    std::vector<int> todo;
    for (int i = 0; i < n; i++) { tsl_ctx* c = G->m[i]; if (!(c->ds.plan_valid && c->ds.cons_checked)) todo.push_back(i); }
    if (todo.size() > 1) TSL_TRY(G->pool->run(todo, [&](int i) -> int { return direct_plan(G->m[i]); }));
    for (int i = 0; i < n; i++) TSL_TRY(direct_plan(G->m[i]));
  }
  bool stale = !G->merged_valid;
  for (int i = 0; i < n; i++) stale |= G->seen_gen[i] != G->m[i]->ds.plan_gen;
  if (stale) {
    for (int i = 0; i < n; i++) HIP_OK(hipStreamSynchronize(G->m[i]->stream));
    TSL_TRY(group_merge(G));
  }
  lap(2);
  {
    DirectSolver& gd = g->ds;
    const DirectSolver& d0 = G->m[0]->ds;
    for (int i = 1; i < n; i++) {
      const DirectSolver& di = G->m[i]->ds;
      if (di.piv_tol != d0.piv_tol || di.flow != d0.flow || di.g32_below != d0.g32_below || di.gemv_wide_below != d0.gemv_wide_below || di.small_rounds != d0.small_rounds)
        return tsl_fail("scene group: members 0 and %d differ in a parameter of the factorisation (direct_piv_tol / _flow / _g32_below / _gemv_wide_below / _small_rounds)", i);
    }
    if (gd.piv_tol != d0.piv_tol) gd.piv_tol = d0.piv_tol;
    gd.flow = G->flow_lost ? 0 : d0.flow; gd.g32_below = d0.g32_below; gd.gemv_wide_below = d0.gemv_wide_below; gd.small_rounds = d0.small_rounds * n; gd.xcd_map = d0.xcd_map;
    gd.prezero = d0.prezero; gd.dbg = d0.dbg;
  }
  ss.assign(n, tsl_solve_stats{});
  std::vector<char> okv(n, 1);
  for (int attempt = 0; attempt < 2; attempt++) {
    DirectSolver& gd = g->ds;
    for (int i = 0; i < n; i++) { HIP_OK(hipEventRecord(G->ev_m[i], G->m[i]->stream)); HIP_OK(hipStreamWaitEvent(g->stream, G->ev_m[i], 0)); }
    gd.numeric_valid = false;
    if (attempt > 0) {
      gd.have_factor = false;
      if (gd.prezero_pending) { HIP_OK(hipStreamWaitEvent(g->stream, gd.ev_zero, 0)); gd.prezero_pending = false; }
    }
    TSL_TRY(direct_factor(g));
    if (attempt == 0) for (int i = 0; i < n; i++) { DirectSolver& d = G->m[i]->ds; if (++d.anorm_age >= 64) d.anorm_valid = false; }
    lap(3);
    TSL_TRY(direct_apply(g, G->vb.p, G->vx.p));
    HIP_OK(hipEventRecord(G->ev_g, g->stream));
    lap(4);
    for (int i = 0; i < n; i++) HIP_OK(hipStreamWaitEvent(G->m[i]->stream, G->ev_g, 0));
    for (int i : act) TSL_TRY(ir_pass_enqueue(G->m[i]));
    bool any_bad = false;
    for (int i : act) {
      tsl_ctx* c = G->m[i];
      HIP_OK(hipStreamSynchronize(c->stream));
      ss[i] = tsl_solve_stats{};
      const int ok = ir_pass_verdict(c, &ss[i], true);
      if (ok < 0) return -1;
      okv[i] = (char)ok;
      any_bad |= !ok;
    }
    if (attempt == 0) {
      int note[8];
      const int lost = ds_flow_lost(g, any_bad, note);
      if (lost < 0) return -1;
      if (lost) {
        fprintf(stderr, "[tsl] scene group: k_ds_gj_flow of the merged factorisation waited in vain for a flag: \"direct_flow\" disabled for the group, refactorising "
                "(workgroup %d of %d gave up; flag value %d, epoch %d)\n", note[2], note[1], note[3], note[4]);
        gd.flow = 0; gd.n_flow_abort++; G->flow_lost = true;
        continue;
      }
    }
    break;
  }
  for (int i : act) {
    tsl_ctx* c = G->m[i];
    tsl_solve_stats& s1 = ss[i];
    if (okv[i]) { s1.flag = 0; s1.method = 4; continue; }
    c->ds.numeric_valid = true; c->ds.have_factor = true;
    const tsl_solve_stats first = s1;
    TSL_TRY(solve_perm(c, &s1, &first));
    G->n_own_path++;
    if (c->verbose >= 2) fprintf(stderr, "[tsl] scene group: member %d went on from the merged pass (rel_residual %.2e) on its own path: flag %d after %d applications\n", i, first.rel_residual, s1.flag, s1.iters);
  }
  for (int i = 0; i < n; i++) { tsl_ctx* c = G->m[i]; c->ds.numeric_valid = false; c->ds.have_factor = false; HIP_OK(hipEventRecord(G->ev_m[i], c->stream)); HIP_OK(hipStreamWaitEvent(g->stream, G->ev_m[i], 0)); }
  TSL_TRY(direct_prezero(g));
  lap(5);
  return 0;
}

extern "C" int tsl_group_step(tsl_group* G, double* const* pos_a, double* const* prev_a, double* const* vel_a, double* const* ref_a, tsl_step_stats* stats) {
  const int n = (int)G->m.size();
  std::vector<std::unique_ptr<Scope>> scopes;
  for (int i = 0; i < n; i++) scopes.emplace_back(new Scope(G->m[i]));
  std::vector<StepMember> m(n);
  for (int i = 0; i < n; i++) {
    if (!direct_enabled(G->m[i])) return tsl_fail("tsl_group_step: scene %d does not use the sparse direct solve", i);
    m[i] = StepMember{G->m[i], pos_a[i], prev_a[i], vel_a[i], ref_a[i]};
  }
  G->g->verbose = G->m[0]->verbose;
  const StepSolve solve = [G](const std::vector<int>& act, std::vector<tsl_solve_stats>& ss, const std::function<void(int)>& lap) -> int {
    TSL_TRY(group_solve(G, act, ss, lap));
    for (int i : act) {
      tsl_ctx* c = G->m[i];
      hipLaunchKernelGGL(k_scatter_perm, dim3(nblk(c->NV, 256)), dim3(256), 0, c->stream, c->NV, c->perm.p, (const double*)c->v_x.p, c->pdir.p);
    }
    return 0;
  };
  return newton_step(m, G->pool.get(), G->g, solve, stats);
}

extern "C" int tsl_matrix_nnzb(tsl_ctx* c, int32_t* nb, int32_t* nnzb) {
  *nb = c->NV; *nnzb = (int32_t)c->nnzb;
  return 0;
}

extern "C" int tsl_matrix_export(tsl_ctx* c, int32_t* row_ptr, int32_t* col, double* vals) {
  Scope scope(c);
  HIP_OK(hipStreamSynchronize(c->stream));
  std::vector<double> hv(c->vals.n);
  HIP_OK(hipMemcpy(hv.data(), c->vals.p, hv.size() * sizeof(double), hipMemcpyDeviceToHost));
  long k = 0;
  row_ptr[0] = 0;
  for (int v = 0; v < c->NV; v++) {
    const auto& r = c->h_rows[v];
    const int p = c->h_rowpos[v], s = p >> 6, lane = p & 63;
    for (size_t j = 0; j < r.size(); j++, k++) {
      col[k] = r[j];
      const size_t base = ((size_t)c->h_slice_off[s] + 64 * j) * 9 + lane;
      for (int e = 0; e < 9; e++) vals[9 * k + e] = hv[base + 64 * e];
    }
    row_ptr[v + 1] = (int32_t)k;
  }
  return 0;
}

extern "C" int tsl_matrix_import(tsl_ctx* c, const double* vals) {
  Scope scope(c);
  HIP_OK(hipStreamSynchronize(c->stream));
  std::vector<double> hv(c->vals.n);
  HIP_OK(hipMemcpy(hv.data(), c->vals.p, hv.size() * sizeof(double), hipMemcpyDeviceToHost));
  long k = 0;
  for (int v = 0; v < c->NV; v++) {
    const int p = c->h_rowpos[v], s = p >> 6, lane = p & 63;
    for (size_t j = 0; j < c->h_rows[v].size(); j++, k++) {
      const size_t base = ((size_t)c->h_slice_off[s] + 64 * j) * 9 + lane;
      for (int e = 0; e < 9; e++) hv[base + 64 * e] = vals[9 * k + e];
    }
  }
  HIP_OK(hipMemcpy(c->vals.p, hv.data(), hv.size() * sizeof(double), hipMemcpyHostToDevice));
  c->ds.numeric_valid = false; c->ds.anorm_valid = false;
  c->mg_ops_valid = false; c->pc_separate = false;
  c->bd_valid = false; c->mg_omega_valid = false; c->mg_cinv_valid = false;
  return 0;
}

extern "C" int tsl_profile_reset(tsl_ctx* c, int enable) {
  c->prof_enable = enable; c->prof_ms = 0; c->prof_chunks = 0; c->ev_sample_next = false; c->prof_launches = 0; c->prof_samples = 0; c->ev_used = 0; c->prof_dev_used = 0; c->prof_dev_ticks = 0; c->prof_dev_n = 0;
  if (enable) {
    c->prof_waves = (size_t)c->n_slices * PCG_WPS;
    c->prof_dev_cap = 1;
    if (c->prof_dev.n == 0) TSL_TRY(c->prof_dev.alloc(2 * c->prof_waves * (size_t)c->prof_dev_cap));
    HIP_OK(hipMemset(c->prof_dev.p, 0, c->prof_dev.n * sizeof(unsigned long long)));
  }
  if (enable && c->ev_pool.empty()) {
    for (int i = 0; i < 64; i++) {
      hipEvent_t a, b;
      HIP_OK(hipEventCreate(&a)); HIP_OK(hipEventCreate(&b));
      c->ev_pool.push_back({a, b});
    }
  }
  return 0;
}

extern "C" int tsl_profile_read(tsl_ctx* c, double* ms_per_launch, int64_t* launches, int64_t* bytes_per_launch) {
  Scope scope(c);
  HIP_OK(hipStreamSynchronize(c->stream));
  prof_collect(c);
  double dev_ms = 0;
  long n_dev = c->prof_dev_n;
  {
    int dev = 0, khz = 100000;
    (void)hipGetDevice(&dev);
    if (hipDeviceGetAttribute(&khz, hipDeviceAttributeWallClockRate, dev) != hipSuccess || khz <= 0) khz = 100000;
    dev_ms = c->prof_dev_ticks / (double)khz;
  }
  c->prof_event_ms = c->prof_samples ? c->prof_ms / c->prof_samples : 0.0;
  *ms_per_launch = n_dev ? dev_ms / n_dev : c->prof_event_ms;
  *launches = c->prof_launches;
  *bytes_per_launch = (int64_t)c->nnzb * 76 + (int64_t)c->NV * (24 + 24);
  return 0;
}

extern "C" int tsl_profile_read_events(tsl_ctx* c, double* ms_per_launch_events) {
  *ms_per_launch_events = c->prof_event_ms;
  return 0;
}

extern "C" int tsl_bench_spmv(tsl_ctx* c, int variant, int reps, double* us_per_launch) {
  Scope scope(c);
  hipStream_t s = c->stream;
  hipEvent_t e0, e1;
  HIP_OK(hipEventCreate(&e0)); HIP_OK(hipEventCreate(&e1));
  const int ns = c->n_slices;
  if (c->v_t4.n < (size_t)ns) return tsl_fail("scratch too small");
  int k1_count = 0;
  const int variant30_grid = std::min<long>(std::max<long>((long)c->v_t4.n, 1), 2048);
  auto launch = [&]() {
    switch (variant) {
      case 0: hipLaunchKernelGGL(k_spmv, dim3(nblk((long)ns * 64, 256)), dim3(256), 0, s, c->NV, ns, c->slice_off.p, c->slice_len.p, c->colidx.p, c->vals.p, c->v_p.p, c->v_Ap.p, SC(c), 0, 0, (unsigned long long*)nullptr); break;
      case 1: hipLaunchKernelGGL((k_spmv_mw<1, 4, false>), dim3(nblk(ns, 4)), dim3(256), 0, s, c->NV, ns, c->slice_off.p, c->slice_len.p, c->colidx.p, c->vals.p, c->v_p.p, c->v_Ap.p, c->v_t4.p, (const int*)nullptr, ContactRows{}); break;
      case 2: hipLaunchKernelGGL((k_spmv_mw<4, 1, false>), dim3(ns), dim3(256), 0, s, c->NV, ns, c->slice_off.p, c->slice_len.p, c->colidx.p, c->vals.p, c->v_p.p, c->v_Ap.p, c->v_t4.p, (const int*)nullptr, ContactRows{}); break;
      case 3: hipLaunchKernelGGL((k_spmv_mw<4, 1, true>), dim3(ns), dim3(256), 0, s, c->NV, ns, c->slice_off.p, c->slice_len.p, c->colidx.p, c->vals.p, c->v_p.p, c->v_Ap.p, c->v_t4.p, (const int*)nullptr, ContactRows{}); break;
      case 4: hipLaunchKernelGGL((k_spmv_mw<2, 2, false>), dim3(nblk(ns, 2)), dim3(256), 0, s, c->NV, ns, c->slice_off.p, c->slice_len.p, c->colidx.p, c->vals.p, c->v_p.p, c->v_Ap.p, c->v_t4.p, (const int*)nullptr, ContactRows{}); break;
      case 5: hipLaunchKernelGGL((k_spmv_mw<8, 1, false>), dim3(ns), dim3(512), 0, s, c->NV, ns, c->slice_off.p, c->slice_len.p, c->colidx.p, c->vals.p, c->v_p.p, c->v_Ap.p, c->v_t4.p, (const int*)nullptr, ContactRows{}); break;
      case 6: hipLaunchKernelGGL((k_spmv_mw<4, 2, false>), dim3(nblk(ns, 2)), dim3(512), 0, s, c->NV, ns, c->slice_off.p, c->slice_len.p, c->colidx.p, c->vals.p, c->v_p.p, c->v_Ap.p, c->v_t4.p, (const int*)nullptr, ContactRows{}); break;
      case 7: hipLaunchKernelGGL((k_spmv_mw<2, 2, true>), dim3(nblk(ns, 2)), dim3(256), 0, s, c->NV, ns, c->slice_off.p, c->slice_len.p, c->colidx.p, c->vals.p, c->v_p.p, c->v_Ap.p, c->v_t4.p, (const int*)nullptr, ContactRows{}); break;
      case 10: hipLaunchKernelGGL(k_spmv, dim3(nblk((long)ns * 64, 256)), dim3(256), 0, s, c->NV, ns, c->slice_off.p, c->slice_len.p, c->colidx.p, c->vals.p, c->v_p.p, c->v_Ap.p, SC(c), 0, 1, (unsigned long long*)nullptr); break;
      case 11: hipLaunchKernelGGL(k_spmv, dim3(nblk((long)ns * 64, 256)), dim3(256), 0, s, c->NV, ns, c->slice_off.p, c->slice_len.p, c->colidx.p, c->vals.p, c->v_p.p, c->v_Ap.p, SC(c), -1, 0, (unsigned long long*)nullptr); break;
      case 12: {
        hipLaunchKernelGGL(k_spmv, dim3(nblk((long)ns * 64, 256)), dim3(256), 0, s, c->NV, ns, c->slice_off.p, c->slice_len.p, c->colidx.p, c->vals.p, c->v_p.p, c->v_Ap.p, SC(c), 0, 1, (unsigned long long*)nullptr);
        hipLaunchKernelGGL(k_cg_update, dim3(nblk(c->NV, 256)), dim3(256), 0, s, c->NV, c->v_p.p, c->v_Ap.p, c->Dinv.p, c->v_x.p, c->v_r.p, c->v_z.p, SC(c), 0);
        hipLaunchKernelGGL(k_cg_p, dim3(nblk(c->NV, 256)), dim3(256), 0, s, c->NV, c->v_z.p, c->v_p.p, SC(c), 0, 0);
      } break;
      case 13: hipLaunchKernelGGL(k_cg_update, dim3(nblk(c->NV, 256)), dim3(256), 0, s, c->NV, c->v_p.p, c->v_Ap.p, c->Dinv.p, c->v_x.p, c->v_r.p, c->v_z.p, SC(c), 0); break;
      case 14: hipLaunchKernelGGL(k_cg_p, dim3(nblk(c->NV, 256)), dim3(256), 0, s, c->NV, c->v_z.p, c->v_p.p, SC(c), 0, 0); break;
      case 30: {
        const size_t nw = c->vals.n / 2;
        const int grid = variant30_grid;
        hipLaunchKernelGGL(k_stream_read, dim3(grid), dim3(256), 0, s, (const double2*)c->vals.p, nw, c->v_t4.p);
      } break;
      case 20: {
        const int par = (k1_count++) & 1;
        hipLaunchKernelGGL((k_pcg_spmv<PCG_WPS, TSL_NT>), dim3(ns), dim3(64 * PCG_WPS), 0, s, c->NV, ns, c->slice_off.p, c->slice_len.p, c->colidx.p, c->vals.p, c->v_z.p,
                           par ? c->v_p.p : c->v_t0.p, par ? c->v_t0.p : c->v_p.p, c->v_Ap.p, c->part_rz.p, c->part_rr.p, c->part_pAp.p, PSC(c), par, 0,
                           (unsigned long long*)nullptr, contact_rows(c, c->c_H.p));
      } break;
      default: break;
    }
  };
  if (variant == 20) {
    const size_t n3 = 3 * (size_t)c->NV;
    const int gb = nblk(c->NV, 256);
    std::vector<double> one((size_t)gb, 0.0);
    one[0] = 1.0;
    HIP_OK(hipMemcpyAsync(c->part_rz.p, one.data(), one.size() * sizeof(double), hipMemcpyHostToDevice, s));
    HIP_OK(hipMemcpyAsync(c->part_rr.p, one.data(), one.size() * sizeof(double), hipMemcpyHostToDevice, s));
    HIP_OK(hipMemcpyAsync(c->v_z.p, c->v_b.p, n3 * sizeof(double), hipMemcpyDeviceToDevice, s));
    HIP_OK(hipMemsetAsync(c->v_p.p, 0, n3 * sizeof(double), s));
    HIP_OK(hipMemsetAsync(c->v_t0.p, 0, n3 * sizeof(double), s));
    HIP_OK(hipMemsetAsync(c->v_Ap.p, 0, n3 * sizeof(double), s));
    PcgScal hs;
    memset(&hs, 0, sizeof(hs));
    hs.rzh[0] = hs.rzh[1] = 2.0; hs.thresh2 = -1.0; hs.bb = 1.0; hs.n_part1 = ns; hs.n_part2 = gb;
    HIP_OK(hipMemcpyAsync(c->scal.p, &hs, sizeof(PcgScal), hipMemcpyHostToDevice, s));
    HIP_OK(hipStreamSynchronize(s));
  } else
  {
    const size_t n3 = 3 * (size_t)c->NV;
    HIP_OK(hipMemcpyAsync(c->v_p.p, c->v_b.p, n3 * sizeof(double), hipMemcpyDeviceToDevice, s));
    HIP_OK(hipMemcpyAsync(c->v_r.p, c->v_b.p, n3 * sizeof(double), hipMemcpyDeviceToDevice, s));
    HIP_OK(hipMemcpyAsync(c->v_z.p, c->v_b.p, n3 * sizeof(double), hipMemcpyDeviceToDevice, s));
    CgScal hs;
    memset(&hs, 0, sizeof(hs));
    hs.rzn[3] = 1e-30; hs.rzn[0] = 1e-30; hs.pAp[0] = 1.0; hs.thresh2 = -1.0;
    HIP_OK(hipMemcpyAsync(c->scal.p, &hs, sizeof(CgScal), hipMemcpyHostToDevice, s));
  }
  for (int i = 0; i < 10; i++) launch();
  HIP_OK(hipEventRecord(e0, s));
  for (int i = 0; i < reps; i++) launch();
  HIP_OK(hipEventRecord(e1, s));
  HIP_OK(hipEventSynchronize(e1));
  float ms = 0;
  HIP_OK(hipEventElapsedTime(&ms, e0, e1));
  *us_per_launch = (double)ms * 1e3 / reps;
  (void)hipEventDestroy(e0); (void)hipEventDestroy(e1);
  return 0;
}

extern "C" int tsl_bench_direct(tsl_ctx* c, int cls, int reps, double* out4) {
  Scope scope(c);
  return direct_bench(c, cls, std::max(1, reps), out4);
}

extern "C" int tsl_direct_info(tsl_ctx* c, double* out10) {
  Scope scope(c);
  HIP_OK(hipStreamSynchronize(c->stream));
  const DirectSolver& d = c->ds;
  int bad[4] = {0, 0, 0, 0};
  if (d.bad.p) HIP_OK(hipMemcpy(bad, d.bad.p, sizeof(bad), hipMemcpyDeviceToHost));
  out10[0] = (double)d.n_plans; out10[1] = (double)d.n_factor; out10[2] = (double)d.n_apply; out10[3] = bad[1] + bad[2] + bad[3]; out10[4] = d.t_plan;
  out10[5] = d.plan_valid ? d.plan.sym.n_sn : 0; out10[6] = d.plan_valid ? d.plan.n_levels : 0; out10[7] = d.plan_valid ? (double)d.plan.batches.size() : 0;
  out10[8] = d.plan_valid ? d.plan.flops : 0; out10[9] = d.plan_valid ? 8.0 * (double)(d.plan.arena + d.plan.sarena) : 0;
  return 0;
}
extern "C" int tsl_direct_counters(tsl_ctx* c, double* out, int32_t n) {
  const DirectSolver& d = c->ds;
  double e = 0;
  if (d.plan_valid) for (const DsFrontDesc& f : d.plan.fr) e += (double)f.b * f.b;
  size_t parked = 0;
  for (const auto& sl : d.cache) parked += sl->used ? 1 : 0;
  int redo = 0;
  if (n > 12 && d.bad.p) { HIP_OK(hipStreamSynchronize(c->stream)); HIP_OK(hipMemcpy(&redo, d.bad.p + DS_REDO, sizeof(int), hipMemcpyDeviceToHost)); }
// ... 37 lines not shown
}

__global__ void __launch_bounds__(256) k_adj_x2a(ClothArgs A, const double* __restrict__ pos, const double* __restrict__ z, double* __restrict__ ag_prev) {
  const int h = blockIdx.x * blockDim.x + threadIdx.x;
  if (h >= A.n_hinge) return;
  const int f1 = A.hg_info[8 * h], l = A.hg_info[8 * h + 1], f2 = A.hg_info[8 * h + 2], p4 = A.hg_info[8 * h + 3], p21 = A.hg_info[8 * h + 4];
  const ClothDev c = A.cloth[A.cid[f1]];
  int v1[3], v2[3]; d3 P1[3], P2[3];
  load_face(pos, A.f2v, f1, v1, P1);
  load_face(pos, A.f2v, f2, v2, P2);
  const FaceGeom g1 = face_geom(P1), g2 = face_geom(P2);
  d3 g[4];
  hinge_grad(g1, g2, l, p4, p21, g);
  const double d_ref = -2.0 * c.Kb * c.dx * c.dx * (1.0 / 3.0);
  const double s = dot(ld3(z, pick3(v1, l)), g[0]) + dot(ld3(z, pick3(v1, (l + 1) % 3)), g[1]) + dot(ld3(z, pick3(v1, (l + 2) % 3)), g[2]) + dot(ld3(z, pick3(v2, p4)), g[3]);
  ag_prev[3 * f1 + l] += -s * d_ref;
}


__global__ void k_zfrozen_gather(int NV, const int* __restrict__ slice_off, const int* __restrict__ slice_len, const int* __restrict__ colidx, const int* __restrict__ trans,
                                 const unsigned char* __restrict__ fz, const double* __restrict__ vals, const double* __restrict__ zp, double* __restrict__ out) {
  const int c = blockIdx.x * blockDim.x + threadIdx.x;
  if (c >= NV) return;
  const unsigned cm = fz[c];
  double acc[3] = {0.0, 0.0, 0.0};
  if (cm) {
    const int slice = c >> 6, lane = c & 63, off = slice_off[slice], len = slice_len[slice];
    for (int k = 0; k < len; k++) {
      const int sl = off + 64 * k + lane;
      const int p = colidx[sl];
      const int tb = trans[sl];
      if (tb < 0) continue;
      const unsigned rm = fz[p];
      if (rm == 7u) continue;
      const d3 zi = ld3(zp, p);
      const double zr[3] = {zi.x, zi.y, zi.z};
      for (int cc = 0; cc < 3; cc++) {
        if (!((cm >> cc) & 1u)) continue;
        double s = 0;
        for (int r = 0; r < 3; r++) if (!((rm >> r) & 1u)) s += vals[(size_t)tb + 64 * (3 * r + cc)] * zr[r];
        acc[cc] -= s;
      }
    }
  }
  out[3 * (size_t)c] = acc[0]; out[3 * (size_t)c + 1] = acc[1]; out[3 * (size_t)c + 2] = acc[2];
}
__global__ void __launch_bounds__(256) k_contact_zfrozen_gather(int NV, const int* __restrict__ rowpos, const int* __restrict__ cr_ptr, const int* __restrict__ cr_ent,
                                                                const int* __restrict__ idx, const int* __restrict__ frozen, const double* __restrict__ Hfull,
                                                                const double* __restrict__ z, double* __restrict__ out) {
  const int v = (int)((blockIdx.x * (size_t)blockDim.x + threadIdx.x) >> 6), lane = threadIdx.x & 63;
  if (v >= NV) return;
  const int fz[3] = {frozen[3 * v], frozen[3 * v + 1], frozen[3 * v + 2]};
  if (!(fz[0] | fz[1] | fz[2])) return;
  const int p = rowpos[v];
  const int r0 = cr_ptr[p], r1 = cr_ptr[p + 1];
  if (r1 <= r0) return;
  double acc[3] = {0.0, 0.0, 0.0};
  for (int e = r0 + lane; e < r1; e += 64) {
    const int q = cr_ent[e], ci = q >> 2, a = q & 3;
    const double* H = Hfull + 144 * (size_t)ci;
    for (int cc = 0; cc < 3; cc++) {
      if (!fz[cc]) continue;
      double s = 0;
      for (int k = 0; k < 4; k++) {
        const int u = idx[4 * ci + k];
        for (int j = 0; j < 3; j++) if (!frozen[3 * u + j]) s += H[(3 * k + j) * 12 + 3 * a + cc] * z[3 * (size_t)u + j];
      }
      acc[cc] -= s;
    }
  }
  for (int cc = 0; cc < 3; cc++) { const double t = wave_sum(acc[cc]); if (lane == 0 && fz[cc]) out[3 * (size_t)v + cc] += t; }
}

__global__ void k_adj_prev(int NV, const double* __restrict__ z, const double* __restrict__ mass, const int* __restrict__ frozen, double dt, double d,
                           double* __restrict__ pg_prev, double* __restrict__ pg_prev2) {
  const size_t n = 3 * (size_t)NV;
  for (size_t i = blockIdx.x * (size_t)blockDim.x + threadIdx.x; i < n; i += (size_t)gridDim.x * blockDim.x) {
    if (frozen[i]) continue;
    const double xh = z[i] * mass[i / 3] / (dt * dt);
    if (pg_prev) pg_prev[i] += xh * (1.0 + d);
    if (pg_prev2) pg_prev2[i] -= xh * d;
  }
}

struct AdjArgs { int step, T; const double* pos_buffer; double* pos_grad; const double* ref_buffer; double* angleref_grad; double* tmp_z_frozen; double adj_damping; };

static int adjoint_pre(tsl_ctx* c, const AdjArgs& a, double** rhs) {
  hipStream_t s = c->stream;
  const int NV = c->NV;
  const size_t n3 = 3 * (size_t)NV, nr = 3 * (size_t)std::max(c->n_cface, 1);
  double* pg_s = a.pos_grad + (size_t)a.step * n3;
  double* pg_prev = a.pos_grad + (size_t)(a.step - 1) * n3;
  double* pg_prev2 = a.step > 1 ? a.pos_grad + (size_t)(a.step - 2) * n3 : nullptr;
  const double* x_s = a.pos_buffer + (size_t)a.step * n3;
  const double* x_prev = a.pos_buffer + (size_t)(a.step - 1) * n3;
  double* ag_s = a.angleref_grad + (size_t)a.step * nr;
  double* ag_prev = a.angleref_grad + (size_t)(a.step - 1) * nr;
  const double* ref_prev = a.ref_buffer + (size_t)(a.step - 1) * nr;
  (void)pg_prev; (void)pg_prev2; (void)ag_prev;
  hipLaunchKernelGGL(k_clamp, dim3(gsz(n3)), dim3(256), 0, s, n3, pg_s, c->adj_clamp);
  if (c->n_cface && c->adj_clamp_angleref)
    hipLaunchKernelGGL(k_clamp, dim3(gsz(3 * (size_t)c->n_cface)), dim3(256), 0, s, 3 * (size_t)c->n_cface, ag_s, 1000.0);
  int nc = 0;
  if (c->contact_enable) TSL_TRY(tsl_contact_detect(c, x_prev, x_prev, &nc));
  else { c->nc = 0; c->nc_ee = 0; c->ds.cons_checked = false; }
  ClothArgs CA = cloth_args(c);
  if (c->vg_stage.n < 3 * (size_t)std::max(c->vg_ns, 1)) { if (c->vg_stage.alloc(3 * (size_t)std::max(c->vg_ns, 1))) return tsl_fail("out of device memory (gradient staging)"); }
  if (c->n_hinge) {
    CA.gstage = c->vg_stage.p;
    hipLaunchKernelGGL(k_adj_a2ax, dim3(nblk(c->n_hinge, 256)), dim3(256), 0, s, CA, x_s, ref_prev, ag_s, ag_prev);
    hipLaunchKernelGGL(k_vertex_gather, dim3(nblk(NV, 256)), dim3(256), 0, s, NV, (const int*)c->vg_ptr.p, (const int*)c->vg_idx.p, (const double*)c->vg_stage.p, c->vg_hinge0, c->vg_tet0, pg_s);
    CA.gstage = nullptr;
  }
  const bool have_mg = !c->mg.empty() && c->mg_enable != 0;
  const bool spd_pc = c->adj_spd_pc && (have_mg || body_active(c)) && !(direct_enabled(c) && (c->ds.enable == 1 || c->ds.hard || c->n_tet > 0 || c->nc > 0));
  c->bd_valid = false;
  c->mg_omega_valid = false; c->mg_cinv_valid = false;
  if (spd_pc) {
    TSL_TRY(assemble(c, x_s, x_prev, x_prev, ref_prev, 1, nullptr));
    if (body_active(c)) TSL_TRY(body_build_inverse(c));
    if (have_mg) TSL_TRY(mg_setup_operators(c));
    if (c->vals_pc.n == 0 && c->vals_pc.alloc(c->vals.n)) return tsl_fail("out of device memory (vals_pc)");
    HIP_OK(hipMemcpyAsync(c->vals_pc.p, c->vals.p, c->vals.n * sizeof(double), hipMemcpyDeviceToDevice, s));
    if (c->nc > 0) {
      if (c->c_H_pc.n == 0 && c->c_H_pc.alloc(c->c_H.n)) return tsl_fail("out of device memory (c_H_pc)");
      HIP_OK(hipMemcpyAsync(c->c_H_pc.p, c->c_H.p, (size_t)c->nc * 144 * sizeof(double), hipMemcpyDeviceToDevice, s));
    }
    c->pc_frozen = true;
  }
  const int rc_asm = assemble(c, x_s, x_prev, x_prev , ref_prev, 0, nullptr);
  c->pc_frozen = false;
  if (rc_asm) return rc_asm;
  if (spd_pc) c->pc_separate = true;
  *rhs = pg_s;
  return 0;
}

static int adjoint_post(tsl_ctx* c, const AdjArgs& a) {
  hipStream_t s = c->stream;
  const int NV = c->NV;
  const size_t n3 = 3 * (size_t)NV, nr = 3 * (size_t)std::max(c->n_cface, 1);
  double* pg_s = a.pos_grad + (size_t)a.step * n3;
  double* pg_prev = a.pos_grad + (size_t)(a.step - 1) * n3;
  double* pg_prev2 = a.step > 1 ? a.pos_grad + (size_t)(a.step - 2) * n3 : nullptr;
  const double* x_s = a.pos_buffer + (size_t)a.step * n3;
  const double* x_prev = a.pos_buffer + (size_t)(a.step - 1) * n3;
  double* ag_s = a.angleref_grad + (size_t)a.step * nr;
  double* ag_prev = a.angleref_grad + (size_t)(a.step - 1) * nr;
  const double* ref_prev = a.ref_buffer + (size_t)(a.step - 1) * nr;
  (void)pg_s; (void)x_prev; (void)ag_s; (void)ref_prev;
  double* tmp_z_frozen = a.tmp_z_frozen;
  const double adj_damping = a.adj_damping;
  ClothArgs CA = cloth_args(c);
  hipLaunchKernelGGL(k_zfrozen_gather, dim3(nblk(NV, 256)), dim3(256), 0, s, NV, c->slice_off.p, c->slice_len.p, c->colidx.p, (const int*)c->trans.p, c->fzmask.p, c->vals_full.p,
                     c->v_x.p, c->v_t4.p);
  hipLaunchKernelGGL(k_scatter_perm, dim3(nblk(NV, 256)), dim3(256), 0, s, NV, c->perm.p, c->v_t4.p, tmp_z_frozen);
  if (c->nc > 0) {
    hipLaunchKernelGGL(k_contact_zfrozen_gather, dim3(nblk((long)NV * 64, 256)), dim3(256), 0, s, NV, (const int*)c->rowpos.p, (const int*)c->cr_ptr.p, (const int*)c->cr_ent.p, c->c_idx.p,
                       c->frozen.p, c->c_Hfull.p, c->pdir.p, tmp_z_frozen);
  }
  if (c->nc > 0) {
    if (c->c_G.n < 12 * (size_t)c->max_n_constraints) { if (c->c_G.alloc(12 * (size_t)c->max_n_constraints)) return -1; }
    const int nvf = c->nc - c->nc_ee;
    if (nvf > 0) hipLaunchKernelGGL(k_contact_backprop, dim3(nblk(nvf, 64)), dim3(64), 0, s, nvf, contact_args(c), x_s, c->pdir.p, c->c_G.p);
    if (c->nc_ee > 0) hipLaunchKernelGGL(k_ee_backprop, dim3(nblk(c->nc_ee, 64)), dim3(64), 0, s, c->nc_ee, ee_args(contact_args(c), nvf), x_s, c->pdir.p, c->c_G.p + 12 * (size_t)nvf);
    hipLaunchKernelGGL(k_contact_row_gather, dim3(nblk((long)NV * 64, 256)), dim3(256), 0, s, NV, (const int*)c->rowpos.p, (const int*)c->cr_ptr.p, (const int*)c->cr_ent.p,
                       (const double*)c->c_G.p, pg_prev);
  }
  if (c->n_hinge) hipLaunchKernelGGL(k_adj_x2a, dim3(nblk(c->n_hinge, 256)), dim3(256), 0, s, CA, x_s, c->pdir.p, ag_prev);
  hipLaunchKernelGGL(k_adj_prev, dim3(gsz(n3)), dim3(256), 0, s, NV, c->pdir.p, c->mass.p, c->frozen.p, c->dt, adj_damping, pg_prev, pg_prev2);
  HIP_OK(hipGetLastError());
  return 0;
}

extern "C" int tsl_adjoint_step(tsl_ctx* c, int step, int T, const double* pos_buffer, double* pos_grad, const double* ref_buffer, double* angleref_grad,
                                double* tmp_z_frozen, double adj_damping, tsl_solve_stats* st) {
  Scope scope(c);
  if (step < 1 || step >= T) return tsl_fail("tsl_adjoint_step: step %d outside [1, %d)", step, T);
  const AdjArgs a{step, T, pos_buffer, pos_grad, ref_buffer, angleref_grad, tmp_z_frozen, adj_damping};
  double* pg_s = nullptr;
  TSL_TRY(adjoint_pre(c, a, &pg_s));
  tsl_solve_stats local;
  if (!st) st = &local;
  TSL_TRY(solve_orig(c, pg_s, c->pdir.p, st));
  if (st->method == 4) TSL_TRY(direct_prezero(c));
  if (c->verbose) fprintf(stderr, "[tsl] adjoint step %d: nc %d solver flag %d iters %d restarts %d rel_residual %.2e\n", step, c->nc, st->flag, st->iters, st->restarts, st->rel_residual);
  TSL_TRY(adjoint_post(c, a));
  HIP_OK(hipStreamSynchronize(c->stream));
  HIP_OK(hipGetLastError());
  return 0;
}

extern "C" int tsl_group_adjoint_step(tsl_group* G, int step, int T, const double* const* pos_buffer_a, double* const* pos_grad_a, const double* const* ref_buffer_a,
                                      double* const* angleref_grad_a, double* const* tmp_z_a, const double* adj_damping_a, tsl_solve_stats* stats) {
  const int n = (int)G->m.size();
  tsl_ctx* g = G->g;
  if (step < 1 || step >= T) return tsl_fail("tsl_group_adjoint_step: step %d outside [1, %d)", step, T);
  std::vector<std::unique_ptr<Scope>> scopes;
  for (int i = 0; i < n; i++) scopes.emplace_back(new Scope(G->m[i]));
  std::vector<AdjArgs> aa(n);
  std::vector<int> act(n);
  for (int i = 0; i < n; i++) {
    if (!direct_enabled(G->m[i])) return tsl_fail("tsl_group_adjoint_step: scene %d does not use the sparse direct solve", i);
    aa[i] = AdjArgs{step, T, pos_buffer_a[i], pos_grad_a[i], ref_buffer_a[i], angleref_grad_a[i], tmp_z_a[i], adj_damping_a[i]};
    act[i] = i;
  }
  g->verbose = G->m[0]->verbose;
  TSL_TRY(G->pool->run(act, [&](int i) -> int {
    tsl_ctx* c = G->m[i];
    double* rhs = nullptr;
    TSL_TRY(adjoint_pre(c, aa[i], &rhs));
    hipLaunchKernelGGL(k_gather_perm, dim3(nblk(c->NV, 256)), dim3(256), 0, c->stream, c->NV, c->perm.p, (const double*)rhs, c->v_b.p);
    return 0;
  }));
  std::vector<tsl_solve_stats> ss;
  TSL_TRY(group_solve(G, act, ss, [](int) {}));
  TSL_TRY(G->pool->run(act, [&](int i) -> int {
    tsl_ctx* c = G->m[i];
    hipLaunchKernelGGL(k_scatter_perm, dim3(nblk(c->NV, 256)), dim3(256), 0, c->stream, c->NV, c->perm.p, (const double*)c->v_x.p, c->pdir.p);
    if (c->verbose) fprintf(stderr, "[tsl] group adjoint step %d, scene %d: nc %d solver flag %d iters %d restarts %d rel_residual %.2e\n", step, i, c->nc, ss[i].flag, ss[i].iters, ss[i].restarts,
                            ss[i].rel_residual);
    TSL_TRY(adjoint_post(c, aa[i]));
    return 0;
  }));
  for (int i = 0; i < n; i++) {
    HIP_OK(hipStreamSynchronize(G->m[i]->stream));
    if (stats) stats[i] = ss[i];
  }
  HIP_OK(hipGetLastError());
  return 0;
}
```

Measured before the change: 532,800.

## Gather element Hessians straight into the masked matrix, skipping full-matrix memset and mask pass

Adds a store mode to the block gather kernel. It writes the final masked value (mass diagonal plus element contributions, with frozen rows and columns replaced) directly into the solver matrix. This removes the memset of the unmasked copy, the vertex-Hessian pass and the separate k_mask_matrix pass during the grouped Newton assembly. Setup now ensures every pattern block is covered by a gather list and zeroes the uncovered padding slots once. The grad memset is also dropped, relying on k_vert_grad to overwrite. The unmasked copy is no longer formed in store mode, so the adjoint now fails if it follows a store-mode assembly without a re-assembly.

Result: no change. 531,600 (-0.2%).

```diff
diff --git a/include/tsl_hip.h b/include/tsl_hip.h
--- a/include/tsl_hip.h
+++ b/include/tsl_hip.h
@@ -81,6 +81,8 @@
 
 int tsl_assemble(tsl_ctx* ctx, const double* pos_dev, const double* prev_pos_dev, const double* vel_dev,
                  const double* ref_angle_dev, int spd, double* grad_dev);
+int tsl_assemble_flavour(tsl_ctx* ctx, const double* pos_dev, const double* prev_pos_dev, const double* vel_dev,
+                         const double* ref_angle_dev, int spd, double* grad_dev, int store);
 
 int tsl_solve(tsl_ctx* ctx, const double* rhs_dev, double* x_dev, tsl_solve_stats* stats_host);
 
@@ -109,6 +111,7 @@
 int tsl_matrix_nnzb(tsl_ctx* ctx, int32_t* nb_host, int32_t* nnzb_host);
 int tsl_matrix_export(tsl_ctx* ctx, int32_t* row_ptr_host, int32_t* col_host, double* vals_host);
 int tsl_matrix_import(tsl_ctx* ctx, const double* vals_host);
+int tsl_matrix_raw(tsl_ctx* ctx, double* vals_host, int64_t cap, int64_t* n_doubles);
 int tsl_constraints_export(tsl_ctx* ctx, int32_t* idx_host, double* w_host, double* k_host, double* dx0_host,
                            double* T_host, double* n_host, double* mu_host, int32_t max_n);
 int tsl_contact_blocks_export(tsl_ctx* ctx, double* blocks_host, int32_t max_n, int32_t masked);
diff --git a/thinshelllab_amd/_lib.py b/thinshelllab_amd/_lib.py
--- a/thinshelllab_amd/_lib.py
+++ b/thinshelllab_amd/_lib.py
@@ -66,8 +66,8 @@
 
 EXPORTS = [
     "tsl_version", "tsl_last_error", "tsl_ctx_create", "tsl_ctx_destroy", "tsl_set_stream", "tsl_set_param", "tsl_set_frozen",
-    "tsl_set_ext_force", "tsl_set_gravity", "tsl_energy", "tsl_assemble", "tsl_solve", "tsl_step", "tsl_contact_detect",
-    "tsl_contact_reset", "tsl_contact_counts", "tsl_update_ref_angle", "tsl_adjoint_step", "tsl_param_grad", "tsl_param_grad_keys", "tsl_friction_grad", "tsl_elastic_force", "tsl_matrix_nnzb", "tsl_matrix_export", "tsl_matrix_import",
+    "tsl_set_ext_force", "tsl_set_gravity", "tsl_energy", "tsl_assemble", "tsl_assemble_flavour", "tsl_solve", "tsl_step", "tsl_contact_detect",
+    "tsl_contact_reset", "tsl_contact_counts", "tsl_update_ref_angle", "tsl_adjoint_step", "tsl_param_grad", "tsl_param_grad_keys", "tsl_friction_grad", "tsl_elastic_force", "tsl_matrix_nnzb", "tsl_matrix_export", "tsl_matrix_import", "tsl_matrix_raw",
     "tsl_constraints_export", "tsl_contact_blocks_export", "tsl_proj_export", "tsl_proj_import", "tsl_set_border", "tsl_spd_project", "tsl_profile_reset", "tsl_profile_read", "tsl_profile_read_events",
     "tsl_bench_spmv", "tsl_bench_direct", "tsl_direct_info", "tsl_direct_counters",
     "tsl_group_create", "tsl_group_destroy", "tsl_group_step", "tsl_group_adjoint_step", "tsl_group_info",
@@ -101,6 +101,7 @@
     L.tsl_set_gravity.argtypes = [C.c_void_p, C.c_void_p]
     L.tsl_energy.argtypes = [C.c_void_p] + [C.c_void_p] * 4 + [C.POINTER(C.c_double)]
     L.tsl_assemble.argtypes = [C.c_void_p] + [C.c_void_p] * 4 + [C.c_int, C.c_void_p]
+    L.tsl_assemble_flavour.argtypes = [C.c_void_p] + [C.c_void_p] * 4 + [C.c_int, C.c_void_p, C.c_int]
     L.tsl_solve.argtypes = [C.c_void_p, C.c_void_p, C.c_void_p, C.POINTER(SolveStats)]
     L.tsl_step.argtypes = [C.c_void_p] + [C.c_void_p] * 4 + [C.POINTER(StepStats)]
     L.tsl_contact_detect.argtypes = [C.c_void_p, C.c_void_p, C.c_void_p, C.POINTER(C.c_int32)]
@@ -112,6 +113,7 @@
     L.tsl_matrix_nnzb.argtypes = [C.c_void_p, C.POINTER(C.c_int32), C.POINTER(C.c_int32)]
     L.tsl_matrix_export.argtypes = [C.c_void_p, C.c_void_p, C.c_void_p, C.c_void_p]
     L.tsl_matrix_import.argtypes = [C.c_void_p, C.c_void_p]
+    L.tsl_matrix_raw.argtypes = [C.c_void_p, C.c_void_p, C.c_int64, C.POINTER(C.c_int64)]
     L.tsl_constraints_export.argtypes = [C.c_void_p] + [C.c_void_p] * 7 + [C.c_int32]
     L.tsl_contact_blocks_export.argtypes = [C.c_void_p, C.c_void_p, C.c_int32, C.c_int32]
     L.tsl_proj_export.argtypes = [C.c_void_p] + [C.c_void_p] * 4
diff --git a/thinshelllab_amd/context.py b/thinshelllab_amd/context.py
--- a/thinshelllab_amd/context.py
+++ b/thinshelllab_amd/context.py
@@ -105,9 +105,9 @@
         check(self.L.tsl_energy(self.h, _ptr(pos), _ptr(prev_pos), _ptr(vel), _ptr(ref_angle), C.byref(e)), "tsl_energy")
         return e.value
 
-    def assemble(self, pos, prev_pos, vel, ref_angle, spd=True, grad=None):
-        self.refresh_stream()
-        check(self.L.tsl_assemble(self.h, _ptr(pos), _ptr(prev_pos), _ptr(vel), _ptr(ref_angle), int(bool(spd)), _ptr(grad)), "tsl_assemble")
+    def assemble(self, pos, prev_pos, vel, ref_angle, spd=True, grad=None, store=False):
+        self.refresh_stream()
+        check(self.L.tsl_assemble_flavour(self.h, _ptr(pos), _ptr(prev_pos), _ptr(vel), _ptr(ref_angle), int(bool(spd)), _ptr(grad), int(bool(store))), "tsl_assemble")
 
     def solve(self, rhs, x=None):
         self.refresh_stream()
@@ -177,6 +177,13 @@
         rp = np.zeros(nb.value + 1, np.int32); col = np.zeros(nnzb.value, np.int32); vals = np.zeros((nnzb.value, 3, 3), np.float64)
         check(self.L.tsl_matrix_export(self.h, rp.ctypes.data, col.ctypes.data, vals.ctypes.data), "tsl_matrix_export")
         return rp, col, vals
+
+    def matrix_raw(self):
+        n = C.c_int64(0)
+        check(self.L.tsl_matrix_raw(self.h, None, 0, C.byref(n)), "tsl_matrix_raw")
+        v = np.zeros(n.value, np.float64)
+        check(self.L.tsl_matrix_raw(self.h, v.ctypes.data, n.value, C.byref(n)), "tsl_matrix_raw")
+        return v
 
     def matrix_import(self, vals):
         rp, col, _ = self.matrix()
diff --git a/thinshelllab_amd/csrc/k_cloth.hpp b/thinshelllab_amd/csrc/k_cloth.hpp
--- a/thinshelllab_amd/csrc/k_cloth.hpp
+++ b/thinshelllab_amd/csrc/k_cloth.hpp
@@ -443,8 +443,17 @@
 }
 
 #define CG_BPW 28
+struct GatherStore {
+  const int2* rc;
+  const int* perm;
+  const double* mass; double dt;
+  const unsigned char* fz;
+  const double* mdt2;
+};
+template <bool STORE>
 __global__ void __launch_bounds__(256) k_cloth_gather(int n_blk, const int* __restrict__ base, const int* __restrict__ ptr, const unsigned* __restrict__ ent, int n_hinge, int n_cface,
-                                                      const double* __restrict__ hrec, const double* __restrict__ frec, const double* __restrict__ trec, double* __restrict__ vals) {
+                                                      const double* __restrict__ hrec, const double* __restrict__ frec, const double* __restrict__ trec, double* __restrict__ vals,
+                                                      GatherStore G) {
   __shared__ double tile[9][CG_BPW + 1];
   const int b0 = blockIdx.x * CG_BPW, t = threadIdx.x;
   if (t < 9 * CG_BPW) {
@@ -470,7 +479,21 @@
   __syncthreads();
   if (t < 9 * CG_BPW) {
     const int e9 = t / CG_BPW, bl = t - CG_BPW * e9, b = b0 + bl;
-    if (b < n_blk) vals[(size_t)base[b] + 64 * e9] += tile[e9][bl];
+    if (b < n_blk) {
+      if (!STORE) vals[(size_t)base[b] + 64 * e9] += tile[e9][bl];
+      else {
+        const int2 rc = G.rc[b];
+        const int r = e9 / 3, cc = e9 - 3 * r;
+        const bool dg = rc.x == rc.y && r == cc;
+        const unsigned rm = G.fz[rc.x], cm = G.fz[rc.y];
+        double prev = 0.0;
+        if (dg) prev = 0.0 + G.mass[G.perm[rc.x]] / (G.dt * G.dt);
+        double v = prev + tile[e9][bl];
+        if (((rm >> r) & 1u) || ((cm >> cc) & 1u)) v = 0.0;
+        if (dg && ((rm >> r) & 1u)) v = G.mdt2[rc.x];
+        vals[(size_t)base[b] + 64 * e9] = v;
+      }
+    }
   }
 }
 
diff --git a/thinshelllab_amd/csrc/k_solver.hpp b/thinshelllab_amd/csrc/k_solver.hpp
--- a/thinshelllab_amd/csrc/k_solver.hpp
+++ b/thinshelllab_amd/csrc/k_solver.hpp
@@ -30,6 +30,13 @@
       dst[base + 64 * e] = v;
     }
   }
+}
+
+__global__ void k_const_slots(int n_blk, const int* __restrict__ blk, double* __restrict__ vals) {
+  const int t = blockIdx.x * blockDim.x + threadIdx.x;
+  if (t >= 9 * n_blk) return;
+  const int b = t / 9, e = t - 9 * b;
+  vals[(size_t)blk[b] + 64 * e] = 0.0;
 }
 
 __global__ void k_block_jacobi(int NV, const int* __restrict__ diag_perm, const double* __restrict__ vals, const double* __restrict__ extra, double* __restrict__ Dinv) {
diff --git a/thinshelllab_amd/csrc/tsl_ctx.hpp b/thinshelllab_amd/csrc/tsl_ctx.hpp
--- a/thinshelllab_amd/csrc/tsl_ctx.hpp
+++ b/thinshelllab_amd/csrc/tsl_ctx.hpp
@@ -233,6 +233,12 @@
   std::vector<std::vector<int>> h_rows;
   DevBuf<int> rowpos, perm, slice_off, slice_len, colidx, diag_perm;
   DevBuf<double> vals, vals_full;
+  bool vals_full_valid = false;
+  bool vals_const_ok = true;
+  int asm_store = 1;
+  DevBuf<int> cg_rc;
+  DevBuf<int> cg_const;
+  int n_cg_const = 0;
   DevBuf<float> vals32;
   bool vals32_valid = false;
   int mg_f32 = 1;
diff --git a/thinshelllab_amd/csrc/tsl_hip.hip b/thinshelllab_amd/csrc/tsl_hip.hip
--- a/thinshelllab_amd/csrc/tsl_hip.hip
+++ b/thinshelllab_amd/csrc/tsl_hip.hip
@@ -267,7 +267,7 @@
     std::stable_sort(forder.begin(), forder.end(), [&](int x, int y) { return key[x] != key[y] ? key[x] < key[y] : f2v[3 * x] < f2v[3 * y]; });
   }
   UP(cf_order, forder);
-  std::vector<int> cg_base, cg_ptr;
+  std::vector<int> cg_base, cg_ptr, cg_rc, cg_const;
   std::vector<unsigned> cg_ent;
   {
     std::vector<std::pair<int, unsigned>> tup;
@@ -295,8 +295,51 @@
       cg_ent.push_back(tup[i].second);
     }
     cg_ptr.push_back((int)tup.size());
+    if (c->n_cface >= (1 << 26) || c->n_hinge >= (1 << 26) || c->n_tet >= (1 << 26)) { delete c; return tsl_fail("mesh too large for the packed gather lists"); }
+    {
+      std::vector<int> have(cg_base), miss;
+      std::sort(have.begin(), have.end());
+      for (int v = 0; v < NV; v++) if (!std::binary_search(have.begin(), have.end(), dblk[v])) miss.push_back(dblk[v]);
+      std::sort(miss.begin(), miss.end());
+      if (!miss.empty()) {
+        const int ncl = c->n_cgblk_cloth, nall = (int)cg_base.size();
+        std::vector<int> nb, np;
+        nb.reserve(nall + miss.size()); np.reserve(nall + miss.size() + 1);
+        size_t mi = 0;
+        for (int j = 0; j <= ncl; j++) {
+          while (mi < miss.size() && (j == ncl || miss[mi] < cg_base[j])) { nb.push_back(miss[mi++]); np.push_back(cg_ptr[j]); }
+          if (j < ncl) { nb.push_back(cg_base[j]); np.push_back(cg_ptr[j]); }
+        }
+        for (int j = ncl; j < nall; j++) { nb.push_back(cg_base[j]); np.push_back(cg_ptr[j]); }
+        np.push_back(cg_ptr[nall]);
+        cg_base.swap(nb); cg_ptr.swap(np);
+        c->n_cgblk_cloth += (int)miss.size();
+      }
+    }
     c->n_cgblk = (int)cg_base.size();
-    if (c->n_cface >= (1 << 26) || c->n_hinge >= (1 << 26) || c->n_tet >= (1 << 26)) { delete c; return tsl_fail("mesh too large for the packed gather lists"); }
+    {
+      std::vector<unsigned char> cov((size_t)P.n_slots, 0);
+      cg_rc.resize(2 * cg_base.size());
+      for (size_t b = 0; b < cg_base.size(); b++) {
+        const int a = cg_base[b];
+        if (a < 0) { delete c; return tsl_fail("gather lists: an element block outside the matrix pattern"); }
+        const long sl = (long)(a / 576) * 64 + a % 576;
+        if (a % 576 >= 64 || sl >= P.n_slots) { delete c; return tsl_fail("gather lists: block address %d is no slot of the value array", a); }
+        if (cov[sl]++) { delete c; return tsl_fail("gather lists: slot %ld is covered by two blocks (cloth and body lists overlap)", sl); }
+        const int slice = (int)(std::upper_bound(P.slice_off.begin(), P.slice_off.end(), (int)sl) - P.slice_off.begin()) - 1;
+        cg_rc[2 * b] = slice * 64 + (int)(sl & 63); cg_rc[2 * b + 1] = P.colidx[sl];
+      }
+      std::vector<unsigned char> pat((size_t)P.n_slots, 0);
+      for (int v = 0; v < NV; v++) {
+        const int pr = P.rowpos[v], s0 = pr >> 6, lane = pr & 63;
+        for (size_t k = 0; k < P.rows[v].size(); k++) pat[(size_t)P.slice_off[s0] + 64 * k + lane] = 1;
+      }
+      for (long sl = 0; sl < P.n_slots; sl++) {
+        if (pat[sl] != cov[sl]) { delete c; return tsl_fail("gather lists: slot %ld of the value array is %s", sl, pat[sl] ? "a block of the pattern that no list covers" : "padding, yet covered by a list"); }
+        if (!cov[sl]) cg_const.push_back((int)((sl >> 6) * 576 + (sl & 63)));
+      }
+      c->n_cg_const = (int)cg_const.size();
+    }
   }
   std::vector<int> vg_ptr(NV + 1, 0), vg_idx;
   {
@@ -313,7 +356,8 @@
   }
 
   UP(cf_blk, cfblk); UP(hg_info, hinfo); UP(hg_v, hv); UP(hg_blk, hgblk);
-  if (c->n_cgblk > 0) { UP(cg_base, cg_base); UP(cg_ptr, cg_ptr); UP(cg_ent, cg_ent); }
+  if (c->n_cgblk > 0) { UP(cg_base, cg_base); UP(cg_ptr, cg_ptr); UP(cg_rc, cg_rc); if (!cg_ent.empty()) UP(cg_ent, cg_ent); }
+  if (c->n_cg_const > 0) UP(cg_const, cg_const);
   UP(vg_ptr, vg_ptr); if (!vg_idx.empty()) UP(vg_idx, vg_idx);
   {
     std::vector<int> trans((size_t)P.n_slots, -1);
@@ -474,6 +518,7 @@
   else if (k == "direct_berr") c->ds.berr_tol = v;
   else if (k == "direct_small_rounds") { c->ds.small_rounds = std::max(1, (int)v); c->ds.plan_valid = false; c->ds.numeric_valid = false; c->ds.cache.clear(); }
   else if (k == "tet_warm") c->tet_warm = (int)v;
+  else if (k == "asm_store") c->asm_store = (int)v;
   else if (k == "ds_dbg") c->ds.dbg = (int)v;
   else if (k == "ds_bench_batch") c->ds.bench_batch = (int)v;
   else if (k == "direct_flow") c->ds.flow = std::max(0, (int)v);
@@ -656,21 +701,36 @@
   }
 }
 
-static int assemble_enqueue_early(tsl_ctx* c, const double* pos, const double* prev, const double* vel, const double* ref, int spd, double* grad, int tet_warm_flag);
-static int assemble_enqueue(tsl_ctx* c, const double* pos, const double* prev, const double* vel, const double* ref, int spd, double* grad, int tet_warm_flag) {
+static void cloth_gather_launch(tsl_ctx* c, hipStream_t s, int b0, int nb, bool store) {
+  const dim3 g(nblk(nb, CG_BPW)), b(256);
+  if (store) {
+    const GatherStore G{(const int2*)c->cg_rc.p + b0, c->perm.p, c->mass.p, c->dt, c->fzmask.p, c->mdt2.p};
+    hipLaunchKernelGGL(k_cloth_gather<true>, g, b, 0, s, nb, c->cg_base.p + b0, c->cg_ptr.p + b0, (const unsigned*)c->cg_ent.p, c->n_hinge, c->n_cface,
+                       (const double*)c->cg_hrec.p, (const double*)c->cg_frec.p, (const double*)c->cg_trec.p, c->vals.p, G);
+  } else
+    hipLaunchKernelGGL(k_cloth_gather<false>, g, b, 0, s, nb, c->cg_base.p + b0, c->cg_ptr.p + b0, (const unsigned*)c->cg_ent.p, c->n_hinge, c->n_cface,
+                       (const double*)c->cg_hrec.p, (const double*)c->cg_frec.p, (const double*)c->cg_trec.p, c->vals_full.p, GatherStore{});
+}
+static void const_slots_restore(tsl_ctx* c, hipStream_t s) {
+  if (c->vals_const_ok) return;
+  if (c->n_cg_const > 0) hipLaunchKernelGGL(k_const_slots, dim3(nblk(9L * c->n_cg_const, 256)), dim3(256), 0, s, c->n_cg_const, (const int*)c->cg_const.p, c->vals.p);
+  c->vals_const_ok = true;
+}
+
+static int assemble_enqueue_early(tsl_ctx* c, const double* pos, const double* prev, const double* vel, const double* ref, int spd, double* grad, int tet_warm_flag, bool store);
+static int assemble_enqueue(tsl_ctx* c, const double* pos, const double* prev, const double* vel, const double* ref, int spd, double* grad, int tet_warm_flag, bool store) {
   hipStream_t s = c->stream;
   const int NV = c->NV;
-  if (c->nc > 0 || c->n_tet > 0) return assemble_enqueue_early(c, pos, prev, vel, ref, spd, grad, tet_warm_flag);
-  HIP_OK(hipMemsetAsync(c->vals_full.p, 0, c->vals_full.n * sizeof(double), s));
+  c->vals_full_valid = !store;
+  if (c->nc > 0 || c->n_tet > 0) return assemble_enqueue_early(c, pos, prev, vel, ref, spd, grad, tet_warm_flag, store);
+  if (store) const_slots_restore(c, s);
+  else HIP_OK(hipMemsetAsync(c->vals_full.p, 0, c->vals_full.n * sizeof(double), s));
   if (c->n_cface) hipLaunchKernelGGL(k_cloth_normals, dim3(nblk(c->n_cface, 256)), dim3(256), 0, s, c->n_cface, pos, c->cf_f2v.p, c->norm_dir.p);
   ClothArgs CA = cloth_args(c);
   const VertArgs VA = vert_args(c);
   CA.gstage = c->vg_stage.p;
-  if (grad) {
-    HIP_OK(hipMemsetAsync(grad, 0, 3 * (size_t)NV * sizeof(double), s));
-    hipLaunchKernelGGL(k_vert_grad, dim3(nblk(NV, 256)), dim3(256), 0, s, VA, pos, prev, vel, grad);
-  }
-  hipLaunchKernelGGL(k_vert_hess, dim3(nblk(NV, 256)), dim3(256), 0, s, VA, c->diag_blk.p, c->vals_full.p);
+  if (grad) hipLaunchKernelGGL(k_vert_grad, dim3(nblk(NV, 256)), dim3(256), 0, s, VA, pos, prev, vel, grad);
+  if (!store) hipLaunchKernelGGL(k_vert_hess, dim3(nblk(NV, 256)), dim3(256), 0, s, VA, c->diag_blk.p, c->vals_full.p);
   if (grad) {
     if (c->n_cface) cloth_grad_face_launch(c, s, CA, pos);
     if (c->n_hinge) hipLaunchKernelGGL(k_cloth_grad_hinge, dim3(nblk(c->n_hinge, 256)), dim3(256), 0, s, CA, pos, ref);
@@ -681,15 +741,13 @@
     cloth_hess_face_launch(c, s, CA, pos, ref, spd);
   }
   if (c->n_hinge) hipLaunchKernelGGL(k_cloth_hess_hinge, dim3(nblk(c->n_hinge, 256)), dim3(256), 0, s, CA, pos, c->cg_hrec.p);
-  if (c->n_cgblk_cloth > 0)
-    hipLaunchKernelGGL(k_cloth_gather, dim3(nblk(c->n_cgblk_cloth, CG_BPW)), dim3(256), 0, s, c->n_cgblk_cloth, c->cg_base.p, c->cg_ptr.p, (const unsigned*)c->cg_ent.p, c->n_hinge, c->n_cface,
-                       (const double*)c->cg_hrec.p, (const double*)c->cg_frec.p, (const double*)c->cg_trec.p, c->vals_full.p);
+  if (c->n_cgblk_cloth > 0) cloth_gather_launch(c, s, 0, c->n_cgblk_cloth, store);
   if (grad) {
     hipLaunchKernelGGL(k_vertex_gather, dim3(nblk(NV, 256)), dim3(256), 0, s, NV, (const int*)c->vg_ptr.p, (const int*)c->vg_idx.p, (const double*)c->vg_stage.p, 0, c->vg_ns, grad);
     hipLaunchKernelGGL(k_mask_vec, dim3(gsz(3 * (size_t)NV)), dim3(256), 0, s, 3 * (size_t)NV, c->frozen.p, grad);
   }
-  hipLaunchKernelGGL(k_mask_matrix, dim3(c->n_slices), dim3(256), 0, s, c->n_slices, c->slice_off.p, c->slice_len.p, c->colidx.p, c->fzmask.p, c->mdt2.p,
-                     c->vals_full.p, c->vals.p, NV);
+  if (!store) hipLaunchKernelGGL(k_mask_matrix, dim3(c->n_slices), dim3(256), 0, s, c->n_slices, c->slice_off.p, c->slice_len.p, c->colidx.p, c->fzmask.p, c->mdt2.p,
+                                 c->vals_full.p, c->vals.p, NV);
   if (!c->pc_frozen) {
     if (direct_takes_solve(c)) c->dinv_valid = false;
     else TSL_TRY(block_jacobi_refresh(c));
@@ -698,7 +756,7 @@
   return 0;
 }
 
-static int assemble_enqueue_early(tsl_ctx* c, const double* pos, const double* prev, const double* vel, const double* ref, int spd, double* grad, int tet_warm_flag) {
+static int assemble_enqueue_early(tsl_ctx* c, const double* pos, const double* prev, const double* vel, const double* ref, int spd, double* grad, int tet_warm_flag, bool store) {
   hipStream_t s = c->stream, st = c->side;
   const bool fork_t = c->n_tet > 0 && c->nc > 0;
   hipStream_t stt = fork_t ? c->side2 : st;
@@ -724,13 +782,11 @@
     if (lit) hipLaunchKernelGGL(k_tet_hess_coop<true>, dim3(nblk(c->n_tet, 16)), dim3(256), 0, stt, TA, pos, spd, vws, 0, c->cg_trec.p);
     else hipLaunchKernelGGL(k_tet_hess_coop<false>, dim3(nblk(c->n_tet, 16)), dim3(256), 0, stt, TA, pos, spd, vws, vws ? tet_warm_flag : 0, c->cg_trec.p);
   }
-  HIP_OK(hipMemsetAsync(c->vals_full.p, 0, c->vals_full.n * sizeof(double), s));
+  if (store) const_slots_restore(c, s);
+  else HIP_OK(hipMemsetAsync(c->vals_full.p, 0, c->vals_full.n * sizeof(double), s));
   if (c->n_cface) hipLaunchKernelGGL(k_cloth_normals, dim3(nblk(c->n_cface, 256)), dim3(256), 0, s, c->n_cface, pos, c->cf_f2v.p, c->norm_dir.p);
-  if (grad) {
-    HIP_OK(hipMemsetAsync(grad, 0, 3 * (size_t)NV * sizeof(double), s));
-    hipLaunchKernelGGL(k_vert_grad, dim3(nblk(NV, 256)), dim3(256), 0, s, VA, pos, prev, vel, grad);
-  }
-  hipLaunchKernelGGL(k_vert_hess, dim3(nblk(NV, 256)), dim3(256), 0, s, VA, c->diag_blk.p, c->vals_full.p);
+  if (grad) hipLaunchKernelGGL(k_vert_grad, dim3(nblk(NV, 256)), dim3(256), 0, s, VA, pos, prev, vel, grad);
+  if (!store) hipLaunchKernelGGL(k_vert_hess, dim3(nblk(NV, 256)), dim3(256), 0, s, VA, c->diag_blk.p, c->vals_full.p);
   HIP_OK(hipEventRecord(c->ev_fork, s));
   if (c->n_cface) {
     const int nq = (int)c->h_cloth.size() * 9;
@@ -741,8 +797,7 @@
   if (c->n_hinge && !hh_side) hipLaunchKernelGGL(k_cloth_hess_hinge, dim3(nblk(c->n_hinge, 256)), dim3(256), 0, s, CA, pos, c->cg_hrec.p);
   const int nt_blk = c->n_cgblk - c->n_cgblk_cloth;
   if (c->n_tet && nt_blk > 0)
-    hipLaunchKernelGGL(k_cloth_gather, dim3(nblk(nt_blk, CG_BPW)), dim3(256), 0, stt, nt_blk, c->cg_base.p + c->n_cgblk_cloth, c->cg_ptr.p + c->n_cgblk_cloth, (const unsigned*)c->cg_ent.p,
-                       c->n_hinge, c->n_cface, (const double*)c->cg_hrec.p, (const double*)c->cg_frec.p, (const double*)c->cg_trec.p, c->vals_full.p);
+    cloth_gather_launch(c, stt, c->n_cgblk_cloth, nt_blk, store);
   HIP_OK(hipEventRecord(c->ev_join2, stt));
   if (grad) {
     if (fork_t) HIP_OK(hipStreamWaitEvent(st, c->ev_fork, 0));
@@ -754,11 +809,10 @@
   }
   if (hh_side && c->n_hinge) HIP_OK(hipStreamWaitEvent(s, c->ev_hh, 0));
   if (gather && c->n_cgblk_cloth > 0)
-    hipLaunchKernelGGL(k_cloth_gather, dim3(nblk(c->n_cgblk_cloth, CG_BPW)), dim3(256), 0, s, c->n_cgblk_cloth, c->cg_base.p, c->cg_ptr.p, (const unsigned*)c->cg_ent.p, c->n_hinge, c->n_cface,
-                       (const double*)c->cg_hrec.p, (const double*)c->cg_frec.p, (const double*)c->cg_trec.p, c->vals_full.p);
+    cloth_gather_launch(c, s, 0, c->n_cgblk_cloth, store);
   HIP_OK(hipStreamWaitEvent(s, c->ev_join2, 0));
-  hipLaunchKernelGGL(k_mask_matrix, dim3(c->n_slices), dim3(256), 0, s, c->n_slices, c->slice_off.p, c->slice_len.p, c->colidx.p, c->fzmask.p, c->mdt2.p,
-                     c->vals_full.p, c->vals.p, NV);
+  if (!store) hipLaunchKernelGGL(k_mask_matrix, dim3(c->n_slices), dim3(256), 0, s, c->n_slices, c->slice_off.p, c->slice_len.p, c->colidx.p, c->fzmask.p, c->mdt2.p,
+                                 c->vals_full.p, c->vals.p, NV);
   if (grad) {
     if (fork_t && c->n_tet) HIP_OK(hipStreamWaitEvent(st, c->ev_g2, 0));
     if (hh_side && c->n_cface) HIP_OK(hipStreamWaitEvent(st, c->ev_gf, 0));
@@ -777,7 +831,7 @@
   return 0;
 }
 
-static int assemble(tsl_ctx* c, const double* pos, const double* prev, const double* vel, const double* ref, int spd, double* grad) {
+static int assemble(tsl_ctx* c, const double* pos, const double* prev, const double* vel, const double* ref, int spd, double* grad, bool store = false) {
   hipStream_t s = c->stream;
   if (c->vg_stage.n < 3 * (size_t)std::max(c->vg_ns, 1)) { if (c->vg_stage.alloc(3 * (size_t)std::max(c->vg_ns, 1))) return tsl_fail("out of device memory (gradient staging)"); }
   if (c->n_tet > 0 && c->cg_trec.n < 144 * (size_t)c->n_tet) { if (c->cg_trec.alloc(144 * (size_t)c->n_tet)) return tsl_fail("out of device memory (element records)"); }
@@ -798,15 +852,18 @@
   c->ds.numeric_valid = false;
   if (spd != c->ds.anorm_spd) { c->ds.anorm_valid = false; c->ds.anorm_spd = spd; }
   if (!c->pc_frozen) { c->mg_ops_valid = false; c->pc_separate = false; }
-  return assemble_enqueue(c, pos, prev, vel, ref, spd, grad, warm);
-}
-
-extern "C" int tsl_assemble(tsl_ctx* c, const double* pos, const double* prev, const double* vel, const double* ref, int spd, double* grad) {
+  return assemble_enqueue(c, pos, prev, vel, ref, spd, grad, warm, store);
+}
+
+extern "C" int tsl_assemble_flavour(tsl_ctx* c, const double* pos, const double* prev, const double* vel, const double* ref, int spd, double* grad, int store) {
   Scope scope(c);
   c->bd_valid = false;
   c->mg_omega_valid = false; c->mg_cinv_valid = false;
   c->ds.anorm_valid = false;
-  return assemble(c, pos, prev, vel, ref, spd, grad);
+  return assemble(c, pos, prev, vel, ref, spd, grad, store != 0);
+}
+extern "C" int tsl_assemble(tsl_ctx* c, const double* pos, const double* prev, const double* vel, const double* ref, int spd, double* grad) {
+  return tsl_assemble_flavour(c, pos, prev, vel, ref, spd, grad, 0);
 }
 
 static ContactRows contact_rows(tsl_ctx* c, const double* blocks) {
@@ -2224,7 +2281,7 @@
   };
   const std::function<int(int)> assemble_one = [&](int i) -> int {
     tsl_ctx* c = m[i].c;
-    TSL_TRY(assemble(c, m[i].pos, m[i].prev, m[i].vel, m[i].ref, 1, c->F.p));
+    TSL_TRY(assemble(c, m[i].pos, m[i].prev, m[i].vel, m[i].ref, 1, c->F.p, c->asm_store != 0));
     hipLaunchKernelGGL(k_gather_perm, dim3(nblk(c->NV, 256)), dim3(256), 0, c->stream, c->NV, c->perm.p, (const double*)c->F.p, c->v_b.p);
     return 0;
   };
@@ -2480,6 +2537,14 @@
   return 0;
 }
 
+extern "C" int tsl_matrix_raw(tsl_ctx* c, double* vals, int64_t cap, int64_t* n) {
+  Scope scope(c);
+  HIP_OK(hipStreamSynchronize(c->stream));
+  if (n) *n = (int64_t)c->vals.n;
+  if (vals && cap >= (int64_t)c->vals.n) HIP_OK(hipMemcpy(vals, c->vals.p, c->vals.n * sizeof(double), hipMemcpyDeviceToHost));
+  return 0;
+}
+
 extern "C" int tsl_matrix_import(tsl_ctx* c, const double* vals) {
   Scope scope(c);
   HIP_OK(hipStreamSynchronize(c->stream));
@@ -2494,6 +2559,7 @@
     }
   }
   HIP_OK(hipMemcpy(c->vals.p, hv.data(), hv.size() * sizeof(double), hipMemcpyHostToDevice));
+  c->vals_const_ok = false;
   c->ds.numeric_valid = false; c->ds.anorm_valid = false;
   c->mg_ops_valid = false; c->pc_separate = false;
   c->bd_valid = false; c->mg_omega_valid = false; c->mg_cinv_valid = false;
@@ -2837,6 +2903,7 @@
   double* tmp_z_frozen = a.tmp_z_frozen;
   const double adj_damping = a.adj_damping;
   ClothArgs CA = cloth_args(c);
+  if (!c->vals_full_valid) return tsl_fail("adjoint step: the unmasked matrix copy is stale (the last assembly of this context was the Newton loop's, which does not form it)");
   hipLaunchKernelGGL(k_zfrozen_gather, dim3(nblk(NV, 256)), dim3(256), 0, s, NV, c->slice_off.p, c->slice_len.p, c->colidx.p, (const int*)c->trans.p, c->fzmask.p, c->vals_full.p,
                      c->v_x.p, c->v_t4.p);
   hipLaunchKernelGGL(k_scatter_perm, dim3(nblk(NV, 256)), dim3(256), 0, s, NV, c->perm.p, c->v_t4.p, tmp_z_frozen);
```
